# OpenDriveLab/ThinkTwice

Hardware: AMD Instinct MI355X
Metric: frames/sec forward (4-cam+LiDAR, thinktwice.py cfg) (higher is better)
Workload: dtype bf16x3h; 1 GPU; forward_inference thinktwice.py cfg: 8 frames x (2 sweeps x 4 cams x 448x896 + 65536-pt LiDAR), ResNet50+PAFPN+DepthNet+UNet+LSS splat, LidarNet, fusion, 5-stage decoder; parallelism=replicas x1 (no data-path collective), launch=eager launches, 3 batches in flight on alternating streams, batches_in_flight=3

## Files before the change

include/thinktwice_hip.h:

```cpp
#ifndef THINKTWICE_HIP_H
#define THINKTWICE_HIP_H

#include <stddef.h>
#include <stdint.h>

#ifdef __cplusplus
extern "C" {
#endif

#define TT_F32 0
#define TT_BF16 1
#define TT_F16 2

#define TT_ACT_NONE 0
#define TT_ACT_RELU 1
#define TT_ACT_SIGMOID 2
#define TT_ACT_GELU 3
#define TT_ACT_SOFTPLUS 4
#define TT_ACT_SOFTPLUS_CLAMP 5

const char* tt_last_error(void);
const char* tt_conv_last_kernel(void);
int tt_conv_set_trace(void* stamps_or_null);
int tt_version(void);

int tt_voxel_pool_fwd(int batch_size, int num_points, int num_channels,
                      int num_voxel_x, int num_voxel_y, int num_voxel_z,
                      const int32_t* geom_xyz, const float* input_features,
                      float* output_features, int32_t* pos_memo, void* stream);

long long tt_voxel_pool_workspace_bytes(int batch_size, int num_points, int num_channels,
                                        int num_voxel_x, int num_voxel_y);
int tt_voxel_pool_fwd_ws(int batch_size, int num_points, int num_channels,
                         int num_voxel_x, int num_voxel_y, int num_voxel_z,
                         const int32_t* geom_xyz, const float* input_features,
                         float* output_features, int32_t* pos_memo,
                         void* workspace, long long workspace_bytes, void* stream);
int tt_voxel_pool_fwd_plan(int batch_size, int num_points, int num_channels,
                           int num_voxel_x, int num_voxel_y, int num_voxel_z,
                           const int32_t* geom_xyz, const float* input_features,
                           float* output_features, int32_t* pos_memo,
                           void* workspace, long long workspace_bytes, int ws_entry, char* label, int label_bytes);

long long tt_voxel_pool_plan_bytes(int batch_size, int num_points, int num_voxel_x, int num_voxel_y);
long long tt_voxel_pool_plan_workspace_bytes(int batch_size, int num_points);
int tt_voxel_pool_plan_build(int batch_size, int num_points, int num_voxel_x, int num_voxel_y, int num_voxel_z,
                             const int32_t* geom_xyz, void* workspace, long long workspace_bytes, void* plan,
                             long long plan_bytes, void* stream);
long long tt_voxel_pool_planned_workspace_bytes(int batch_size, int num_points, int num_channels, int num_voxel_x,
                                                int num_voxel_y);
int tt_voxel_pool_fwd_planned(int batch_size, int num_points, int num_channels, int num_voxel_x, int num_voxel_y,
                              const void* plan, const float* input_features, float* output_features, void* workspace,
                              long long workspace_bytes, void* stream);

int tt_voxel_pool_bwd(int batch_size, int num_points, int num_channels,
                      int num_voxel_x, int num_voxel_y,
                      const int32_t* pos_memo, const float* grad_out_bhwc,
                      float* grad_in, void* stream);

int tt_frustum_voxel_index(int batch_size, int num_cams, int D, int fH, int fW,
                           const float* frustum, const float* mats,
                           const float* voxel_lo, const float* voxel_size,
                           int32_t* geom_xyz, float* geom_f32_or_null,
                           void* stream);

int tt_lift_splat_fwd(int batch_size, int num_cams, int D, int fH, int fW, int C,
                      int num_voxel_x, int num_voxel_y, int num_voxel_z,
                      const void* depth_logits, const void* context, int dtype,
                      const int32_t* geom_xyz, float* out, int out_cstride,
                      int out_coff, int rot_flip, void* stream);

long long tt_lift_splat_workspace_bytes(int batch_size, int num_cams, int D, int fH, int fW, int C,
                                        int num_voxel_x, int num_voxel_y);
int tt_lift_splat_fwd_ws(int batch_size, int num_cams, int D, int fH, int fW, int C,
                         int num_voxel_x, int num_voxel_y, int num_voxel_z,
                         const void* depth_logits, const void* context, int dtype,
                         const int32_t* geom_xyz, float* out, int out_cstride,
                         int out_coff, int rot_flip, void* ws, long long ws_bytes, void* stream);
int tt_lift_splat_fwd_plan(int batch_size, int num_cams, int D, int fH, int fW, int C,
                           int num_voxel_x, int num_voxel_y, int num_voxel_z,
                           const void* depth_logits, const void* context, int dtype,
                           const int32_t* geom_xyz, float* out, int out_cstride,
                           int out_coff, int rot_flip, void* ws, long long ws_bytes, char* label, int label_bytes);

typedef struct tt_conv_desc {
    const void* in;   int N, H, W, Cin, in_cstride, in_coff;
    long long in_nstride;
    const void* weight; int Cout, KH, KW, stride, pad, dil;
    void* out; int OH, OW, out_cstride, out_coff;
    long long out_nstride;
    int pixel_shuffle2;
    const float* scale; const float* shift;
    const float* shift_n; int shift_n_mod;
    const void* res1; int res1_cstride, res1_coff;
    const void* res2; int res2_cstride, res2_coff;
    int act;
    int dtype;
    int out_dtype;
    const int* gather_idx;
    const int* m_dev;
    float* splitk_ws;
    const void* weight_x3;
    const int* row_perm;
    const unsigned* row_mask;
    int splitk_slices;
    int in_pair, out_pair;
    const void* weight_h2;
    float* out2; int out2_cstride, out2_coff;
    int res1_up_h, res1_up_w;
    int res1_f32;
    int in_up2;
} tt_conv_desc;

int tt_conv2d_fwd(const tt_conv_desc* d, void* stream);
int tt_conv2d_splitk_slices(const tt_conv_desc* d);
int tt_conv2d_plan(const tt_conv_desc* d, char* label, int label_bytes);

int tt_seg_feedback_chain(const float* x, long long R, int x_stride, int K1, const float* w1, const float* scale1,
                          const float* shift1, int act1, const float* w2, const void* w2_x3, int N2, const float* scale2,
                          const float* shift2, int act2, float* out, int out_stride, int out_coff, void* stream);

typedef struct tt_chain_stage {
    const void* w; const float* bias;
    int K, Kp, N, act, in_sel;
    const float* res; int res_stride, res_coff;
    const float* side; const float* side_w; int side_stride, side_k;
    float* out; int out_stride, out_coff;
} tt_chain_stage;
int tt_mlp_chain(const float* x, long long R, int x_stride, int nstages, const tt_chain_stage* stages, int n_split,
                 void* stream);
long long tt_mlp_chain_wide_workspace_bytes(long long R, int nstages, const tt_chain_stage* stages);
int tt_mlp_chain_wide(const float* x, long long R, int x_stride, int nstages, const tt_chain_stage* stages, int n_groups,
                      void* workspace, long long workspace_bytes, void* stream);
int tt_mlp_chain_wide_max_workgroups(void);
int tt_mlp_chain_wide_faults(void);
int tt_device_faults(void);
int tt_clear_device_faults(void);
int tt_mlp_chain_wide_set_max_spin(int polls);
int tt_mlp_chain_wide_set_trace(void* stamps_or_null);

long long tt_dec_gru_scratch_floats(int B);
int tt_dec_gru(int B, const float* inp6, const float* state, float* fut, float* scratch, const void* const* w0,
               const float* const* wx, const float* const* b0, const void* const* w2, const float* const* b2,
               const void* wd0, const float* bd0, const void* wd2, const float* bd2, void* stream);
long long tt_dec_flatten_scratch_floats(int maps);
int tt_dec_flatten(int maps, const float* in, float* out, float* mids_or_null, float* scratch, const void* const* w,
                   const float* const* b, const float* bn_scale, const float* bn_shift, void* stream);
int tt_dec_set_trace(void* stamps_or_null);
long long tt_dec_bev_update_scratch_floats(int B);
int tt_dec_bev_update(int B, const float* bev, const float* G, float* out, long long out_bstride, float* out2,
                      long long out2_bstride, float* scratch, const void* w0, const float* b0, const void* const* w2,
                      const float* b2, void* stream);

int tt_nchw_to_nhwc_pad(const float* in, void* out, int N, int C, int H, int W, int Cp,
                        int out_dtype, void* stream);
int tt_nchw_to_nhwc_border(const float* in, void* out, int N, int C, int H, int W, int Cp, int Hp, int Wp,
                           int top, int left, int out_dtype, void* stream);
int tt_nhwc_to_nchw(const void* in, float* out, int N, int C, int H, int W, int cstride, int coff,
                    int in_dtype, void* stream);
int tt_maxpool3x3s2(const void* in, void* out, int N, int H, int W, int C, int dtype, void* stream);
int tt_upsample_nearest_add(void* dst, const void* src, int N, int H, int W, int C, int h, int w,
                            int dtype, void* stream);
int tt_bilinear_up2(const void* in, void* out, int N, int H, int W, int C, int dtype, void* stream);
int tt_bilinear_up2_pair(const float* in, float* out, int N, int H, int W, int C, void* stream);
int tt_spatial_pool(const void* in, float* out, int N, int HW, int C, int cstride, int coff, int mode,
                    int dtype, void* stream);
int tt_channel_gate(const void* x, const float* gate, const void* res, void* out, int N, int HW, int C,
                    int gate_act, int out_act, int dtype, void* stream);
int tt_affine_rows(const void* x, const float* scale, const float* shift, void* out, long long R, int C,
                   int x_stride, int out_stride, int act, int dtype, void* stream);
int tt_layernorm_rows(const void* x, const float* gamma, const float* beta, void* out, long long R,
                      int D, int x_stride, int out_stride, float eps, int dtype, void* stream);
int tt_copy_nhwc(const void* in, void* out, int N, int H, int W, int C, int in_cstride, int in_coff,
                 int out_cstride, int out_coff, int rot_flip, int in_dtype, int out_dtype, void* stream);
int tt_broadcast_rows(const void* v, void* out, int N, int HW, int C, int v_stride, int out_cstride,
                      int out_coff, int dtype, void* stream);
int tt_ew(const void* a, const void* b, const void* g, void* out, long long R, int C, int a_stride,
          int a_coff, int b_stride, int b_coff, int g_stride, int g_coff, int o_stride, int o_coff,
          int op, int act, int dtype, void* stream);
int tt_concat_rows(float* out, long long R, int out_stride, int nseg, const float* const* srcs, const int* strides,
                   const int* widths, const int* coffs, const int* divs, const int* mods, void* stream);

int tt_deform_im2col3x3(const void* x, const float* offsets, void* cols, int N, int H, int W, int C,
                        int off_cstride, int pad, int dtype, void* stream);

int tt_look_project_pack(int B, const float* wp, const float* lidar2img, const float* ida_mat,
                         float img_h, float img_w, float* ref_packed, int* query_of_slot,
                         int* count, int* max_len, void* stream);
int tt_look_gather_query(int B, const int* query_of_slot, const float* ref_packed, const float* wp,
                         const float* ctrl_softplus, const float* temporal_embedding,
                         const float* static_embedding, const float* measurement_feat,
                         const float* flattened_feat, const void* const* level_maps,
                         const int* level_hw, int maps_dtype, float* out, int row_stride, void* stream);
int tt_msda_sample(int B, const void* value, int value_dtype, const float* offsets, const float* logits,
                   const float* ref_packed, const int* level_hw, float* out, void* stream);
int tt_msda_sample_strided(int B, const void* value, int value_dtype, int value_cstride, int value_coff,
                           const float* offsets, const float* logits, const float* ref_packed, const int* level_hw,
                           float* out, void* stream);
int tt_sca_reduce(int B, const float* x, const int* max_len, float* out, void* stream);

int tt_look_query_ln(int B, const int* query_of_slot, const float* ref_packed, const float* wp, const float* ctrl,
                     int raw_ctrl, const float* temporal_embedding, const float* static_embedding,
                     const float* measurement_feat, const float* flattened_feat, const void* const* level_maps,
                     const int* level_hw, int maps_dtype, const float* gamma, const float* beta, float eps, float* out,
                     int row_stride, void* stream);
int tt_msda_sample_ln(int B, const void* value, int value_dtype, int value_cstride, int value_coff,
                      const float* offsets, const float* logits, const float* ref_packed, const int* level_hw,
                      const float* gamma, const float* beta, float eps, float* out, float* out_ln,
                      const int* max_len_or_null, void* stream);
int tt_msda_sample_proj_ln(int B, const void* const* level_maps, const int* level_hw, const float* offsets,
                           const float* logits, const float* ref_packed, const float* wvT, const float* bias,
                           const float* vshift, const float* gamma, const float* beta, float eps, float* out,
                           float* out_ln, const int* max_len_or_null, void* stream);
int tt_sca_reduce_ln(int B, const float* x, const int* max_len, const float* gamma, const float* beta, float eps,
                     float* out, void* stream);
int tt_dec_merge_in(int B, const float* fflat, const float* look, const float* temporal_embedding,
                    const float* measurement_feat, const float* gamma, const float* beta, float eps, float* out,
                    void* stream);

long long tt_lidar_voxelize_workspace_bytes(long long num_points_total);
int tt_lidar_voxelize(const float* points, int B, int Np, int nfeat, const float* pc_range_lo,
                      const float* voxel_size, const int* grid_xyz, int z_limit, int max_points,
                      void* workspace, long long workspace_bytes, float* voxel_feats, int* coords,
                      int* num_voxels, void* stream);
long long tt_lidar_voxelize_capped_workspace_bytes(long long num_points_total);
int tt_lidar_voxelize_capped(const float* points, int B, int Np, int nfeat, const float* pc_range_lo, const float* voxel_size,
                             const int* grid_xyz, int z_limit, int max_points, int max_voxels, void* workspace,
                             long long workspace_bytes, float* voxel_feats, int* coords, int* num_voxels, void* stream);
int tt_sp_volume_build(const int* coords, const int* num_rows, long long max_rows, int batch,
                       const int* dims_zyx, int* vol, void* stream);
long long tt_sp_strided_outputs_workspace_bytes(long long out_cells);
int tt_sp_strided_outputs(const int* in_coords, const int* in_rows, long long max_in, int batch,
                          const int* kernel_stride_pad, const int* out_dims_zyx, void* workspace,
                          long long workspace_bytes, int* out_vol, int* out_coords, int* out_rows,
                          long long max_out, void* stream);
int tt_sp_rulebook(const int* out_coords, const int* out_rows, long long max_out,
                   const int* kernel_stride_pad, const int* in_dims_zyx, const int* in_vol, int* nbr,
                   void* stream);
long long tt_sp_tile_plan_workspace_bytes(long long max_rows);
int tt_sp_tile_plan(const int* nbr, const int* num_rows, long long max_rows, int KV, void* workspace,
                    long long workspace_bytes, int* row_perm, unsigned* row_mask_sorted,
                    unsigned long long* pairs_or_null, void* stream);
int tt_sp_to_dense(const void* feats, const int* coords, const int* num_rows, long long max_rows, int C,
                   const int* dims_zyx, void* dense, int dtype, void* stream);

int tt_preprocess_images(const uint8_t* raw_hwc, int num_images, int H, int W, const float* mapx,
                         const float* mapy, int resized_h, int resized_w, int crop_y, int crop_x,
                         int out_h, int out_w, const float* mean3, const float* std3, void* out_nhwc,
                         int out_channels_padded, int out_dtype, float* out_nchw_or_null, void* stream);

#define TT_IDA_MAX_SETS 64
typedef struct tt_ida_set {
    int resized_h, resized_w;
    int crop_y, crop_x;
    int flip;
} tt_ida_set;
int tt_preprocess_images_ida(const uint8_t* raw_hwc, int B, int T, int N, int H, int W, const float* mapx,
                             const float* mapy, const tt_ida_set* sets, int out_h, int out_w, const float* mean3,
                             const float* std3, void* out_nhwc, int out_channels_padded, int out_dtype,
                             float* out_nchw_or_null, void* stream);
int tt_preprocess_labels_ida(const float* maps, int B, int N, int H, int W, const float* mapx, const float* mapy,
                             const tt_ida_set* sets, int out_h, int out_w, float* out, void* stream);

#define TT_AUG_MAX_OPS 8
#define TT_AUG_NOISE_K 4
#define TT_AUG_LUT 0
#define TT_AUG_NOISE 1
#define TT_AUG_DROPOUT 2
#define TT_AUG_COARSE 3
// ... 329 lines not shown
```

thinktwice_amd/build.py:

```python
import os
import subprocess
import sys
from concurrent.futures import ThreadPoolExecutor

from . import _lib

HERE = os.path.dirname(os.path.abspath(__file__))
CSRC = os.path.join(HERE, "csrc")
OBJ = os.path.join(CSRC, "_obj")
LIB = os.path.join(HERE, "libthinktwice_hip.so")
HIPCC = os.environ.get("HIPCC", "/opt/rocm/bin/hipcc")
FLAGS = ["--offload-arch=gfx950", "-O3", "-std=c++17", "-fPIC", "-munsafe-fp-atomics", "-ffp-contract=off",
         "-Wno-unused-result"]


EXTRA_FLAGS = {"conv_x3_pipe.hip": ["-fno-slp-vectorize"], "conv_x3_up2.hip": ["-fno-slp-vectorize"],
               "conv_x3_patch.hip": ["-fno-slp-vectorize"]}


def _sources():
    return sorted(f for f in os.listdir(CSRC) if f.endswith((".hip", ".cpp")))


def _deps_mtime():
    hdrs = [os.path.join(CSRC, f) for f in os.listdir(CSRC) if f.endswith((".h", ".inc"))]
    hdrs.append(os.path.join(HERE, "..", "include", "thinktwice_hip.h"))
    hdrs.append(os.path.abspath(__file__))
    return max(os.path.getmtime(h) for h in hdrs)


def _compile(src, hdr_mtime, verbose):
    obj = os.path.join(OBJ, src + ".o")
    spath = os.path.join(CSRC, src)
    if os.path.exists(obj) and os.path.getmtime(obj) > max(os.path.getmtime(spath), hdr_mtime):
        return obj
    cmd = [HIPCC] + FLAGS + EXTRA_FLAGS.get(src, []) + (["-x", "hip"] if src.endswith(".hip") else []) + ["-c", spath, "-o", obj]
    if verbose:
        print(" ".join(cmd), flush=True)
    subprocess.run(cmd, check=True)
    return obj


def write_plan_thunks():
    lines = ["// GENERATED by thinktwice_amd/build.py from include/thinktwice_hip.h -- do not edit.",
             "// One thunk per stream-taking entry: tt_plan argument vector -> the entry's own signature.", ""]
    table = []
    for name, p in _lib.prototypes().items():
        if not _lib.takes_stream(name, p.params):
            continue
        casts = []
        for i, (t, _) in enumerate(p.params[:-1]):
            if "*" in t:
                casts.append(f"({t})a[{i}].p")
            elif t in ("float", "double"):
                casts.append(f"({t})a[{i}].d")
            else:
                casts.append(f"({t})a[{i}].i")
        casts.append("stream")
        lines.append(f"static int thunk_{name}(const PlanVal* a, void* stream) {{ return {name}({', '.join(casts)}); }}")
        table.append((name, len(p.params) - 1))
    lines.append("")
    lines.append("static const PlanThunk kPlanThunks[] = {")
    for name, n in table:
        lines.append(f'    {{"{name}", thunk_{name}, {n}}},')
    lines.append("};")
    text = "\n".join(lines) + "\n"
    out = os.path.join(CSRC, "plan_thunks.inc")
    if not os.path.exists(out) or open(out).read() != text:
        open(out, "w").write(text)


def source_fingerprint():
    import hashlib
    h = hashlib.sha256()
    files = [os.path.join(CSRC, f) for f in sorted(os.listdir(CSRC)) if f.endswith((".hip", ".cpp", ".h"))]
    files.append(os.path.join(HERE, "..", "include", "thinktwice_hip.h"))
    for f in files:
        h.update(os.path.basename(f).encode())
        h.update(open(f, "rb").read())
    return h.hexdigest()[:16]


def build(verbose=True, force=False):
    os.makedirs(OBJ, exist_ok=True)
    write_plan_thunks()
    if force:
        for f in os.listdir(OBJ):
            os.remove(os.path.join(OBJ, f))
    hdr_mtime = _deps_mtime()
    srcs = _sources()
    with ThreadPoolExecutor(max_workers=min(8, len(srcs))) as ex:
        objs = list(ex.map(lambda s: _compile(s, hdr_mtime, verbose), srcs))
    if (not os.path.exists(LIB)) or any(os.path.getmtime(o) > os.path.getmtime(LIB) for o in objs):
        cmd = [HIPCC, "--offload-arch=gfx950", "-shared", "-fPIC", "-o", LIB] + objs
        if verbose:
            print(" ".join(cmd), flush=True)
        subprocess.run(cmd, check=True)
    host_src = os.path.join(HERE, "..", "tools", "plan_host.cpp")
    host_bin = os.path.join(HERE, "..", "tools", "plan_host")
    if os.path.exists(host_src) and (not os.path.exists(host_bin) or
                                     os.path.getmtime(host_bin) < max(os.path.getmtime(host_src), os.path.getmtime(LIB))):
        cmd = [HIPCC, "--offload-arch=gfx950", "-O2", "-std=c++17", "-Wno-unused-result", "-I", os.path.join(HERE, "..", "include"),
               host_src, "-L", HERE, "-lthinktwice_hip", "-Wl,-rpath,$ORIGIN/../thinktwice_amd", "-o", host_bin]
        if verbose:
            print(" ".join(cmd), flush=True)
        subprocess.run(cmd, check=True)
    return LIB


if __name__ == "__main__":
    build(verbose=True, force="--force" in sys.argv)
    print(LIB)
```

thinktwice_amd/csrc/conv_choose.cpp:

```cpp
#include <stdint.h>

#include "conv_choose.h"

namespace tt {
namespace {

bool aligned16(const void* p) { return (reinterpret_cast<uintptr_t>(p) & 15) == 0; }

void set_tile(ConvChoice* c, int family, int bn, int waves_m, int waves_n, int bkb, int stages) {
    c->family = family;
    c->bn = bn;
    c->waves_m = waves_m;
    c->waves_n = waves_n;
    c->bkb = bkb;
    c->stages = stages;
}

bool choose_h2(const ConvArgs& a, ConvChoice* c) {
    if (a.gather || a.m_dev || a.ws || a.pixel_shuffle2 || a.Cin % 64 != 0 || a.KH * a.KW > 31 || a.K < 64) return false;
    static const bool pipe = env_flag("TT_H2_PIPE", true);
    if (pipe && a.Cout % 128 == 0 && a.K >= 1152) set_tile(c, CONV_H2_PIPE, 128, 4, 1, 128, 32);
    else if (a.Cout > 64) set_tile(c, CONV_H2, 128, 4, 2, 128, 32);
    else set_tile(c, CONV_H2, 64, 8, 1, 128, 33);
    return true;
}

bool choose_small(const ConvArgs& a, ConvChoice* c) {
    if (a.gather || a.m_dev || a.M > 4096) return false;
    if ((long long)div_up(a.M, 32) * div_up(a.Cout, 32) > 4096) return false;
    set_tile(c, CONV_SMALL, 32, 1, 1, 32, 1);
    return true;
}

int tail_split_rows(const ConvArgs& a) {
    if (a.Cout % 256 != 0) return 0;
    const int tiles_m = div_up(a.M, 256), tiles_n = a.Cout / 256;
    const long long T = (long long)tiles_m * tiles_n;
    const int rounds = (int)((T + kNumCU - 1) / kNumCU);
    const int last = (int)(T - (long long)kNumCU * (rounds - 1));
    if (rounds < 2 || rounds > 8 || last > kNumCU / 4) return 0;
    const int peel = div_up(last, tiles_n);
    return peel < tiles_m ? tiles_m - peel : 0;
}

bool choose_x3_splitk(const ConvArgs& a, bool assume_ws, ConvChoice* c) {
    if (a.gather || a.m_dev || a.M < 512 || a.M > 8192 || a.Cout < 64 || a.KH * a.KW > 32) return false;
    if (a.Cin % 32 != 0 || a.K < 1024 || a.pixel_shuffle2) return false;
    const int tiles = div_up(a.M, 256) * div_up(a.Cout, 64);
    const int nk = a.K / 32;
    if (tiles >= 256) return false;
    int sp = 512 / tiles;
    if (sp > nk / 8) sp = nk / 8;
    if (sp > 16) sp = 16;
    if (sp < 2) return false;
    const int slices = div_up(nk, div_up(nk, sp));
    if (slices < 2 || (!assume_ws && a.ws_slices < slices)) return false;
    set_tile(c, CONV_GLDS, 64, 8, 1, 128, 2);
    c->x3 = true;
    c->splits = sp;
    c->slices = slices;
    return true;
}

bool choose_sp_runs_l2(const ConvArgs& a, ConvChoice* c) {
    if (!a.gather || a.row_perm || a.KH != 1 || a.KW != 27 || a.pixel_shuffle2 || a.M < kSpL2MinRows) return false;
    if ((a.Cin != 16 && a.Cin != 32) || (a.Cout != 16 && a.Cout != 32 && a.Cout != 64)) return false;
    if ((a.in_cstride & 3) || (a.in_coff & 3) || !aligned16(a.in) || !a.vec_epi || a.out_dtype != TT_F32) return false;
    set_tile(c, CONV_SP_RUNS_L2, 32, 8, 1, a.Cin * 4, 1);
    c->gather = c->x3 = true;
    return true;
}

bool choose_sp_runs(const ConvArgs& a, ConvChoice* c) {
    if (!a.gather || a.row_perm || a.KH != 1 || a.KW != 27) return false;
    if (a.stride != 1) return false;
    if (a.Cin % 32 != 0 || a.Cin > 128 || a.M < 2048 || a.pixel_shuffle2) return false;
    if ((a.in_cstride & 3) || (a.in_coff & 3)) return false;
    if (a.Cout == 32) set_tile(c, CONV_SP_RUNS, 32, 8, 1, 128, 2);
    else if (a.Cout == 64) set_tile(c, CONV_SP_RUNS, 64, 8, 1, 128, 2);
    else if (a.Cout == 128) set_tile(c, CONV_SP_RUNS, 128, 4, 2, 128, 2);
    else return false;
    c->gather = c->x3 = true;
    return true;
}

bool x3_pipe_ok(const ConvArgs& a, int bn) {
    return !(a.gather || a.m_dev || (bn != 256 && bn != 128) || a.Cout % bn != 0 || a.Cin % 32 != 0 || a.KH * a.KW > 31 || a.K < 64);
}

bool choose_x3_patch(const ConvArgs& a, ConvChoice* c) {
    static const bool on = env_flag("TT_X3_PATCH", true);
    if (!on || !(a.flags & 32) || a.M < kPatchMinRows) return false;
    if (a.KH != 3 || a.KW != 3 || a.stride != 1 || a.pad != 1 || a.dil != 1 || a.OH != a.H || a.OW != a.W) return false;
    if (a.Cin % 32 != 0 || !(a.Cout == 64 || (a.Cout >= 8 && a.Cout <= 32)) || !a.vec_epi || a.out_dtype != TT_F32) return false;
    if (a.res1 || a.res2 || a.shift_n || a.out2 || a.ws || a.pixel_shuffle2 || a.gather || a.m_dev) return false;
    if ((long long)a.H * a.W * a.in_cstride >= (1ll << 30)) return false;
    if (a.Cout == 64 && a.K >= 1152) return false;
    set_tile(c, CONV_X3_PATCH, a.Cout == 64 ? 64 : 32, 8, 1, 128, 3);
    return true;
}

bool choose_x3(const ConvArgs& a, ConvChoice* c) {
    c->x3 = true;
    if (a.gather) {
        if (choose_sp_runs_l2(a, c)) return true;
        if (choose_sp_runs(a, c)) return true;
        const bool cin_ok = a.Cin >= 16 && (a.Cin & (a.Cin - 1)) == 0;
        if (!cin_ok || a.M < 2048 || a.Cout < 16 || a.Cout > 128) return false;
        set_tile(c, CONV_GLDS, a.Cout <= 32 ? 32 : (a.Cout <= 64 ? 64 : 128), 8, 1, 128, 2);
        c->gather = true;
        return true;
    }
    if (a.m_dev || a.M < 2048 || a.KH * a.KW > 32) return false;
    if (a.Cin % 32 != 0 || a.K < 64) return false;
    const bool apair = (a.flags & 32) != 0;
    if (apair && (a.in_coff % 16 != 0 || a.in_cstride % 16 != 0)) return false;
    c->apair = apair;
    if (choose_x3_patch(a, c)) return true;
    if (a.Cout < 64) {
        if (a.Cout > 32 || a.Cout < 8) return false;
        if (!apair && a.M < (1 << 16)) return false;
        set_tile(c, CONV_GLDS, 32, 8, 1, 128, 2);
        return true;
    }
    const int tiles_m = div_up(a.M, 256);
    auto cost = [&](int bn, double rate) {
        const long long tiles = (long long)tiles_m * div_up(a.Cout, bn);
        return (double)((tiles + kNumCU - 1) / kNumCU) * bn / rate;
    };
    const bool wide = a.Cout % 256 == 0 || a.Cout > 512;
    const int main_rows = tail_split_rows(a);
    auto cost256 = [&]() {
        if (!main_rows) return cost(256, 1.0);
        const long long tn = a.Cout / 256;
        const long long main_tiles = (long long)main_rows * tn, tail_tiles = (long long)(tiles_m - main_rows) * tn * 4;
        return (double)((main_tiles + kNumCU - 1) / kNumCU) * 256 / 1.0 + (double)((tail_tiles + kNumCU - 1) / kNumCU) * 64 / 0.63;
    };
    const double c256 = wide ? cost256() : 1e30;
    const double c128 = a.Cout > 64 ? cost(128, (a.K >= 1152 && a.Cout % 128 == 0) ? 0.95 : 0.85) : 1e30;
    const double c64 = cost(64, 0.63);
    const int bn = (c256 <= c128 && c256 <= c64) ? 256 : (c128 <= c64 ? 128 : 64);
    static const bool pipe = env_flag("TT_X3_PIPE", true);
    if (pipe && a.K >= 1152 && bn != 64 && x3_pipe_ok(a, bn)) {
        static const bool run3 = env_flag("TT_X3_RUN3", true);
        const bool runs = run3 && a.KW == 3 && a.KH <= 5 && a.stride == 1 && a.dil == 1 && a.pad == 1 && a.OH == a.H && a.OW == a.W &&
                          (a.N == 1 || a.in_nstride == (long long)a.H * a.W * a.in_cstride);
        set_tile(c, runs ? CONV_X3_RUN3 : CONV_X3_PIPE, bn, 4, 1, 128, 23);
    } else if (bn == 256) {
        set_tile(c, CONV_GLDS, 256, 4, 2, 128, 23);
    } else {
        set_tile(c, CONV_GLDS, bn, 8, 1, 128, 2);
    }
    if (bn == 256) c->main_rows = main_rows;
    return true;
}

int choose_up2(const ConvArgs& a, const ConvFacts& f, ConvChoice* c) {
    TT_REQUIRE(f.dtype == TT_F32 && a.out_dtype == TT_F32 && f.weight_x3 && aligned16(f.weight_x3) && !f.weight_h2,
               "tt_conv2d_fwd: in_up2 goes with a bf16x3 layer (f32 storage, a 16-byte aligned weight_x3)");
    TT_REQUIRE(!a.gather && !a.m_dev && !a.ws && !a.pixel_shuffle2 && !(a.flags & 32) && !a.res1 && !a.res2 && !a.shift_n && !f.out2,
               "tt_conv2d_fwd: in_up2 takes no in_pair, residual, per-image shift, out2, split-K workspace, gather or pixel shuffle");
    TT_REQUIRE(a.KH == 3 && a.KW == 3 && a.stride == 1 && a.pad == 1 && a.dil == 1 && a.H % 2 == 0 && a.W % 2 == 0 && a.OH == a.H &&
                   a.OW == a.W,
               "tt_conv2d_fwd: in_up2 is a 3 x 3 / stride 1 / pad 1 layer over an even H x W (got %d x %d, k %d x %d s %d p %d d %d)", a.H,
               a.W, a.KH, a.KW, a.stride, a.pad, a.dil);
    TT_REQUIRE(a.Cin % 32 == 0 && a.Cout == 64 && a.M > 4096 && a.vec_epi,
               "tt_conv2d_fwd: in_up2 layer outside the kernel's contract (Cin %% 32 == 0, Cout == 64, more than 4096 rows, aligned "
               "output: M=%d Cin=%d Cout=%d)", a.M, a.Cin, a.Cout);
    const long long img = (long long)(a.H / 2) * (a.W / 2) * a.Cin;
    TT_REQUIRE(a.in_cstride == a.Cin && a.in_coff == 0 && a.in_nstride == img && img < (1ll << 30),
               "tt_conv2d_fwd: in_up2 reads a contiguous [N][H/2][W/2][Cin] source of less than 2^30 elements per image");
    set_tile(c, CONV_X3_UP2, 64, 8, 1, 128, 3);
    c->x3 = true;
    return 0;
}

bool choose_glds(const ConvArgs& a, int dtype, ConvChoice* c) {
    constexpr int min_tiles = 2;
    if (a.gather) {
        const bool cin_ok = a.Cin >= 16 && (a.Cin & (a.Cin - 1)) == 0;
        if (dtype == TT_F32 || !cin_ok || a.M < 2048 || a.Cout < 16 || a.Cout > 128) return false;
        if (a.Cout <= 32) set_tile(c, CONV_GLDS, 32, 8, 1, 128, 2);
        else if (a.Cout <= 64) set_tile(c, CONV_GLDS, 64, 8, 1, 128, 2);
        else set_tile(c, CONV_GLDS, 128, 4, 2, 128, 2);
        c->gather = true;
        return true;
    }
    if (a.m_dev || a.M < 2048 || a.Cout < 64 || a.KH * a.KW > 32) return false;
    if (dtype == TT_F32) {
        if (a.Cin % 16 != 0 || div_up(a.K, 16) < min_tiles) return false;
        if (a.Cout > 64) set_tile(c, CONV_GLDS, 128, 4, 2, 64, 3);
        else set_tile(c, CONV_GLDS, 64, 8, 1, 64, 3);
        return true;
    }
    if (a.Cin % 32 != 0 || div_up(a.K, 32) < min_tiles) return false;
    if (a.Cout > 64) {
        const long long tiles256 = (long long)div_up(a.M, 256) * (a.Cout / 256);
        if (a.Cout % 256 == 0 && tiles256 >= 200) {
            if (a.Cin % 64 == 0) {
                set_tile(c, CONV_GLDS, 256, 2, 4, 128, 2);
                c->main_rows = tail_split_rows(a);
            } else {
                set_tile(c, CONV_GLDS, 256, 2, 4, 64, 3);
            }
        } else if (a.K <= 512) {
            set_tile(c, CONV_GLDS, 128, 2, 2, 64, 3);
        } else {
            set_tile(c, CONV_GLDS, 128, 4, 2, 64, 3);
        }
        return true;
    }
    if (a.Cin % 64 == 0) set_tile(c, CONV_GLDS, 64, 8, 1, 128, 2);
    else set_tile(c, CONV_GLDS, 64, 8, 1, 64, 3);
    return true;
}

int choose_igemm(const ConvArgs& a, int dtype, bool ws, bool assume_ws, ConvChoice* c) {
    if (a.Cout > 64) set_tile(c, CONV_IGEMM, 128, 2, 2, 64, 2);
    else if (a.Cout > 32) set_tile(c, CONV_IGEMM, 64, 2, 2, 64, 2);
    else set_tile(c, CONV_IGEMM, 32, 4, 1, 64, 2);
    if (dtype != TT_F32) c->bkb = 128;
    c->gather = a.gather != nullptr;
    const int tiles = div_up(a.M, 128) * div_up(a.Cout, c->bn);
    const int nk = div_up(a.K, c->bkb / (dtype == TT_F32 ? 4 : 2));
    if (ws && !a.m_dev && tiles < 128 && nk >= 8) {
        int sp = div_up(512, tiles);
        if (sp > nk / 2) sp = nk / 2;
        if (sp > 64) sp = 64;
        c->splits = sp < 1 ? 1 : sp;
    }
    if (c->splits <= 1) return 0;
    c->slices = c->splits;
    if (!assume_ws) {
        c->slices = 0;
        if (a.ws_slices > 0) {
            const int eff = div_up(nk, div_up(nk, c->splits));
            TT_REQUIRE(a.ws_slices >= eff, "tt_conv2d_fwd: split-K workspace holds %d slices, %d needed", a.ws_slices, eff);
            c->slices = eff;
        }
    }
    return 0;
}

}

int conv_choose(const ConvArgs& a, const ConvFacts& f, ConvChoice* c) {
    *c = ConvChoice{};
    c->splits = 1;
    const bool ws = a.ws || f.assume_ws;
    if (a.flags & 256) return choose_up2(a, f, c);
    if (f.weight_h2) {
        TT_REQUIRE(aligned16(f.weight_h2), "tt_conv2d_fwd: weight_h2 must be 16-byte aligned");
        TT_REQUIRE(choose_h2(a, c), "tt_conv2d_fwd: weight_h2 layer outside the h2 kernel's contract (Cin=%d KH*KW=%d)", a.Cin,
                   a.KH * a.KW);
        return 0;
    }
    TT_REQUIRE(!f.out2 || a.vec_epi, "tt_conv2d_fwd: out2 needs the vector epilogue (aligned channel counts)");
    TT_REQUIRE(!f.res1_up || a.vec_epi, "tt_conv2d_fwd: an upsampled res1 needs the vector epilogue (aligned channel counts)");
    TT_REQUIRE(!f.res1_f32 || (a.vec_epi && a.res_vec), "tt_conv2d_fwd: an f32 res1 needs the vector epilogue and aligned residual rows");
    TT_REQUIRE(!(f.dtype == TT_F32 && a.out_dtype != TT_F32 && a.res1) || (a.vec_epi && a.res_vec),
               "tt_conv2d_fwd: a 16-bit output of an f32 layer with a residual needs the vector epilogue");
    if (a.flags & (32 | 64)) {
        TT_REQUIRE(a.vec_epi && aligned16(f.weight_x3) && a.K % 16 == 0,
                   "tt_conv2d_fwd: in_pair / out_pair need the vector epilogue and a 16-byte aligned weight_x3");
        TT_REQUIRE(choose_x3(a, c), "tt_conv2d_fwd: pair-format layer outside the LDS-DMA bf16x3 kernel's contract (M=%d Cin=%d Cout=%d)",
                   a.M, a.Cin, a.Cout);
        return 0;
    }
    if (!ws && !f.out2 && !f.res1_up && !f.res1_f32 && choose_small(a, c)) return 0;
    const bool x3 = f.weight_x3 && f.dtype == TT_F32;
    if (ws && x3 && a.K % 16 == 0 && aligned16(f.weight_x3) && choose_x3_splitk(a, f.assume_ws, c)) return 0;
    if (!ws && x3) {
        TT_REQUIRE(aligned16(f.weight_x3) && a.K % 16 == 0, "tt_conv2d_fwd: weight_x3 needs 16-byte alignment and K %% 16 == 0 (K = %d)",
                   a.K);
        if (choose_x3(a, c)) return 0;
        *c = ConvChoice{};
        c->splits = 1;
    }
    if (!ws && choose_glds(a, f.dtype, c)) return 0;
    return choose_igemm(a, f.dtype, ws, f.assume_ws, c);
}

ConvChoice conv_tail_choice(const ConvChoice& c) {
    ConvChoice t{};
    set_tile(&t, CONV_GLDS, 64, 8, 1, 128, 2);
    t.x3 = c.x3;
    t.apair = c.apair;
    t.splits = 1;
    return t;
}

void conv_label(const ConvChoice& c, int dtype, char* out, size_t bytes) {
    const char* tn = dtype == TT_F32 ? "float" : "16-bit";
    const char* pre = c.apair ? " pre-split A" : "";
    const char* tail = c.main_rows > 0 ? " + tail" : "";
    switch (c.family) {
        case CONV_H2: snprintf(out, bytes, "conv_h2_kernel<%d, %d, %d, %d, %d>", c.bn, c.waves_m, c.waves_n, c.stages / 10, c.stages % 10); break;
        case CONV_H2_PIPE: snprintf(out, bytes, "conv_h2_pipe_kernel"); break;
        case CONV_SMALL: snprintf(out, bytes, "conv_small_kernel"); break;
        case CONV_SP_RUNS_L2: snprintf(out, bytes, "sp_conv_runs_l2_kernel<%d>", c.bkb / 4); break;
        case CONV_SP_RUNS: snprintf(out, bytes, "sp_conv_runs_kernel<%d, %d, %d>", c.bn / (32 * c.waves_n), c.waves_m, c.waves_n); break;
        case CONV_X3_PIPE: snprintf(out, bytes, "conv_x3_pipe_kernel<%s>%s%s", c.bn == 128 ? "4, 1, 128" : "4, 1", pre, tail); break;
        case CONV_X3_RUN3: snprintf(out, bytes, "conv_x3_run3_kernel<%d>%s%s", c.bn, pre, tail); break;
        case CONV_X3_UP2: snprintf(out, bytes, "conv_x3_run3_kernel<%d, up2>", c.bn); break;
        case CONV_X3_PATCH: snprintf(out, bytes, "conv_x3_run3_kernel<%d, patch>%s", c.bn, pre); break;
        case CONV_GLDS:
            snprintf(out, bytes, "conv_igemm_glds_kernel<%s, %d, %d, %d, %d, %d, %s, %s>%s%s", tn, c.bn, c.waves_m, c.waves_n, c.bkb,
                     c.stages, c.gather ? "true" : "false", c.x3 ? "true" : "false", pre, c.splits > 1 ? " split-K" : tail);
            break;
        default: snprintf(out, bytes, "conv_igemm_kernel<%s, 128, %d>%s", tn, c.bn, c.splits > 1 ? " split-K" : ""); break;
    }
}

}
```

thinktwice_amd/csrc/conv_choose.h:

```cpp
#pragma once
#include <stddef.h>

#include "tt_common.h"

namespace tt {

struct ConvArgs {
    const void* in;
    const void* weight;
    void* out;
    const float* scale;
    const float* shift;
    const float* shift_n;
    const void* res1;
    const void* res2;
    const int* gather;
    const int* m_dev;
    const int* row_perm;
    const unsigned* row_mask;
    float* ws;
    long long in_nstride, out_nstride;
    int N, H, W, Cin, in_cstride, in_coff;
    int Cout, KH, KW, stride, pad, dil;
    int OH, OW, out_cstride, out_coff;
    int pixel_shuffle2, shift_n_mod;
    int res1_cstride, res1_coff, res2_cstride, res2_coff;
    int act, out_dtype;
    int M, K;
    int cin_fast;
    int out_fast;
    int vec_epi;
    int res_vec;
    int splits;
    int tiles_n;
    int m_begin;
    int ws_slices;
    int flags;
    int res1_up_h, res1_up_w;
    float* out2;
    int out2_cstride, out2_coff;
    long long* trace;
};

enum ConvFamily {
    CONV_H2,
    CONV_H2_PIPE,
    CONV_SMALL,
    CONV_SP_RUNS_L2,
    CONV_SP_RUNS,
    CONV_X3_PIPE,
    CONV_X3_RUN3,
    CONV_X3_UP2,
    CONV_X3_PATCH,
    CONV_GLDS,
    CONV_IGEMM,
};

constexpr int kSpL2MinRows = 16384;

constexpr int kPatchMinRows = 16384;

struct ConvFacts {
    int dtype;
    const void* weight_x3;
    const void* weight_h2;
    bool out2, res1_up, res1_f32;
    bool assume_ws;
};

struct ConvChoice {
    int family;
    int bn;
    int waves_m, waves_n, bkb, stages;
    bool gather, x3, apair;
    int main_rows;
    int splits;
    int slices;
};

int conv_choose(const ConvArgs& a, const ConvFacts& f, ConvChoice* c);
ConvChoice conv_tail_choice(const ConvChoice& c);
void conv_label(const ConvChoice& c, int dtype, char* out, size_t bytes);

}
```

thinktwice_amd/csrc/conv_common.h:

```cpp
#pragma once
#include <type_traits>
#include "bf16x3.h"
#include "conv_choose.h"

namespace tt {
extern thread_local char g_conv_kernel[96];
extern long long* g_conv_trace;

template <int TN>
__device__ __forceinline__ void zero_acc(f32x16 (&acc)[TN]) {
#pragma unroll
    for (int j = 0; j < TN; ++j)
#pragma unroll
        for (int r = 0; r < 16; ++r) acc[j][r] = 0.f;
}
template <int TM, int TN>
__device__ __forceinline__ void zero_acc(f32x16 (&acc)[TM][TN]) {
#pragma unroll
    for (int i = 0; i < TM; ++i) zero_acc(acc[i]);
}

template <int TN, int WTN>
__device__ __forceinline__ void stage_scaled(float* sC, const f32x16 (&acc)[TN], const float (&sc)[TN],
                                             const float (&sh)[TN], int lane) {
// ... 211 lines not shown
                        if constexpr (RM == 2) add_rvf(v, r1[q]);
                        else if constexpr (RM == 1) add_rv(v, r1[q]);
                        if (act == TT_ACT_RELU) {
#pragma unroll
                            for (int e = 0; e < CO; ++e) v[e] = v[e] > 0.f ? v[e] : 0.f;
                        }
                        store_row((long long)mr * p.out_cstride + obase, v);
                        if (out2) store_row2(mr, v);
                    }
                }
            };
            if (!has_r1) hot(std::integral_constant<int, 0>{});
            else if (EXT && sizeof(T) == 2 && r1_f32) {
                if constexpr (EXT && sizeof(T) == 2) hot(std::integral_constant<int, 2>{});
            } else hot(std::integral_constant<int, 1>{});
        } else {
#pragma unroll 1
            for (int pass = 0; pass < NPASS; ++pass) {
                const int rl = pass * rpp + row_in_pass;
                const int m = mb + rl;
                if (m >= Mlim || !col_ok) continue;
                float v[CO];
#pragma unroll
                for (int e = 0; e < CO; e += 4) {
                    const float4 t0 = *reinterpret_cast<const float4*>(sC + rl * LDC + col_l + e);
                    v[e] = t0.x; v[e + 1] = t0.y; v[e + 2] = t0.z; v[e + 3] = t0.w;
                }
                int n = 0;
                const int mo = p.row_perm ? p.row_perm[m] : m;
                const long long o = out_offset(mo, co, n);
                if (sn_loop) {
                    const float* sn = p.shift_n + (long long)(n % p.shift_n_mod) * cout_real + co;
#pragma unroll
                    for (int e = 0; e < CO; ++e) v[e] += sn[e];
                }
#pragma unroll
                for (int which = 0; which < 2; ++which) {
                    const void* rb = which ? p.res2 : p.res1;
                    if (!rb) continue;
                    const T* rp = reinterpret_cast<const T*>(rb) +
                                  (which ? (long long)mo : res1_row(mo)) * (which ? p.res2_cstride : p.res1_cstride) +
                                  (which ? p.res2_coff : p.res1_coff) + co;
                    if (which == 0 && r1_f32) {
                        const float* rf = reinterpret_cast<const float*>(rb) + res1_row(mo) * p.res1_cstride + p.res1_coff + co;
#pragma unroll
                        for (int e = 0; e < CO; ++e) v[e] += rf[e];
                    } else if (rvec) {
                        add_rv(v, *reinterpret_cast<const RV*>(rp));
                    } else {
#pragma unroll
                        for (int e = 0; e < CO; ++e) v[e] += Elem<T>::ld(rp + e);
                    }
                }
#pragma unroll
                for (int e = 0; e < CO; ++e) v[e] = apply_act(v[e], act);
                store_row(o, v);
                if (out2) store_row2(mo, v);
            }
        }
    }
}

template <typename T, int TM, int TN, int WTM, int WTN, bool EXT = (sizeof(T) == 4)>
__device__ __forceinline__ void conv_epilogue(const ConvArgs& p, f32x16 (&acc)[TM][TN], unsigned char* smem,
                                              int wave, int lane, int wm, int wn, int m0, int n0, int Mlim) {
    const int cout_real = p.pixel_shuffle2 ? (p.Cout >> 2) : p.Cout;
    const int ohw = p.OH * p.OW;
    if (p.act == 99) return;
    if (p.ws) {
#pragma unroll
        for (int j = 0; j < TN; ++j) {
            const int col = n0 + wn * WTN + j * 32 + (lane & 31);
            if (col >= p.Cout) continue;
#pragma unroll
            for (int i = 0; i < TM; ++i)
#pragma unroll
                for (int r = 0; r < 16; ++r) {
                    const int m = m0 + wm * WTM + i * 32 + (r & 3) + 8 * (r >> 2) + 4 * (lane >> 5);
                    if (m < Mlim) {
                        if (p.ws_slices > 0) p.ws[((long long)blockIdx.y * p.M + m) * p.Cout + col] = acc[i][j][r];
                        else unsafeAtomicAdd(p.ws + (long long)m * p.Cout + col, acc[i][j][r]);
                    }
                }
        }
        return;
    }
    float* sC = reinterpret_cast<float*>(smem) + wave * (32 * (WTN + 4));
    __syncthreads();
    if (p.vec_epi) {
        if (p.out_dtype == TT_F32 && !(p.flags & 64))
            conv_epilogue_vec<T, 4, TM, TN, WTM, WTN, EXT>(p, acc, sC, lane, wm, wn, m0, n0, Mlim);
        else
            conv_epilogue_vec<T, 8, TM, TN, WTM, WTN, EXT>(p, acc, sC, lane, wm, wn, m0, n0, Mlim);
        return;
    }
    constexpr int LDC = WTN + 4;
    const int act = p.act;
    float sc[TN], sh[TN];
    load_scale_shift<TN, WTN>(p, sc, sh, lane, wn, n0);
#pragma unroll
    for (int i = 0; i < TM; ++i) {
        stage_scaled<TN, WTN>(sC, acc[i], sc, sh, lane);
#pragma unroll 1
        for (int idx = lane; idx < 32 * WTN; idx += 64) {
            const int rl = idx / WTN, cl = idx - rl * WTN;
            const int m = m0 + wm * WTM + i * 32 + rl;
            const int col = n0 + wn * WTN + cl;
            if (m >= Mlim || col >= p.Cout) continue;
            int co = col, q = 0;
            if (p.pixel_shuffle2) {
                q = col / cout_real;
                co = col - q * cout_real;
            }
            float v = sC[rl * LDC + cl];
            const int n = m / ohw;
            const int mo = p.row_perm ? p.row_perm[m] : m;
            long long o;
            if (p.out_fast) {
                o = (long long)mo * p.out_cstride + p.out_coff + co;
            } else {
                const int rem = m - n * ohw;
                int oh = rem / p.OW, ow = rem - oh * p.OW;
                int OWo = p.OW;
                if (p.pixel_shuffle2) {
                    oh = 2 * oh + (q >> 1);
                    ow = 2 * ow + (q & 1);
                    OWo = 2 * p.OW;
                }
                o = (long long)n * p.out_nstride + ((long long)oh * OWo + ow) * p.out_cstride + p.out_coff + co;
            }
            if (p.shift_n) v += p.shift_n[(n % p.shift_n_mod) * cout_real + co];
            if (p.res1)
                v += Elem<T>::ld(reinterpret_cast<const T*>(p.res1) + (long long)mo * p.res1_cstride + p.res1_coff + co);
            if (p.res2)
                v += Elem<T>::ld(reinterpret_cast<const T*>(p.res2) + (long long)mo * p.res2_cstride + p.res2_coff + co);
            v = apply_act(v, act);
            if (p.out_dtype == TT_F32)
                reinterpret_cast<float*>(p.out)[o] = v;
            else
                store16(p.out, o, v, p.out_dtype);
            if (p.out2) p.out2[(long long)mo * p.out2_cstride + p.out2_coff + co] = v;
        }
    }
}

int launch_conv_h2(const ConvChoice& c, ConvArgs& a, hipStream_t st);
int launch_conv_small(ConvArgs& a, int dtype, hipStream_t st);
int launch_sp_conv_l2(const ConvChoice& c, ConvArgs& a, hipStream_t st);
int launch_sp_conv_runs(const ConvChoice& c, ConvArgs& a, hipStream_t st);
int launch_conv_x3_pipe(const ConvChoice& c, ConvArgs& a, hipStream_t st);
int launch_conv_glds(const ConvChoice& c, ConvArgs& a, int dtype, hipStream_t st);
int launch_conv_x3_up2(const ConvChoice& c, ConvArgs& a, hipStream_t st);
int launch_conv_x3_patch(const ConvChoice& c, ConvArgs& a, hipStream_t st);

}
```

thinktwice_amd/csrc/conv_igemm.hip:

```cpp
#include <stdlib.h>

#include "conv_common.h"

namespace tt {

template <typename T, int BM, int BN, int WAVES_M, int WAVES_N, bool GATHER, int KX = 1>
__global__ __launch_bounds__(256) void conv_igemm_kernel(const ConvArgs p) {
    constexpr int VEC = Elem<T>::kVec;
    constexpr int BKB = ((sizeof(T) == 4) ? 64 : 128) * KX;
    constexpr int BK = BKB / (int)sizeof(T);
    constexpr int VPR = BKB / 16;
    constexpr int ROWB = BKB + 16;
    constexpr int NVA = (BM * VPR + 255) / 256;
    constexpr int NVB = (BN * VPR + 255) / 256;
    constexpr int WTM = BM / WAVES_M, WTN = BN / WAVES_N;
    constexpr int TM = WTM / 32, TN = WTN / 32;
    static_assert(WAVES_M * WAVES_N == 4, "4 waves");

    extern __shared__ __attribute__((aligned(16))) unsigned char smem[];
    const int nbuf = (p.K > BK) ? 2 : 1;
    unsigned char* sA = smem;
    unsigned char* sB = smem + nbuf * BM * ROWB;

    const int tid = threadIdx.x;
// ... 93 lines not shown
                }
                if (j >= 0) {
                    const T* src = in + (long long)j * p.in_cstride + p.in_coff + ci;
                    ra[i] = *reinterpret_cast<const uint4*>(src);
                } else {
                    ra[i] = make_uint4(0, 0, 0, 0);
                }
            } else {
                const int ih = a_h0[i] + kh * p.dil;
                const int iw = a_w0[i] + kw * p.dil;
                const bool ok = a_ok[i] && (k < p.K) && ih >= 0 && ih < p.H && iw >= 0 && iw < p.W;
                if (ok) {
                    const T* src = in + a_base[i] + ((long long)ih * p.W + iw) * p.in_cstride + ci;
                    ra[i] = *reinterpret_cast<const uint4*>(src);
                } else {
                    ra[i] = make_uint4(0, 0, 0, 0);
                }
            }
        }
#pragma unroll
        for (int i = 0; i < NVB; ++i) {
            const int k = k0 + b_vc[i] * VEC;
            if (b_ok[i] && k < p.K) {
                rb[i] = *reinterpret_cast<const uint4*>(wgt + (long long)(n0 + b_row[i]) * p.K + k);
            } else {
                rb[i] = make_uint4(0, 0, 0, 0);
            }
        }
    };
    auto store_tile = [&](int buf) {
#pragma unroll
        for (int i = 0; i < NVA; ++i)
            if (tid + 256 * i < BM * VPR)
                *reinterpret_cast<uint4*>(sA + (buf * BM + a_row[i]) * ROWB + a_vc[i] * 16) = ra[i];
#pragma unroll
        for (int i = 0; i < NVB; ++i)
            if (tid + 256 * i < BN * VPR)
                *reinterpret_cast<uint4*>(sB + (buf * BN + b_row[i]) * ROWB + b_vc[i] * 16) = rb[i];
    };

    f32x16 acc[TM][TN];
    zero_acc(acc);

    if (GATHER && p.cin_fast) {
#pragma unroll
        for (int i = 0; i < NVA; ++i)
            jn[i] = (a_ok[i] && kt0 * BK < p.K) ? p.gather[a_base[i] + (kt0 * BK) / p.Cin] : -1;
    }
    load_tile(kt0);
    store_tile(0);
    __syncthreads();

    const int frag_off = (lane & 31) * ROWB + (lane >> 5) * 16;
    for (int kt = kt0; kt < nk; ++kt) {
        const int buf = (kt - kt0) & 1;
        if (kt + 1 < nk) load_tile(kt + 1);
        const unsigned char* tA = sA + (buf * BM + wm * WTM) * ROWB + frag_off;
        const unsigned char* tB = sB + (buf * BN + wn * WTN) * ROWB + frag_off;
#pragma unroll
        for (int kc = 0; kc < BKB / 32; ++kc) {
            uint4 fa[TM], fb[TN];
#pragma unroll
            for (int i = 0; i < TM; ++i)
                fa[i] = *reinterpret_cast<const uint4*>(tA + i * 32 * ROWB + kc * 32);
#pragma unroll
            for (int j = 0; j < TN; ++j)
                fb[j] = *reinterpret_cast<const uint4*>(tB + j * 32 * ROWB + kc * 32);
#pragma unroll
            for (int i = 0; i < TM; ++i)
#pragma unroll
                for (int j = 0; j < TN; ++j) Mfma<T>::run(fa[i], fb[j], acc[i][j]);
        }
        if (kt + 1 < nk) store_tile(buf ^ 1);
        __syncthreads();
    }

    conv_epilogue<T, TM, TN, WTM, WTN>(p, acc, smem, wave, lane, wm, wn, m0, n0, Mlim);
}

template <typename T>
__global__ __launch_bounds__(256) void splitk_finalize_kernel(const ConvArgs p) {
    const long long t = (long long)blockIdx.x * blockDim.x + threadIdx.x;
    if (t >= (long long)p.M * p.Cout) return;
    const int m = (int)(t / p.Cout), col = (int)(t % p.Cout);
    const int cout_real = p.pixel_shuffle2 ? (p.Cout >> 2) : p.Cout;
    int co = col, q = 0;
    if (p.pixel_shuffle2) { q = col / cout_real; co = col - q * cout_real; }
    const int ohw = p.OH * p.OW;
    const int n = m / ohw;
    const int rem = m - n * ohw;
    int oh = rem / p.OW, ow = rem - oh * p.OW, OWo = p.OW;
    if (p.pixel_shuffle2) { oh = 2 * oh + (q >> 1); ow = 2 * ow + (q & 1); OWo = 2 * p.OW; }
    const long long o = (long long)n * p.out_nstride + ((long long)oh * OWo + ow) * p.out_cstride + p.out_coff + co;
    float acc = p.ws[t];
    for (int sl = 1; sl < p.ws_slices; ++sl) acc += p.ws[(long long)sl * p.M * p.Cout + t];
    float v = acc * (p.scale ? p.scale[co] : 1.f) + (p.shift ? p.shift[co] : 0.f);
    if (p.shift_n) v += p.shift_n[(n % p.shift_n_mod) * cout_real + co];
    if (p.res1) v += Elem<T>::ld(reinterpret_cast<const T*>(p.res1) + (long long)m * p.res1_cstride + p.res1_coff + co);
    if (p.res2) v += Elem<T>::ld(reinterpret_cast<const T*>(p.res2) + (long long)m * p.res2_cstride + p.res2_coff + co);
    v = apply_act(v, p.act);
    if (p.out_dtype == TT_F32) reinterpret_cast<float*>(p.out)[o] = v;
    else store16(p.out, o, v, p.out_dtype);
}

template <typename T, int BM, int BN, int WAVES_M, int WAVES_N, bool GATHER, int KX = 1>
static int launch_conv(const ConvChoice& c, ConvArgs& a, hipStream_t st) {
    constexpr int BKB = ((sizeof(T) == 4) ? 64 : 128) * KX;
    constexpr int BK = BKB / (int)sizeof(T);
    constexpr int ROWB = BKB + 16;
    const int tiles_m = div_up(a.M, BM);
    a.tiles_n = div_up(a.Cout, BN);
    a.cin_fast = (a.Cin % BK == 0) ? 1 : 0;
    constexpr int WTN_ = BN / WAVES_N;
    size_t smem = (size_t)((a.K > BK) ? 2 : 1) * (BM + BN) * ROWB;
    const size_t epi = (size_t)4 * 32 * (WTN_ + 4) * 4;
    if (smem < epi) smem = epi;
    auto kern = conv_igemm_kernel<T, BM, BN, WAVES_M, WAVES_N, GATHER, KX>;
    const int tiles = tiles_m * a.tiles_n;
    a.splits = c.splits;
    if (a.splits <= 1) a.ws = nullptr;
    if (a.ws) a.ws_slices = c.slices;
    size_t mx = (size_t)2 * (BM + BN) * ROWB;
    if (mx < epi) mx = epi;
    if (mx > 48 * 1024 && lds_opt_in(reinterpret_cast<const void*>(kern), mx, "conv_igemm_kernel")) return -1;
    hipLaunchKernelGGL(kern, dim3((unsigned)tiles, (unsigned)a.splits), dim3(256), smem, st, a);
    return 1;
}

template <typename T, bool GATHER>
static int launch_igemm2(const ConvChoice& c, ConvArgs& a, hipStream_t st) {
    if (c.bn == 128 && c.waves_m == 2 && c.waves_n == 2) return launch_conv<T, 128, 128, 2, 2, GATHER>(c, a, st);
    if (c.bn == 64 && c.waves_m == 2 && c.waves_n == 2) return launch_conv<T, 128, 64, 2, 2, GATHER>(c, a, st);
    if (c.bn == 32 && c.waves_m == 4 && c.waves_n == 1) return launch_conv<T, 128, 32, 4, 1, GATHER>(c, a, st);
    TT_REQUIRE(false, "tt_conv2d_fwd: no conv_igemm_kernel for a %d-wide tile of %d x %d waves", c.bn, c.waves_m, c.waves_n);
}

static int launch_conv_igemm(const ConvChoice& c, ConvArgs& a, int dtype, hipStream_t st) {
    if (dtype == TT_F32) return a.gather ? launch_igemm2<float, true>(c, a, st) : launch_igemm2<float, false>(c, a, st);
    if (dtype == TT_F16) return a.gather ? launch_igemm2<f16_t, true>(c, a, st) : launch_igemm2<f16_t, false>(c, a, st);
    return a.gather ? launch_igemm2<uint16_t, true>(c, a, st) : launch_igemm2<uint16_t, false>(c, a, st);
}

static void launch_splitk_finalize(const ConvArgs& a, int dtype, hipStream_t st) {
    const dim3 grid((unsigned)div_up((long long)a.M * a.Cout, 256));
    if (dtype == TT_F32) hipLaunchKernelGGL(splitk_finalize_kernel<float>, grid, dim3(256), 0, st, a);
    else if (dtype == TT_F16) hipLaunchKernelGGL(splitk_finalize_kernel<f16_t>, grid, dim3(256), 0, st, a);
    else hipLaunchKernelGGL(splitk_finalize_kernel<uint16_t>, grid, dim3(256), 0, st, a);
}

}

using namespace tt;

static int conv2d_prepare(const tt_conv_desc* d, ConvArgs& a, ConvFacts& f) {
    TT_REQUIRE(d && d->in && d->weight && d->out, "tt_conv2d_fwd: null pointer");
    TT_REQUIRE(d->dtype == TT_F32 || d->dtype == TT_BF16 || d->dtype == TT_F16, "tt_conv2d_fwd: bad dtype %d", d->dtype);
    TT_REQUIRE(d->out_dtype == TT_F32 || d->out_dtype == d->dtype ||
                   (d->dtype == TT_F32 && (d->out_dtype == TT_F16 || d->out_dtype == TT_BF16) && !d->res2),
               "tt_conv2d_fwd: out_dtype must be TT_F32, the operand dtype, or (f32 operands, at most res1) a 16-bit type "
               "(got %d for dtype %d)", d->out_dtype, d->dtype);
    TT_REQUIRE(!d->res1_f32 || (d->weight_h2 && d->res1),
               "tt_conv2d_fwd: res1_f32 goes with an h2 layer's res1 (the other 16-bit kernels read residuals of their operand type)");
    TT_REQUIRE(d->dtype == TT_F32 || d->weight_h2 || (!d->out2 && d->res1_up_w <= 0),
               "tt_conv2d_fwd: out2 / res1_up_* exist in the f32-operand kernels and the h2 kernel only");
    TT_REQUIRE(!d->weight_h2 || (d->dtype == TT_F16 && !d->gather_idx && !d->splitk_ws && !d->pixel_shuffle2),
               "tt_conv2d_fwd: weight_h2 goes with dense TT_F16 operands (no split-K workspace, no pixel shuffle)");
    TT_REQUIRE(!d->out2 || (!d->splitk_ws && !d->pixel_shuffle2 && !d->gather_idx && d->out2_cstride % 4 == 0 &&
                            d->out2_coff % 4 == 0 && (reinterpret_cast<uintptr_t>(d->out2) & 15) == 0),
               "tt_conv2d_fwd: out2 needs a dense row-linear layer and 16-byte aligned rows");
    const int vec = d->dtype == TT_F32 ? 4 : 8;
    TT_REQUIRE(d->Cin > 0 && d->Cin % vec == 0 && d->in_cstride % vec == 0 && d->in_coff % vec == 0,
               "tt_conv2d_fwd: Cin=%d in_cstride=%d in_coff=%d must be multiples of %d (pad channels)",
               d->Cin, d->in_cstride, d->in_coff, vec);
    TT_REQUIRE((reinterpret_cast<uintptr_t>(d->in) & 15) == 0 &&
                   (reinterpret_cast<uintptr_t>(d->weight) & 15) == 0,
               "tt_conv2d_fwd: in/weight must be 16-byte aligned");
    TT_REQUIRE(d->N > 0 && d->H > 0 && d->W > 0 && d->Cout > 0 && d->KH > 0 && d->KW > 0 &&
                   d->stride > 0 && d->dil > 0 && d->OH > 0 && d->OW > 0,
               "tt_conv2d_fwd: bad geometry");
    TT_REQUIRE(!d->pixel_shuffle2 || d->Cout % 4 == 0, "tt_conv2d_fwd: pixel_shuffle2 needs Cout%%4==0");
    a.in = d->in; a.weight = d->weight; a.out = d->out;
    a.scale = d->scale; a.shift = d->shift; a.shift_n = d->shift_n;
    a.res1 = d->res1; a.res2 = d->res2;
    a.gather = d->gather_idx; a.m_dev = d->m_dev;
    a.row_perm = d->gather_idx ? d->row_perm : nullptr;
    a.row_mask = d->gather_idx ? d->row_mask : nullptr;
    TT_REQUIRE(!a.row_perm == !a.row_mask, "tt_conv2d_fwd: row_perm and row_mask come together");
    a.ws = d->splitk_ws;
    a.ws_slices = d->splitk_ws ? d->splitk_slices : 0;
    TT_REQUIRE(!d->gather_idx || (d->H == 1 && d->W == 1 && d->OH == 1 && d->OW == 1 && d->KH == 1 &&
                                  !d->pixel_shuffle2),
               "tt_conv2d_fwd: gather mode wants H=W=OH=OW=KH=1, KW=taps");
    a.N = d->N; a.H = d->H; a.W = d->W; a.Cin = d->Cin; a.in_cstride = d->in_cstride; a.in_coff = d->in_coff;
    a.in_nstride = d->in_nstride ? d->in_nstride : (long long)d->H * d->W * d->in_cstride;
    a.Cout = d->Cout; a.KH = d->KH; a.KW = d->KW; a.stride = d->stride; a.pad = d->pad; a.dil = d->dil;
    a.OH = d->OH; a.OW = d->OW; a.out_cstride = d->out_cstride; a.out_coff = d->out_coff;
    const long long def_on = (long long)d->OH * d->OW * d->out_cstride * (d->pixel_shuffle2 ? 4 : 1);
    a.out_nstride = d->out_nstride ? d->out_nstride : def_on;
    a.pixel_shuffle2 = d->pixel_shuffle2;
    a.shift_n_mod = d->shift_n_mod > 0 ? d->shift_n_mod : 1;
    a.res1_cstride = d->res1_cstride; a.res1_coff = d->res1_coff;
    a.res2_cstride = d->res2_cstride; a.res2_coff = d->res2_coff;
    a.act = d->act; a.out_dtype = d->out_dtype;
    a.out2 = d->out2; a.out2_cstride = d->out2_cstride; a.out2_coff = d->out2_coff;
    a.res1_up_h = d->res1_up_h; a.res1_up_w = d->res1_up_w;
    TT_REQUIRE((d->res1_up_h > 0) == (d->res1_up_w > 0) && (d->res1_up_w <= 0 || (d->res1 && !d->gather_idx && !d->splitk_ws &&
                                                                                 !d->pixel_shuffle2)),
               "tt_conv2d_fwd: res1_up_h / res1_up_w come together, with a dense layer's res1");
    a.M = d->N * d->OH * d->OW;
    a.K = d->KH * d->KW * d->Cin;
    a.out_fast = (!d->pixel_shuffle2 && a.out_nstride == (long long)d->OH * d->OW * d->out_cstride) ? 1 : 0;
    TT_REQUIRE(!(d->pixel_shuffle2 && (d->res1 || d->res2)),
               "tt_conv2d_fwd: residuals are not supported with pixel_shuffle2");
    a.tiles_n = 1; a.cin_fast = 0; a.m_begin = 0;
    a.trace = g_conv_trace;
    a.flags = 16;
    if (d->in_pair || d->out_pair) {
        TT_REQUIRE(d->dtype == TT_F32 && d->out_dtype == TT_F32 && d->weight_x3 && !d->gather_idx && !d->splitk_ws && !d->pixel_shuffle2,
                   "tt_conv2d_fwd: in_pair / out_pair go with dense bf16x3 layers (f32 containers, weight_x3, no split-K workspace)");
        TT_REQUIRE(!d->out_pair || (!d->res1 && !d->res2 && !d->shift_n && d->Cout % 16 == 0 && d->out_cstride % 16 == 0 &&
                                    d->out_coff % 16 == 0 && (reinterpret_cast<uintptr_t>(d->out) & 63) == 0),
                   "tt_conv2d_fwd: out_pair needs Cout / out_cstride / out_coff multiples of 16, a 64-byte aligned output and no "
                   "residual / per-image shift");
        if (d->in_pair) a.flags |= 32;
        if (d->out_pair) a.flags |= 64;
    }
    if (d->res1_f32) a.flags |= 128;
    if (d->in_up2) {
        TT_REQUIRE(!d->in_pair, "tt_conv2d_fwd: in_up2 reads an f32 source: it does not go with in_pair");
        a.in_nstride = d->in_nstride ? d->in_nstride : (long long)(d->H / 2) * (d->W / 2) * d->in_cstride;
        a.flags |= 256;
    }
    {
        const int co_vec = (d->out_dtype == TT_F32 && !d->out_pair) ? 4 : 8;
        const int osz = d->out_dtype == TT_F32 ? 4 : 2;
        const int cr = d->pixel_shuffle2 ? d->Cout / 4 : d->Cout;
        bool ok = (cr % co_vec == 0) && (d->out_cstride % co_vec == 0) && (d->out_coff % co_vec == 0) &&
                  (a.out_nstride % co_vec == 0) && ((reinterpret_cast<uintptr_t>(d->out) & 15) == 0);
        (void)osz;
        a.vec_epi = ok ? 1 : 0;
        auto res_ok = [&](const void* r, int cs, int co_) {
            return !r || ((cs % co_vec == 0) && (co_ % co_vec == 0) && ((reinterpret_cast<uintptr_t>(r) & 15) == 0));
        };
        a.res_vec = (res_ok(d->res1, d->res1_cstride, d->res1_coff) && res_ok(d->res2, d->res2_cstride, d->res2_coff)) ? 1 : 0;
    }
    f.dtype = d->dtype;
    f.weight_x3 = d->weight_x3;
    f.weight_h2 = d->weight_h2;
    f.out2 = d->out2 != nullptr;
    f.res1_up = d->res1_up_w > 0;
    f.res1_f32 = d->res1_f32 != 0;
    f.assume_ws = false;
    return 0;
}

extern "C" int tt_conv2d_fwd(const tt_conv_desc* d, void* stream) {
    ConvArgs a;
    ConvFacts f;
    ConvChoice c;
    if (const int r = conv2d_prepare(d, a, f)) return r;
    if (const int r = conv_choose(a, f, &c)) return r;
    hipStream_t st = (hipStream_t)stream;
    const bool pair = d->in_pair || d->out_pair;
    const char* what = "tt_conv2d_fwd";
    int r;
    if (c.x3) a.weight = d->weight_x3;
    switch (c.family) {
        case CONV_H2:
        case CONV_H2_PIPE:
            a.weight = d->weight_h2;
            what = "tt_conv2d_fwd(h2)";
            r = launch_conv_h2(c, a, st);
            break;
        case CONV_SMALL:
            what = "tt_conv2d_fwd(small)";
            r = launch_conv_small(a, d->dtype, st);
            break;
        case CONV_SP_RUNS_L2:
            what = "tt_conv2d_fwd(sp l2)";
            r = launch_sp_conv_l2(c, a, st);
            break;
        case CONV_SP_RUNS:
            what = "tt_conv2d_fwd(glds x3)";
            r = launch_sp_conv_runs(c, a, st);
            break;
        case CONV_X3_PIPE:
        case CONV_X3_RUN3:
            what = pair ? "tt_conv2d_fwd(glds x3, pair)" : "tt_conv2d_fwd(glds x3)";
            r = launch_conv_x3_pipe(c, a, st);
            break;
        case CONV_X3_UP2:
            what = "tt_conv2d_fwd(x3 up2)";
            r = launch_conv_x3_up2(c, a, st);
            break;
        case CONV_X3_PATCH:
            what = "tt_conv2d_fwd(x3 patch, pair)";
            r = launch_conv_x3_patch(c, a, st);
            break;
        case CONV_GLDS:
            what = !c.x3 ? "tt_conv2d_fwd(glds)" : c.splits > 1 ? "tt_conv2d_fwd(glds x3 split-K)" : pair ? "tt_conv2d_fwd(glds x3, pair)" : "tt_conv2d_fwd(glds x3)";
            if (c.splits > 1) a.ws_slices = c.slices;
            r = launch_conv_glds(c, a, d->dtype, st);
            break;
        default:
            a.row_perm = nullptr;
            a.row_mask = nullptr;
            r = launch_conv_igemm(c, a, d->dtype, st);
            break;
    }
    if (r < 0) return r;
    conv_label(c, d->dtype, g_conv_kernel, sizeof(g_conv_kernel));
    if (c.main_rows > 0) {
        ConvArgs t = a;
        t.m_begin = c.main_rows * 256;
        if (launch_conv_glds(conv_tail_choice(c), t, d->dtype, st) < 0) return -1;
    }
    if (c.splits > 1) launch_splitk_finalize(a, d->dtype, st);
    return check_launch(what);
}

extern "C" int tt_conv2d_splitk_slices(const tt_conv_desc* d) {
    ConvArgs a;
    ConvFacts f;
    ConvChoice c;
    if (conv2d_prepare(d, a, f)) return 0;
    if (d->in_pair || d->out_pair || d->in_up2 || d->weight_h2 || d->res1_up_w > 0) return 0;
    f.assume_ws = true;
    if (conv_choose(a, f, &c)) return 0;
    return c.splits > 1 ? c.slices : 0;
}

extern "C" int tt_conv2d_plan(const tt_conv_desc* d, char* label, int label_bytes) {
    ConvArgs a;
    ConvFacts f;
    ConvChoice c;
    if (const int r = conv2d_prepare(d, a, f)) return r;
    if (const int r = conv_choose(a, f, &c)) return r;
    TT_REQUIRE(label && label_bytes > 0, "tt_conv2d_plan: no room for the label");
    conv_label(c, d->dtype, label, (size_t)label_bytes);
    return 0;
}
```

thinktwice_amd/csrc/plan_thunks.inc:

```

static int thunk_tt_voxel_pool_fwd(const PlanVal* a, void* stream) { return tt_voxel_pool_fwd((int)a[0].i, (int)a[1].i, (int)a[2].i, (int)a[3].i, (int)a[4].i, (int)a[5].i, (const int32_t*)a[6].p, (const float*)a[7].p, (float*)a[8].p, (int32_t*)a[9].p, stream); }
static int thunk_tt_voxel_pool_fwd_ws(const PlanVal* a, void* stream) { return tt_voxel_pool_fwd_ws((int)a[0].i, (int)a[1].i, (int)a[2].i, (int)a[3].i, (int)a[4].i, (int)a[5].i, (const int32_t*)a[6].p, (const float*)a[7].p, (float*)a[8].p, (int32_t*)a[9].p, (void*)a[10].p, (long long)a[11].i, stream); }
static int thunk_tt_voxel_pool_plan_build(const PlanVal* a, void* stream) { return tt_voxel_pool_plan_build((int)a[0].i, (int)a[1].i, (int)a[2].i, (int)a[3].i, (int)a[4].i, (const int32_t*)a[5].p, (void*)a[6].p, (long long)a[7].i, (void*)a[8].p, (long long)a[9].i, stream); }
static int thunk_tt_voxel_pool_fwd_planned(const PlanVal* a, void* stream) { return tt_voxel_pool_fwd_planned((int)a[0].i, (int)a[1].i, (int)a[2].i, (int)a[3].i, (int)a[4].i, (const void*)a[5].p, (const float*)a[6].p, (float*)a[7].p, (void*)a[8].p, (long long)a[9].i, stream); }
static int thunk_tt_voxel_pool_bwd(const PlanVal* a, void* stream) { return tt_voxel_pool_bwd((int)a[0].i, (int)a[1].i, (int)a[2].i, (int)a[3].i, (int)a[4].i, (const int32_t*)a[5].p, (const float*)a[6].p, (float*)a[7].p, stream); }
static int thunk_tt_frustum_voxel_index(const PlanVal* a, void* stream) { return tt_frustum_voxel_index((int)a[0].i, (int)a[1].i, (int)a[2].i, (int)a[3].i, (int)a[4].i, (const float*)a[5].p, (const float*)a[6].p, (const float*)a[7].p, (const float*)a[8].p, (int32_t*)a[9].p, (float*)a[10].p, stream); }
static int thunk_tt_lift_splat_fwd(const PlanVal* a, void* stream) { return tt_lift_splat_fwd((int)a[0].i, (int)a[1].i, (int)a[2].i, (int)a[3].i, (int)a[4].i, (int)a[5].i, (int)a[6].i, (int)a[7].i, (int)a[8].i, (const void*)a[9].p, (const void*)a[10].p, (int)a[11].i, (const int32_t*)a[12].p, (float*)a[13].p, (int)a[14].i, (int)a[15].i, (int)a[16].i, stream); }
static int thunk_tt_lift_splat_fwd_ws(const PlanVal* a, void* stream) { return tt_lift_splat_fwd_ws((int)a[0].i, (int)a[1].i, (int)a[2].i, (int)a[3].i, (int)a[4].i, (int)a[5].i, (int)a[6].i, (int)a[7].i, (int)a[8].i, (const void*)a[9].p, (const void*)a[10].p, (int)a[11].i, (const int32_t*)a[12].p, (float*)a[13].p, (int)a[14].i, (int)a[15].i, (int)a[16].i, (void*)a[17].p, (long long)a[18].i, stream); }
static int thunk_tt_conv2d_fwd(const PlanVal* a, void* stream) { return tt_conv2d_fwd((const tt_conv_desc*)a[0].p, stream); }
static int thunk_tt_seg_feedback_chain(const PlanVal* a, void* stream) { return tt_seg_feedback_chain((const float*)a[0].p, (long long)a[1].i, (int)a[2].i, (int)a[3].i, (const float*)a[4].p, (const float*)a[5].p, (const float*)a[6].p, (int)a[7].i, (const float*)a[8].p, (const void*)a[9].p, (int)a[10].i, (const float*)a[11].p, (const float*)a[12].p, (int)a[13].i, (float*)a[14].p, (int)a[15].i, (int)a[16].i, stream); }
static int thunk_tt_mlp_chain(const PlanVal* a, void* stream) { return tt_mlp_chain((const float*)a[0].p, (long long)a[1].i, (int)a[2].i, (int)a[3].i, (const tt_chain_stage*)a[4].p, (int)a[5].i, stream); }
static int thunk_tt_mlp_chain_wide(const PlanVal* a, void* stream) { return tt_mlp_chain_wide((const float*)a[0].p, (long long)a[1].i, (int)a[2].i, (int)a[3].i, (const tt_chain_stage*)a[4].p, (int)a[5].i, (void*)a[6].p, (long long)a[7].i, stream); }
static int thunk_tt_dec_gru(const PlanVal* a, void* stream) { return tt_dec_gru((int)a[0].i, (const float*)a[1].p, (const float*)a[2].p, (float*)a[3].p, (float*)a[4].p, (const void* const*)a[5].p, (const float* const*)a[6].p, (const float* const*)a[7].p, (const void* const*)a[8].p, (const float* const*)a[9].p, (const void*)a[10].p, (const float*)a[11].p, (const void*)a[12].p, (const float*)a[13].p, stream); }
static int thunk_tt_dec_flatten(const PlanVal* a, void* stream) { return tt_dec_flatten((int)a[0].i, (const float*)a[1].p, (float*)a[2].p, (float*)a[3].p, (float*)a[4].p, (const void* const*)a[5].p, (const float* const*)a[6].p, (const float*)a[7].p, (const float*)a[8].p, stream); }
static int thunk_tt_dec_bev_update(const PlanVal* a, void* stream) { return tt_dec_bev_update((int)a[0].i, (const float*)a[1].p, (const float*)a[2].p, (float*)a[3].p, (long long)a[4].i, (float*)a[5].p, (long long)a[6].i, (float*)a[7].p, (const void*)a[8].p, (const float*)a[9].p, (const void* const*)a[10].p, (const float*)a[11].p, stream); }
static int thunk_tt_nchw_to_nhwc_pad(const PlanVal* a, void* stream) { return tt_nchw_to_nhwc_pad((const float*)a[0].p, (void*)a[1].p, (int)a[2].i, (int)a[3].i, (int)a[4].i, (int)a[5].i, (int)a[6].i, (int)a[7].i, stream); }
static int thunk_tt_nchw_to_nhwc_border(const PlanVal* a, void* stream) { return tt_nchw_to_nhwc_border((const float*)a[0].p, (void*)a[1].p, (int)a[2].i, (int)a[3].i, (int)a[4].i, (int)a[5].i, (int)a[6].i, (int)a[7].i, (int)a[8].i, (int)a[9].i, (int)a[10].i, (int)a[11].i, stream); }
static int thunk_tt_nhwc_to_nchw(const PlanVal* a, void* stream) { return tt_nhwc_to_nchw((const void*)a[0].p, (float*)a[1].p, (int)a[2].i, (int)a[3].i, (int)a[4].i, (int)a[5].i, (int)a[6].i, (int)a[7].i, (int)a[8].i, stream); }
static int thunk_tt_maxpool3x3s2(const PlanVal* a, void* stream) { return tt_maxpool3x3s2((const void*)a[0].p, (void*)a[1].p, (int)a[2].i, (int)a[3].i, (int)a[4].i, (int)a[5].i, (int)a[6].i, stream); }
static int thunk_tt_upsample_nearest_add(const PlanVal* a, void* stream) { return tt_upsample_nearest_add((void*)a[0].p, (const void*)a[1].p, (int)a[2].i, (int)a[3].i, (int)a[4].i, (int)a[5].i, (int)a[6].i, (int)a[7].i, (int)a[8].i, stream); }
static int thunk_tt_bilinear_up2(const PlanVal* a, void* stream) { return tt_bilinear_up2((const void*)a[0].p, (void*)a[1].p, (int)a[2].i, (int)a[3].i, (int)a[4].i, (int)a[5].i, (int)a[6].i, stream); }
static int thunk_tt_bilinear_up2_pair(const PlanVal* a, void* stream) { return tt_bilinear_up2_pair((const float*)a[0].p, (float*)a[1].p, (int)a[2].i, (int)a[3].i, (int)a[4].i, (int)a[5].i, stream); }
static int thunk_tt_spatial_pool(const PlanVal* a, void* stream) { return tt_spatial_pool((const void*)a[0].p, (float*)a[1].p, (int)a[2].i, (int)a[3].i, (int)a[4].i, (int)a[5].i, (int)a[6].i, (int)a[7].i, (int)a[8].i, stream); }
static int thunk_tt_channel_gate(const PlanVal* a, void* stream) { return tt_channel_gate((const void*)a[0].p, (const float*)a[1].p, (const void*)a[2].p, (void*)a[3].p, (int)a[4].i, (int)a[5].i, (int)a[6].i, (int)a[7].i, (int)a[8].i, (int)a[9].i, stream); }
static int thunk_tt_affine_rows(const PlanVal* a, void* stream) { return tt_affine_rows((const void*)a[0].p, (const float*)a[1].p, (const float*)a[2].p, (void*)a[3].p, (long long)a[4].i, (int)a[5].i, (int)a[6].i, (int)a[7].i, (int)a[8].i, (int)a[9].i, stream); }
static int thunk_tt_layernorm_rows(const PlanVal* a, void* stream) { return tt_layernorm_rows((const void*)a[0].p, (const float*)a[1].p, (const float*)a[2].p, (void*)a[3].p, (long long)a[4].i, (int)a[5].i, (int)a[6].i, (int)a[7].i, (float)a[8].d, (int)a[9].i, stream); }
static int thunk_tt_copy_nhwc(const PlanVal* a, void* stream) { return tt_copy_nhwc((const void*)a[0].p, (void*)a[1].p, (int)a[2].i, (int)a[3].i, (int)a[4].i, (int)a[5].i, (int)a[6].i, (int)a[7].i, (int)a[8].i, (int)a[9].i, (int)a[10].i, (int)a[11].i, (int)a[12].i, stream); }
static int thunk_tt_broadcast_rows(const PlanVal* a, void* stream) { return tt_broadcast_rows((const void*)a[0].p, (void*)a[1].p, (int)a[2].i, (int)a[3].i, (int)a[4].i, (int)a[5].i, (int)a[6].i, (int)a[7].i, (int)a[8].i, stream); }
static int thunk_tt_ew(const PlanVal* a, void* stream) { return tt_ew((const void*)a[0].p, (const void*)a[1].p, (const void*)a[2].p, (void*)a[3].p, (long long)a[4].i, (int)a[5].i, (int)a[6].i, (int)a[7].i, (int)a[8].i, (int)a[9].i, (int)a[10].i, (int)a[11].i, (int)a[12].i, (int)a[13].i, (int)a[14].i, (int)a[15].i, (int)a[16].i, stream); }
static int thunk_tt_concat_rows(const PlanVal* a, void* stream) { return tt_concat_rows((float*)a[0].p, (long long)a[1].i, (int)a[2].i, (int)a[3].i, (const float* const*)a[4].p, (const int*)a[5].p, (const int*)a[6].p, (const int*)a[7].p, (const int*)a[8].p, (const int*)a[9].p, stream); }
static int thunk_tt_deform_im2col3x3(const PlanVal* a, void* stream) { return tt_deform_im2col3x3((const void*)a[0].p, (const float*)a[1].p, (void*)a[2].p, (int)a[3].i, (int)a[4].i, (int)a[5].i, (int)a[6].i, (int)a[7].i, (int)a[8].i, (int)a[9].i, stream); }
static int thunk_tt_look_project_pack(const PlanVal* a, void* stream) { return tt_look_project_pack((int)a[0].i, (const float*)a[1].p, (const float*)a[2].p, (const float*)a[3].p, (float)a[4].d, (float)a[5].d, (float*)a[6].p, (int*)a[7].p, (int*)a[8].p, (int*)a[9].p, stream); }
static int thunk_tt_look_gather_query(const PlanVal* a, void* stream) { return tt_look_gather_query((int)a[0].i, (const int*)a[1].p, (const float*)a[2].p, (const float*)a[3].p, (const float*)a[4].p, (const float*)a[5].p, (const float*)a[6].p, (const float*)a[7].p, (const float*)a[8].p, (const void* const*)a[9].p, (const int*)a[10].p, (int)a[11].i, (float*)a[12].p, (int)a[13].i, stream); }
static int thunk_tt_msda_sample(const PlanVal* a, void* stream) { return tt_msda_sample((int)a[0].i, (const void*)a[1].p, (int)a[2].i, (const float*)a[3].p, (const float*)a[4].p, (const float*)a[5].p, (const int*)a[6].p, (float*)a[7].p, stream); }
static int thunk_tt_msda_sample_strided(const PlanVal* a, void* stream) { return tt_msda_sample_strided((int)a[0].i, (const void*)a[1].p, (int)a[2].i, (int)a[3].i, (int)a[4].i, (const float*)a[5].p, (const float*)a[6].p, (const float*)a[7].p, (const int*)a[8].p, (float*)a[9].p, stream); }
static int thunk_tt_sca_reduce(const PlanVal* a, void* stream) { return tt_sca_reduce((int)a[0].i, (const float*)a[1].p, (const int*)a[2].p, (float*)a[3].p, stream); }
static int thunk_tt_look_query_ln(const PlanVal* a, void* stream) { return tt_look_query_ln((int)a[0].i, (const int*)a[1].p, (const float*)a[2].p, (const float*)a[3].p, (const float*)a[4].p, (int)a[5].i, (const float*)a[6].p, (const float*)a[7].p, (const float*)a[8].p, (const float*)a[9].p, (const void* const*)a[10].p, (const int*)a[11].p, (int)a[12].i, (const float*)a[13].p, (const float*)a[14].p, (float)a[15].d, (float*)a[16].p, (int)a[17].i, stream); }
static int thunk_tt_msda_sample_ln(const PlanVal* a, void* stream) { return tt_msda_sample_ln((int)a[0].i, (const void*)a[1].p, (int)a[2].i, (int)a[3].i, (int)a[4].i, (const float*)a[5].p, (const float*)a[6].p, (const float*)a[7].p, (const int*)a[8].p, (const float*)a[9].p, (const float*)a[10].p, (float)a[11].d, (float*)a[12].p, (float*)a[13].p, (const int*)a[14].p, stream); }
static int thunk_tt_msda_sample_proj_ln(const PlanVal* a, void* stream) { return tt_msda_sample_proj_ln((int)a[0].i, (const void* const*)a[1].p, (const int*)a[2].p, (const float*)a[3].p, (const float*)a[4].p, (const float*)a[5].p, (const float*)a[6].p, (const float*)a[7].p, (const float*)a[8].p, (const float*)a[9].p, (const float*)a[10].p, (float)a[11].d, (float*)a[12].p, (float*)a[13].p, (const int*)a[14].p, stream); }
static int thunk_tt_sca_reduce_ln(const PlanVal* a, void* stream) { return tt_sca_reduce_ln((int)a[0].i, (const float*)a[1].p, (const int*)a[2].p, (const float*)a[3].p, (const float*)a[4].p, (float)a[5].d, (float*)a[6].p, stream); }
static int thunk_tt_dec_merge_in(const PlanVal* a, void* stream) { return tt_dec_merge_in((int)a[0].i, (const float*)a[1].p, (const float*)a[2].p, (const float*)a[3].p, (const float*)a[4].p, (const float*)a[5].p, (const float*)a[6].p, (float)a[7].d, (float*)a[8].p, stream); }
static int thunk_tt_lidar_voxelize(const PlanVal* a, void* stream) { return tt_lidar_voxelize((const float*)a[0].p, (int)a[1].i, (int)a[2].i, (int)a[3].i, (const float*)a[4].p, (const float*)a[5].p, (const int*)a[6].p, (int)a[7].i, (int)a[8].i, (void*)a[9].p, (long long)a[10].i, (float*)a[11].p, (int*)a[12].p, (int*)a[13].p, stream); }
static int thunk_tt_lidar_voxelize_capped(const PlanVal* a, void* stream) { return tt_lidar_voxelize_capped((const float*)a[0].p, (int)a[1].i, (int)a[2].i, (int)a[3].i, (const float*)a[4].p, (const float*)a[5].p, (const int*)a[6].p, (int)a[7].i, (int)a[8].i, (int)a[9].i, (void*)a[10].p, (long long)a[11].i, (float*)a[12].p, (int*)a[13].p, (int*)a[14].p, stream); }
static int thunk_tt_sp_volume_build(const PlanVal* a, void* stream) { return tt_sp_volume_build((const int*)a[0].p, (const int*)a[1].p, (long long)a[2].i, (int)a[3].i, (const int*)a[4].p, (int*)a[5].p, stream); }
static int thunk_tt_sp_strided_outputs(const PlanVal* a, void* stream) { return tt_sp_strided_outputs((const int*)a[0].p, (const int*)a[1].p, (long long)a[2].i, (int)a[3].i, (const int*)a[4].p, (const int*)a[5].p, (void*)a[6].p, (long long)a[7].i, (int*)a[8].p, (int*)a[9].p, (int*)a[10].p, (long long)a[11].i, stream); }
static int thunk_tt_sp_rulebook(const PlanVal* a, void* stream) { return tt_sp_rulebook((const int*)a[0].p, (const int*)a[1].p, (long long)a[2].i, (const int*)a[3].p, (const int*)a[4].p, (const int*)a[5].p, (int*)a[6].p, stream); }
static int thunk_tt_sp_tile_plan(const PlanVal* a, void* stream) { return tt_sp_tile_plan((const int*)a[0].p, (const int*)a[1].p, (long long)a[2].i, (int)a[3].i, (void*)a[4].p, (long long)a[5].i, (int*)a[6].p, (unsigned*)a[7].p, (unsigned long long*)a[8].p, stream); }
static int thunk_tt_sp_to_dense(const PlanVal* a, void* stream) { return tt_sp_to_dense((const void*)a[0].p, (const int*)a[1].p, (const int*)a[2].p, (long long)a[3].i, (int)a[4].i, (const int*)a[5].p, (void*)a[6].p, (int)a[7].i, stream); }
static int thunk_tt_preprocess_images(const PlanVal* a, void* stream) { return tt_preprocess_images((const uint8_t*)a[0].p, (int)a[1].i, (int)a[2].i, (int)a[3].i, (const float*)a[4].p, (const float*)a[5].p, (int)a[6].i, (int)a[7].i, (int)a[8].i, (int)a[9].i, (int)a[10].i, (int)a[11].i, (const float*)a[12].p, (const float*)a[13].p, (void*)a[14].p, (int)a[15].i, (int)a[16].i, (float*)a[17].p, stream); }
static int thunk_tt_preprocess_images_ida(const PlanVal* a, void* stream) { return tt_preprocess_images_ida((const uint8_t*)a[0].p, (int)a[1].i, (int)a[2].i, (int)a[3].i, (int)a[4].i, (int)a[5].i, (const float*)a[6].p, (const float*)a[7].p, (const tt_ida_set*)a[8].p, (int)a[9].i, (int)a[10].i, (const float*)a[11].p, (const float*)a[12].p, (void*)a[13].p, (int)a[14].i, (int)a[15].i, (float*)a[16].p, stream); }
static int thunk_tt_preprocess_labels_ida(const PlanVal* a, void* stream) { return tt_preprocess_labels_ida((const float*)a[0].p, (int)a[1].i, (int)a[2].i, (int)a[3].i, (int)a[4].i, (const float*)a[5].p, (const float*)a[6].p, (const tt_ida_set*)a[7].p, (int)a[8].i, (int)a[9].i, (float*)a[10].p, stream); }
static int thunk_tt_photometric_u8(const PlanVal* a, void* stream) { return tt_photometric_u8((const uint8_t*)a[0].p, (int)a[1].i, (int)a[2].i, (int)a[3].i, (int)a[4].i, (const tt_aug_program*)a[5].p, (const tt_aug_program*)a[6].p, (void*)a[7].p, (long long)a[8].i, (uint8_t*)a[9].p, stream); }
static int thunk_tt_preprocess_images_ida_aug(const PlanVal* a, void* stream) { return tt_preprocess_images_ida_aug((const uint8_t*)a[0].p, (int)a[1].i, (int)a[2].i, (int)a[3].i, (int)a[4].i, (int)a[5].i, (const float*)a[6].p, (const float*)a[7].p, (const tt_ida_set*)a[8].p, (int)a[9].i, (int)a[10].i, (const float*)a[11].p, (const float*)a[12].p, (void*)a[13].p, (int)a[14].i, (int)a[15].i, (float*)a[16].p, (const tt_aug_program*)a[17].p, (const tt_aug_program*)a[18].p, (void*)a[19].p, (long long)a[20].i, stream); }
static int thunk_tt_decode_depth_u8(const PlanVal* a, void* stream) { return tt_decode_depth_u8((const uint8_t*)a[0].p, (long long)a[1].i, (float*)a[2].p, stream); }
static int thunk_tt_rgb2hsv_u8(const PlanVal* a, void* stream) { return tt_rgb2hsv_u8((const uint8_t*)a[0].p, (long long)a[1].i, (const tt_hsv_tables*)a[2].p, (uint8_t*)a[3].p, stream); }
static int thunk_tt_decode_seg_u8(const PlanVal* a, void* stream) { return tt_decode_seg_u8((const uint8_t*)a[0].p, (int)a[1].i, (int)a[2].i, (int)a[3].i, (int)a[4].i, (const uint8_t*)a[5].p, (long long)a[6].i, (const tt_seg_decode_conf*)a[7].p, (void*)a[8].p, (long long)a[9].i, (float*)a[10].p, stream); }
static int thunk_tt_decode_seg_u8_phases(const PlanVal* a, void* stream) { return tt_decode_seg_u8_phases((const uint8_t*)a[0].p, (int)a[1].i, (int)a[2].i, (int)a[3].i, (int)a[4].i, (const uint8_t*)a[5].p, (long long)a[6].i, (const tt_seg_decode_conf*)a[7].p, (void*)a[8].p, (long long)a[9].i, (float*)a[10].p, (int)a[11].i, stream); }
static int thunk_tt_png_decode_u8(const PlanVal* a, void* stream) { return tt_png_decode_u8((const uint8_t*)a[0].p, (long long)a[1].i, (const tt_png_image*)a[2].p, (const tt_png_image*)a[3].p, (int)a[4].i, (void*)a[5].p, (long long)a[6].i, (uint8_t*)a[7].p, (long long)a[8].i, (int32_t*)a[9].p, stream); }
static int thunk_tt_png_decode_u8_phases(const PlanVal* a, void* stream) { return tt_png_decode_u8_phases((const uint8_t*)a[0].p, (long long)a[1].i, (const tt_png_image*)a[2].p, (const tt_png_image*)a[3].p, (int)a[4].i, (void*)a[5].p, (long long)a[6].i, (uint8_t*)a[7].p, (long long)a[8].i, (int32_t*)a[9].p, (int)a[10].i, stream); }
static int thunk_tt_checksum_ranges_u8(const PlanVal* a, void* stream) { return tt_checksum_ranges_u8((const uint8_t*)a[0].p, (long long)a[1].i, (const tt_checksum_range*)a[2].p, (const tt_checksum_range*)a[3].p, (int)a[4].i, (int)a[5].i, (const uint32_t*)a[6].p, (uint32_t*)a[7].p, (void*)a[8].p, (long long)a[9].i, stream); }
static int thunk_tt_png_decode_u8_verified(const PlanVal* a, void* stream) { return tt_png_decode_u8_verified((const uint8_t*)a[0].p, (long long)a[1].i, (const tt_png_image*)a[2].p, (const tt_png_image*)a[3].p, (int)a[4].i, (const tt_png_chunk*)a[5].p, (const tt_png_chunk*)a[6].p, (int)a[7].i, (int)a[8].i, (void*)a[9].p, (long long)a[10].i, (uint8_t*)a[11].p, (long long)a[12].i, (int32_t*)a[13].p, stream); }
static int thunk_tt_grad_norm_clip(const PlanVal* a, void* stream) { return tt_grad_norm_clip((const float*)a[0].p, (long long)a[1].i, (float)a[2].d, (float*)a[3].p, (float*)a[4].p, stream); }
static int thunk_tt_adamw_step(const PlanVal* a, void* stream) { return tt_adamw_step((float*)a[0].p, (const float*)a[1].p, (float*)a[2].p, (float*)a[3].p, (long long)a[4].i, (float)a[5].d, (float)a[6].d, (float)a[7].d, (float)a[8].d, (float)a[9].d, (int)a[10].i, (const float*)a[11].p, stream); }
static int thunk_tt_adamw_step_dev(const PlanVal* a, void* stream) { return tt_adamw_step_dev((float*)a[0].p, (const float*)a[1].p, (float*)a[2].p, (float*)a[3].p, (long long)a[4].i, (float)a[5].d, (float)a[6].d, (float)a[7].d, (float)a[8].d, (float)a[9].d, (const int*)a[10].p, (const float*)a[11].p, stream); }
static int thunk_tt_adamw_advance(const PlanVal* a, void* stream) { return tt_adamw_advance((int*)a[0].p, (const float*)a[1].p, stream); }
static int thunk_tt_grad_gather(const PlanVal* a, void* stream) { return tt_grad_gather((const tt_grad_seg*)a[0].p, (int)a[1].i, (float*)a[2].p, (const float*)a[3].p, (int)a[4].i, stream); }
static int thunk_tt_loss_smooth_l1(const PlanVal* a, void* stream) { return tt_loss_smooth_l1((const float*)a[0].p, (const float*)a[1].p, (long long)a[2].i, (int)a[3].i, (long long)a[4].i, (float)a[5].d, (float)a[6].d, (int)a[7].i, (float*)a[8].p, (void*)a[9].p, stream); }
static int thunk_tt_loss_smooth_l1_bwd(const PlanVal* a, void* stream) { return tt_loss_smooth_l1_bwd((const float*)a[0].p, (const float*)a[1].p, (long long)a[2].i, (int)a[3].i, (long long)a[4].i, (float)a[5].d, (float)a[6].d, (float*)a[7].p, stream); }
static int thunk_tt_loss_beta_kl_bwd(const PlanVal* a, void* stream) { return tt_loss_beta_kl_bwd((const float*)a[0].p, (const float*)a[1].p, (const float*)a[2].p, (const float*)a[3].p, (long long)a[4].i, (int)a[5].i, (long long)a[6].i, (float)a[7].d, (float*)a[8].p, (float*)a[9].p, stream); }
static int thunk_tt_loss_beta_kl(const PlanVal* a, void* stream) { return tt_loss_beta_kl((const float*)a[0].p, (const float*)a[1].p, (const float*)a[2].p, (const float*)a[3].p, (long long)a[4].i, (int)a[5].i, (long long)a[6].i, (float)a[7].d, (float*)a[8].p, (void*)a[9].p, stream); }
static int thunk_tt_loss_l1_cols(const PlanVal* a, void* stream) { return tt_loss_l1_cols((const float*)a[0].p, (const float*)a[1].p, (long long)a[2].i, (const float*)a[3].p, (const float*)a[4].p, (long long)a[5].i, (int)a[6].i, (float*)a[7].p, (void*)a[8].p, stream); }
static int thunk_tt_loss_seg_focal(const PlanVal* a, void* stream) { return tt_loss_seg_focal((const float*)a[0].p, (int)a[1].i, (int)a[2].i, (const float*)a[3].p, (int)a[4].i, (int)a[5].i, (int)a[6].i, (int)a[7].i, (float*)a[8].p, (void*)a[9].p, stream); }
static int thunk_tt_loss_seg_focal_bwd(const PlanVal* a, void* stream) { return tt_loss_seg_focal_bwd((const float*)a[0].p, (int)a[1].i, (int)a[2].i, (const float*)a[3].p, (int)a[4].i, (int)a[5].i, (int)a[6].i, (int)a[7].i, (const float*)a[8].p, (const float*)a[9].p, (float*)a[10].p, stream); }
static int thunk_tt_loss_depth_bce(const PlanVal* a, void* stream) { return tt_loss_depth_bce((const float*)a[0].p, (int)a[1].i, (int)a[2].i, (const float*)a[3].p, (int)a[4].i, (int)a[5].i, (int)a[6].i, (int)a[7].i, (float)a[8].d, (float)a[9].d, (float*)a[10].p, (void*)a[11].p, stream); }
static int thunk_tt_loss_depth_bce_bwd(const PlanVal* a, void* stream) { return tt_loss_depth_bce_bwd((const float*)a[0].p, (int)a[1].i, (int)a[2].i, (const float*)a[3].p, (int)a[4].i, (int)a[5].i, (int)a[6].i, (int)a[7].i, (float)a[8].d, (float)a[9].d, (const float*)a[10].p, (const float*)a[11].p, (float*)a[12].p, stream); }
static int thunk_tt_conv2d_wgrad(const PlanVal* a, void* stream) { return tt_conv2d_wgrad((const float*)a[0].p, (int)a[1].i, (int)a[2].i, (int)a[3].i, (int)a[4].i, (int)a[5].i, (int)a[6].i, (const float*)a[7].p, (int)a[8].i, (int)a[9].i, (int)a[10].i, (int)a[11].i, (int)a[12].i, (int)a[13].i, (int)a[14].i, (int)a[15].i, (int)a[16].i, (int)a[17].i, (int)a[18].i, (int)a[19].i, (float*)a[20].p, (void*)a[21].p, (long long)a[22].i, stream); }
static int thunk_tt_conv2d_wgrad_x3(const PlanVal* a, void* stream) { return tt_conv2d_wgrad_x3((const float*)a[0].p, (int)a[1].i, (int)a[2].i, (int)a[3].i, (int)a[4].i, (int)a[5].i, (int)a[6].i, (const float*)a[7].p, (int)a[8].i, (int)a[9].i, (int)a[10].i, (int)a[11].i, (int)a[12].i, (int)a[13].i, (int)a[14].i, (int)a[15].i, (int)a[16].i, (int)a[17].i, (int)a[18].i, (int)a[19].i, (float*)a[20].p, (void*)a[21].p, (long long)a[22].i, stream); }
static int thunk_tt_conv_epilogue_bwd(const PlanVal* a, void* stream) { return tt_conv_epilogue_bwd((const float*)a[0].p, (int)a[1].i, (int)a[2].i, (const float*)a[3].p, (int)a[4].i, (int)a[5].i, (const float*)a[6].p, (int)a[7].i, (int)a[8].i, (const float*)a[9].p, (int)a[10].i, (int)a[11].i, (const float*)a[12].p, (const float*)a[13].p, (long long)a[14].i, (int)a[15].i, (int)a[16].i, (float*)a[17].p, (int)a[18].i, (int)a[19].i, (float*)a[20].p, (int)a[21].i, (int)a[22].i, (float*)a[23].p, (int)a[24].i, (int)a[25].i, (int)a[26].i, (float*)a[27].p, (float*)a[28].p, (int)a[29].i, (const int*)a[30].p, (const float*)a[31].p, (const float*)a[32].p, (void*)a[33].p, (long long)a[34].i, stream); }
static int thunk_tt_gather_conv_wgrad(const PlanVal* a, void* stream) { return tt_gather_conv_wgrad((const float*)a[0].p, (int)a[1].i, (int)a[2].i, (const int*)a[3].p, (const int*)a[4].p, (long long)a[5].i, (int)a[6].i, (const float*)a[7].p, (int)a[8].i, (int)a[9].i, (int)a[10].i, (int)a[11].i, (float*)a[12].p, (void*)a[13].p, (long long)a[14].i, stream); }
static int thunk_tt_sp_inverse_rulebook(const PlanVal* a, void* stream) { return tt_sp_inverse_rulebook((const int*)a[0].p, (const int*)a[1].p, (long long)a[2].i, (int)a[3].i, (int*)a[4].p, stream); }
static int thunk_tt_sp_from_dense(const PlanVal* a, void* stream) { return tt_sp_from_dense((const float*)a[0].p, (const int*)a[1].p, (const int*)a[2].p, (long long)a[3].i, (int)a[4].i, (int)a[5].i, (int)a[6].i, (int)a[7].i, (float*)a[8].p, stream); }
static int thunk_tt_maxpool3x3s2_bwd(const PlanVal* a, void* stream) { return tt_maxpool3x3s2_bwd((const float*)a[0].p, (const float*)a[1].p, (float*)a[2].p, (int)a[3].i, (int)a[4].i, (int)a[5].i, (int)a[6].i, stream); }
static int thunk_tt_upsample_nearest_add_bwd(const PlanVal* a, void* stream) { return tt_upsample_nearest_add_bwd((const float*)a[0].p, (float*)a[1].p, (int)a[2].i, (int)a[3].i, (int)a[4].i, (int)a[5].i, (int)a[6].i, (int)a[7].i, stream); }
static int thunk_tt_bilinear_up2_bwd(const PlanVal* a, void* stream) { return tt_bilinear_up2_bwd((const float*)a[0].p, (float*)a[1].p, (int)a[2].i, (int)a[3].i, (int)a[4].i, (int)a[5].i, stream); }
static int thunk_tt_channel_gate_bwd(const PlanVal* a, void* stream) { return tt_channel_gate_bwd((const float*)a[0].p, (const float*)a[1].p, (const float*)a[2].p, (float*)a[3].p, (float*)a[4].p, (int)a[5].i, (int)a[6].i, (int)a[7].i, (const float*)a[8].p, (float*)a[9].p, stream); }
static int thunk_tt_spatial_meanmax_bwd(const PlanVal* a, void* stream) { return tt_spatial_meanmax_bwd((const float*)a[0].p, (const float*)a[1].p, (float*)a[2].p, (int)a[3].i, (int)a[4].i, (int)a[5].i, stream); }
static int thunk_tt_spatial_mean_bwd(const PlanVal* a, void* stream) { return tt_spatial_mean_bwd((const float*)a[0].p, (float*)a[1].p, (int)a[2].i, (int)a[3].i, (int)a[4].i, (int)a[5].i, (int)a[6].i, stream); }
static int thunk_tt_ew_bwd(const PlanVal* a, void* stream) { return tt_ew_bwd((int)a[0].i, (int)a[1].i, (long long)a[2].i, (int)a[3].i, (const float*)a[4].p, (int)a[5].i, (int)a[6].i, (const float*)a[7].p, (int)a[8].i, (int)a[9].i, (const float*)a[10].p, (int)a[11].i, (int)a[12].i, (const float*)a[13].p, (int)a[14].i, (int)a[15].i, (const float*)a[16].p, (int)a[17].i, (int)a[18].i, (float*)a[19].p, (int)a[20].i, (int)a[21].i, (float*)a[22].p, (int)a[23].i, (int)a[24].i, (float*)a[25].p, (int)a[26].i, (int)a[27].i, stream); }
static int thunk_tt_look_gather_query_bwd(const PlanVal* a, void* stream) { return tt_look_gather_query_bwd((int)a[0].i, (const int*)a[1].p, (const float*)a[2].p, (const float*)a[3].p, (int)a[4].i, (float*)a[5].p, (float*)a[6].p, (float*)a[7].p, (float*)a[8].p, (float* const*)a[9].p, (const int*)a[10].p, stream); }
static int thunk_tt_msda_sample_bwd(const PlanVal* a, void* stream) { return tt_msda_sample_bwd((int)a[0].i, (const float*)a[1].p, (int)a[2].i, (int)a[3].i, (const float*)a[4].p, (const float*)a[5].p, (const float*)a[6].p, (const int*)a[7].p, (const float*)a[8].p, (float*)a[9].p, (float*)a[10].p, (float*)a[11].p, stream); }
static int thunk_tt_sca_reduce_bwd(const PlanVal* a, void* stream) { return tt_sca_reduce_bwd((int)a[0].i, (const float*)a[1].p, (const int*)a[2].p, (float*)a[3].p, stream); }
static int thunk_tt_layernorm_rows_bwd(const PlanVal* a, void* stream) { return tt_layernorm_rows_bwd((const float*)a[0].p, (const float*)a[1].p, (const float*)a[2].p, (float*)a[3].p, (float*)a[4].p, (float*)a[5].p, (long long)a[6].i, (int)a[7].i, (int)a[8].i, (int)a[9].i, (int)a[10].i, (float)a[11].d, (void*)a[12].p, (long long)a[13].i, stream); }
static int thunk_tt_concat_piece_bwd(const PlanVal* a, void* stream) { return tt_concat_piece_bwd((const float*)a[0].p, (int)a[1].i, (int)a[2].i, (long long)a[3].i, (int)a[4].i, (int)a[5].i, (int)a[6].i, (float*)a[7].p, (int)a[8].i, (int)a[9].i, stream); }
static int thunk_tt_broadcast_rows_bwd(const PlanVal* a, void* stream) { return tt_broadcast_rows_bwd((const float*)a[0].p, (float*)a[1].p, (int)a[2].i, (int)a[3].i, (int)a[4].i, (int)a[5].i, (int)a[6].i, (int)a[7].i, stream); }
static int thunk_tt_lift_splat_bwd(const PlanVal* a, void* stream) { return tt_lift_splat_bwd((int)a[0].i, (int)a[1].i, (int)a[2].i, (int)a[3].i, (int)a[4].i, (int)a[5].i, (int)a[6].i, (int)a[7].i, (int)a[8].i, (const float*)a[9].p, (const float*)a[10].p, (const int32_t*)a[11].p, (const float*)a[12].p, (int)a[13].i, (int)a[14].i, (float*)a[15].p, (float*)a[16].p, stream); }
static int thunk_tt_deform_im2col3x3_bwd(const PlanVal* a, void* stream) { return tt_deform_im2col3x3_bwd((const float*)a[0].p, (const float*)a[1].p, (const float*)a[2].p, (float*)a[3].p, (float*)a[4].p, (int)a[5].i, (int)a[6].i, (int)a[7].i, (int)a[8].i, (int)a[9].i, (int)a[10].i, stream); }
static int thunk_tt_lidar_merge_half_sweeps(const PlanVal* a, void* stream) { return tt_lidar_merge_half_sweeps((const float*)a[0].p, (int)a[1].i, (const float*)a[2].p, (int)a[3].i, (const float*)a[4].p, (float)a[5].d, (float*)a[6].p, stream); }
static int thunk_tt_lidar_union_sweeps(const PlanVal* a, void* stream) { return tt_lidar_union_sweeps((const float*)a[0].p, (long long)a[1].i, (const tt_union_sweep*)a[2].p, (int)a[3].i, (int)a[4].i, (int)a[5].i, (float*)a[6].p, stream); }
static int thunk_tt_bn_stats(const PlanVal* a, void* stream) { return tt_bn_stats((const float*)a[0].p, (long long)a[1].i, (int)a[2].i, (int)a[3].i, (int)a[4].i, (const int*)a[5].p, (int)a[6].i, (double*)a[7].p, (void*)a[8].p, (long long)a[9].i, stream); }
static int thunk_tt_bn_finalize(const PlanVal* a, void* stream) { return tt_bn_finalize((const double*)a[0].p, (int)a[1].i, (int)a[2].i, (const float*)a[3].p, (const float*)a[4].p, (float)a[5].d, (float)a[6].d, (float*)a[7].p, (float*)a[8].p, (float*)a[9].p, (float*)a[10].p, (float*)a[11].p, (float*)a[12].p, stream); }
static int thunk_tt_bn_apply(const PlanVal* a, void* stream) { return tt_bn_apply((const float*)a[0].p, (long long)a[1].i, (int)a[2].i, (int)a[3].i, (int)a[4].i, (const int*)a[5].p, (int)a[6].i, (const float*)a[7].p, (const float*)a[8].p, (const float*)a[9].p, (const float*)a[10].p, (int)a[11].i, (int)a[12].i, (const float*)a[13].p, (int)a[14].i, (int)a[15].i, (int)a[16].i, (float*)a[17].p, (int)a[18].i, (int)a[19].i, stream); }
static int thunk_tt_bn_bwd_reduce(const PlanVal* a, void* stream) { return tt_bn_bwd_reduce((float*)a[0].p, (int)a[1].i, (int)a[2].i, (const float*)a[3].p, (int)a[4].i, (int)a[5].i, (const float*)a[6].p, (int)a[7].i, (int)a[8].i, (long long)a[9].i, (int)a[10].i, (const int*)a[11].p, (int)a[12].i, (const float*)a[13].p, (const float*)a[14].p, (int)a[15].i, (float*)a[16].p, (int)a[17].i, (int)a[18].i, (float*)a[19].p, (int)a[20].i, (int)a[21].i, (double*)a[22].p, (void*)a[23].p, (long long)a[24].i, stream); }
static int thunk_tt_bn_bwd_apply(const PlanVal* a, void* stream) { return tt_bn_bwd_apply((const float*)a[0].p, (int)a[1].i, (int)a[2].i, (const float*)a[3].p, (int)a[4].i, (int)a[5].i, (long long)a[6].i, (int)a[7].i, (const int*)a[8].p, (int)a[9].i, (const double*)a[10].p, (const double*)a[11].p, (const float*)a[12].p, (const float*)a[13].p, (const float*)a[14].p, (float*)a[15].p, (int)a[16].i, (int)a[17].i, stream); }
static int thunk_tt_dropout_fwd(const PlanVal* a, void* stream) { return tt_dropout_fwd((const float*)a[0].p, (float*)a[1].p, (long long)a[2].i, (float)a[3].d, (unsigned long long)a[4].i, (const uint8_t*)a[5].p, (uint8_t*)a[6].p, stream); }
static int thunk_tt_dropout_bwd(const PlanVal* a, void* stream) { return tt_dropout_bwd((const float*)a[0].p, (const uint8_t*)a[1].p, (float*)a[2].p, (long long)a[3].i, (float)a[4].d, stream); }
static int thunk_tt_action_post(const PlanVal* a, void* stream) { return tt_action_post((const float*)a[0].p, (const float*)a[1].p, (const float*)a[2].p, (float)a[3].d, (float)a[4].d, (float)a[5].d, (float)a[6].d, (const tt_action_cfg*)a[7].p, (tt_action_state*)a[8].p, (double*)a[9].p, stream); }
static int thunk_tt_fill_u32(const PlanVal* a, void* stream) { return tt_fill_u32((void*)a[0].p, (long long)a[1].i, (unsigned)a[2].i, stream); }
static int thunk_tt_copy_bytes(const PlanVal* a, void* stream) { return tt_copy_bytes((void*)a[0].p, (const void*)a[1].p, (long long)a[2].i, stream); }

static const PlanThunk kPlanThunks[] = {
    {"tt_voxel_pool_fwd", thunk_tt_voxel_pool_fwd, 10},
    {"tt_voxel_pool_fwd_ws", thunk_tt_voxel_pool_fwd_ws, 12},
    {"tt_voxel_pool_plan_build", thunk_tt_voxel_pool_plan_build, 10},
    {"tt_voxel_pool_fwd_planned", thunk_tt_voxel_pool_fwd_planned, 10},
    {"tt_voxel_pool_bwd", thunk_tt_voxel_pool_bwd, 8},
    {"tt_frustum_voxel_index", thunk_tt_frustum_voxel_index, 11},
    {"tt_lift_splat_fwd", thunk_tt_lift_splat_fwd, 17},
    {"tt_lift_splat_fwd_ws", thunk_tt_lift_splat_fwd_ws, 19},
    {"tt_conv2d_fwd", thunk_tt_conv2d_fwd, 1},
    {"tt_seg_feedback_chain", thunk_tt_seg_feedback_chain, 17},
    {"tt_mlp_chain", thunk_tt_mlp_chain, 6},
    {"tt_mlp_chain_wide", thunk_tt_mlp_chain_wide, 8},
    {"tt_dec_gru", thunk_tt_dec_gru, 14},
    {"tt_dec_flatten", thunk_tt_dec_flatten, 9},
    {"tt_dec_bev_update", thunk_tt_dec_bev_update, 12},
    {"tt_nchw_to_nhwc_pad", thunk_tt_nchw_to_nhwc_pad, 8},
    {"tt_nchw_to_nhwc_border", thunk_tt_nchw_to_nhwc_border, 12},
    {"tt_nhwc_to_nchw", thunk_tt_nhwc_to_nchw, 9},
    {"tt_maxpool3x3s2", thunk_tt_maxpool3x3s2, 7},
    {"tt_upsample_nearest_add", thunk_tt_upsample_nearest_add, 9},
    {"tt_bilinear_up2", thunk_tt_bilinear_up2, 7},
    {"tt_bilinear_up2_pair", thunk_tt_bilinear_up2_pair, 6},
    {"tt_spatial_pool", thunk_tt_spatial_pool, 9},
    {"tt_channel_gate", thunk_tt_channel_gate, 10},
    {"tt_affine_rows", thunk_tt_affine_rows, 10},
    {"tt_layernorm_rows", thunk_tt_layernorm_rows, 10},
    {"tt_copy_nhwc", thunk_tt_copy_nhwc, 13},
    {"tt_broadcast_rows", thunk_tt_broadcast_rows, 9},
    {"tt_ew", thunk_tt_ew, 17},
    {"tt_concat_rows", thunk_tt_concat_rows, 10},
    {"tt_deform_im2col3x3", thunk_tt_deform_im2col3x3, 10},
    {"tt_look_project_pack", thunk_tt_look_project_pack, 10},
    {"tt_look_gather_query", thunk_tt_look_gather_query, 14},
    {"tt_msda_sample", thunk_tt_msda_sample, 8},
    {"tt_msda_sample_strided", thunk_tt_msda_sample_strided, 10},
    {"tt_sca_reduce", thunk_tt_sca_reduce, 4},
    {"tt_look_query_ln", thunk_tt_look_query_ln, 18},
    {"tt_msda_sample_ln", thunk_tt_msda_sample_ln, 15},
    {"tt_msda_sample_proj_ln", thunk_tt_msda_sample_proj_ln, 15},
    {"tt_sca_reduce_ln", thunk_tt_sca_reduce_ln, 7},
    {"tt_dec_merge_in", thunk_tt_dec_merge_in, 9},
    {"tt_lidar_voxelize", thunk_tt_lidar_voxelize, 14},
    {"tt_lidar_voxelize_capped", thunk_tt_lidar_voxelize_capped, 15},
    {"tt_sp_volume_build", thunk_tt_sp_volume_build, 6},
    {"tt_sp_strided_outputs", thunk_tt_sp_strided_outputs, 12},
    {"tt_sp_rulebook", thunk_tt_sp_rulebook, 7},
    {"tt_sp_tile_plan", thunk_tt_sp_tile_plan, 9},
    {"tt_sp_to_dense", thunk_tt_sp_to_dense, 8},
    {"tt_preprocess_images", thunk_tt_preprocess_images, 18},
    {"tt_preprocess_images_ida", thunk_tt_preprocess_images_ida, 17},
    {"tt_preprocess_labels_ida", thunk_tt_preprocess_labels_ida, 11},
    {"tt_photometric_u8", thunk_tt_photometric_u8, 10},
    {"tt_preprocess_images_ida_aug", thunk_tt_preprocess_images_ida_aug, 21},
    {"tt_decode_depth_u8", thunk_tt_decode_depth_u8, 3},
    {"tt_rgb2hsv_u8", thunk_tt_rgb2hsv_u8, 4},
    {"tt_decode_seg_u8", thunk_tt_decode_seg_u8, 11},
    {"tt_decode_seg_u8_phases", thunk_tt_decode_seg_u8_phases, 12},
    {"tt_png_decode_u8", thunk_tt_png_decode_u8, 10},
    {"tt_png_decode_u8_phases", thunk_tt_png_decode_u8_phases, 11},
    {"tt_checksum_ranges_u8", thunk_tt_checksum_ranges_u8, 10},
    {"tt_png_decode_u8_verified", thunk_tt_png_decode_u8_verified, 14},
    {"tt_grad_norm_clip", thunk_tt_grad_norm_clip, 5},
    {"tt_adamw_step", thunk_tt_adamw_step, 12},
    {"tt_adamw_step_dev", thunk_tt_adamw_step_dev, 12},
    {"tt_adamw_advance", thunk_tt_adamw_advance, 2},
    {"tt_grad_gather", thunk_tt_grad_gather, 5},
    {"tt_loss_smooth_l1", thunk_tt_loss_smooth_l1, 10},
    {"tt_loss_smooth_l1_bwd", thunk_tt_loss_smooth_l1_bwd, 8},
    {"tt_loss_beta_kl_bwd", thunk_tt_loss_beta_kl_bwd, 10},
    {"tt_loss_beta_kl", thunk_tt_loss_beta_kl, 10},
    {"tt_loss_l1_cols", thunk_tt_loss_l1_cols, 9},
    {"tt_loss_seg_focal", thunk_tt_loss_seg_focal, 10},
    {"tt_loss_seg_focal_bwd", thunk_tt_loss_seg_focal_bwd, 11},
    {"tt_loss_depth_bce", thunk_tt_loss_depth_bce, 12},
    {"tt_loss_depth_bce_bwd", thunk_tt_loss_depth_bce_bwd, 13},
    {"tt_conv2d_wgrad", thunk_tt_conv2d_wgrad, 23},
    {"tt_conv2d_wgrad_x3", thunk_tt_conv2d_wgrad_x3, 23},
    {"tt_conv_epilogue_bwd", thunk_tt_conv_epilogue_bwd, 35},
    {"tt_gather_conv_wgrad", thunk_tt_gather_conv_wgrad, 15},
    {"tt_sp_inverse_rulebook", thunk_tt_sp_inverse_rulebook, 5},
    {"tt_sp_from_dense", thunk_tt_sp_from_dense, 9},
    {"tt_maxpool3x3s2_bwd", thunk_tt_maxpool3x3s2_bwd, 7},
    {"tt_upsample_nearest_add_bwd", thunk_tt_upsample_nearest_add_bwd, 8},
    {"tt_bilinear_up2_bwd", thunk_tt_bilinear_up2_bwd, 6},
    {"tt_channel_gate_bwd", thunk_tt_channel_gate_bwd, 10},
    {"tt_spatial_meanmax_bwd", thunk_tt_spatial_meanmax_bwd, 6},
    {"tt_spatial_mean_bwd", thunk_tt_spatial_mean_bwd, 7},
    {"tt_ew_bwd", thunk_tt_ew_bwd, 28},
    {"tt_look_gather_query_bwd", thunk_tt_look_gather_query_bwd, 11},
    {"tt_msda_sample_bwd", thunk_tt_msda_sample_bwd, 12},
    {"tt_sca_reduce_bwd", thunk_tt_sca_reduce_bwd, 4},
    {"tt_layernorm_rows_bwd", thunk_tt_layernorm_rows_bwd, 14},
    {"tt_concat_piece_bwd", thunk_tt_concat_piece_bwd, 10},
    {"tt_broadcast_rows_bwd", thunk_tt_broadcast_rows_bwd, 8},
    {"tt_lift_splat_bwd", thunk_tt_lift_splat_bwd, 17},
    {"tt_deform_im2col3x3_bwd", thunk_tt_deform_im2col3x3_bwd, 11},
    {"tt_lidar_merge_half_sweeps", thunk_tt_lidar_merge_half_sweeps, 7},
    {"tt_lidar_union_sweeps", thunk_tt_lidar_union_sweeps, 7},
    {"tt_bn_stats", thunk_tt_bn_stats, 10},
    {"tt_bn_finalize", thunk_tt_bn_finalize, 13},
    {"tt_bn_apply", thunk_tt_bn_apply, 20},
    {"tt_bn_bwd_reduce", thunk_tt_bn_bwd_reduce, 25},
    {"tt_bn_bwd_apply", thunk_tt_bn_bwd_apply, 18},
    {"tt_dropout_fwd", thunk_tt_dropout_fwd, 7},
    {"tt_dropout_bwd", thunk_tt_dropout_bwd, 5},
    {"tt_action_post", thunk_tt_action_post, 10},
    {"tt_fill_u32", thunk_tt_fill_u32, 3},
    {"tt_copy_bytes", thunk_tt_copy_bytes, 3},
};
```

thinktwice_amd/layers.py:

```python
import torch

from . import _lib, ops, weights

ACT = {"none": _lib.ACT_NONE, "relu": _lib.ACT_RELU, "sigmoid": _lib.ACT_SIGMOID, "gelu": _lib.ACT_GELU,
       "softplus": _lib.ACT_SOFTPLUS}


BN_TRAIN = False
BN_GROUPS = 1


class bn_groups:

    def __init__(self, n):
        self.n = n

    def __enter__(self):
        global BN_GROUPS
        self.saved, BN_GROUPS = BN_GROUPS, self.n

    def __exit__(self, *exc):
        global BN_GROUPS
        BN_GROUPS = self.saved
        return False


def _bn_spec(sd, bn, device, eps, momentum):
    return ops.BNSpec(bn, _dev(sd[bn + ".weight"], device), _dev(sd[bn + ".bias"], device),
                      _dev(sd[bn + ".running_mean"], device), _dev(sd[bn + ".running_var"], device), eps, momentum)


class Conv:
    def __init__(self, w, scale, shift, stride=1, pad=0, dil=1, act="none", pixel_shuffle2=False, x3=False, bn=None,
                 bias=None, h2=False):
        self.w, self.scale, self.shift = w, scale, shift
        self.bn, self.bias = bn, bias
        self.w_x3 = weights.split_pairs_x3(w) if x3 else None
        self.w_h2 = None
        if h2:
            self.w_h2 = weights.split_pairs_h2(w)
            self.w = w.to(torch.float16)
        self.stride, self.pad, self.dil = stride, pad, dil
        self.act = ACT[act]
        self.ps2 = pixel_shuffle2
        self.cin = w.shape[-1]

    def __call__(self, x, **kw):
        if BN_TRAIN and self.bn is not None:
            return self._bn_train(x, **kw)
        return ops.conv2d(x, self.w, stride=self.stride, pad=self.pad, dil=self.dil, scale=self.scale,
                          shift=self.shift, act=self.act, pixel_shuffle2=self.ps2, w_x3=self.w_x3, w_h2=self.w_h2, **kw)

    def _bn_train(self, x, res1=None, res1_coff=0, res2=None, res2_coff=0, out=None, out_coff=0, out_dtype=None, **kw):
        z = ops.conv2d(x, self.w, stride=self.stride, pad=self.pad, dil=self.dil, scale=None, shift=self.bias, act=0,
                       pixel_shuffle2=self.ps2, w_x3=self.w_x3, out_dtype=torch.float32, bn_raw=True, **kw)
        return ops.batchnorm_train(z, self.bn, self.act, res1=res1, res1_coff=res1_coff, res2=res2, res2_coff=res2_coff,
                                   out=out, out_coff=out_coff, groups=BN_GROUPS)


def _dev(t, device):
    return None if t is None else t.to(device=device, dtype=torch.float32).contiguous()


def conv_from_sd(sd, name, dtype, device, bn=None, eps=1e-5, stride=1, pad=0, dil=1, act="none",
                 cin_pad=None, weight=None, cin_lo=0, bn_momentum=0.1):
    w = sd[name + ".weight"] if weight is None else weight
    bias = sd.get(name + ".bias")
    h2 = isinstance(dtype, str) and dtype == weights.H2
    wq = weights.prep_conv_weight(w.to(device), torch.float32 if h2 else dtype, cin_pad)
    if bn is not None:
        scale, shift = weights.fold_bn(sd[bn + ".weight"], sd[bn + ".bias"], sd[bn + ".running_mean"],
                                       sd[bn + ".running_var"], eps, bias)
    else:
        scale, shift = None, bias
    from . import autodiff
    full = sd[name + ".weight"]
    autodiff.CONV_META[wq] = autodiff.ConvMeta(
        name, w.shape[1], bn,
        None if bn is None else _dev(sd[bn + ".running_mean"], device),
        None if bn is None else torch.sqrt(_dev(sd[bn + ".running_var"], device) + eps), _dev(bias, device),
        kind="conv" if weight is None else "cin_slice", full_shape=tuple(full.shape), lo=cin_lo)
    if bn is not None:
        autodiff.CONV_META[wq].scale_ref = _dev(scale, device)
    return Conv(wq, _dev(scale, device), _dev(shift, device), stride, pad, dil, act, x3=weights.is_x3(dtype),
                bn=None if bn is None else _bn_spec(sd, bn, device, eps, bn_momentum), bias=_dev(bias, device), h2=h2)


def conv_from_weight(w, dtype, scale=None, shift=None, **kw):
    return Conv(w, scale, shift, x3=weights.is_x3(dtype), **kw)


def linear_from_sd(sd, name, device, act="none", in_pad=None, dtype=torch.float32, bn=None, eps=1e-5, bn_momentum=0.1):
    w = sd[name + ".weight"]
    wq = weights.prep_linear_weight(w.to(device), dtype, in_pad)
    bias = sd.get(name + ".bias")
    if bn is not None:
        scale, shift = weights.fold_bn(sd[bn + ".weight"], sd[bn + ".bias"], sd[bn + ".running_mean"],
                                       sd[bn + ".running_var"], eps, bias)
    else:
        scale, shift = None, bias
    from . import autodiff
    autodiff.CONV_META[wq] = autodiff.ConvMeta(
        name, w.shape[1], bn,
        None if bn is None else _dev(sd[bn + ".running_mean"], device),
        None if bn is None else torch.sqrt(_dev(sd[bn + ".running_var"], device) + eps), _dev(bias, device),
        kind="linear")
    return Conv(wq, _dev(scale, device), _dev(shift, device), act=act, x3=weights.is_x3(dtype),
                bn=None if bn is None else _bn_spec(sd, bn, device, eps, bn_momentum), bias=_dev(bias, device))


def deconv2x2_from_sd(sd, name, dtype, device, bn=None, eps=1e-5, act="none", bn_momentum=0.1):
    wq = weights.prep_deconv2x2_weight(sd[name + ".weight"].to(device), dtype)
    bias = sd.get(name + ".bias")
    from . import autodiff
    autodiff.CONV_META[wq] = autodiff.ConvMeta(
        name, sd[name + ".weight"].shape[0], bn,
        None if bn is None else _dev(sd[bn + ".running_mean"], device),
        None if bn is None else torch.sqrt(_dev(sd[bn + ".running_var"], device) + eps), _dev(bias, device))
    if bn is not None:
        scale, shift = weights.fold_bn(sd[bn + ".weight"], sd[bn + ".bias"], sd[bn + ".running_mean"],
                                       sd[bn + ".running_var"], eps, bias)
    else:
        scale, shift = None, bias
    return Conv(wq, _dev(scale, device), _dev(shift, device), act=act, pixel_shuffle2=True, x3=weights.is_x3(dtype),
                bn=None if bn is None else _bn_spec(sd, bn, device, eps, bn_momentum), bias=_dev(bias, device))


def rows(x):
    return x.view(x.shape[0], 1, 1, x.shape[1])


def unrows(x):
    return x.view(x.shape[0], x.shape[-1])


class BNAffine:

    def __init__(self, scale, shift, spec):
        self.scale, self.shift, self.spec = scale, shift, spec

    def __getitem__(self, i):
        return (self.scale, self.shift)[i]

    def __call__(self, x, act=0, out=None, running_updates=1):
        if BN_TRAIN:
            if running_updates == 1:
                return ops.batchnorm_train(x.contiguous(), self.spec, act, out=out)
            import copy
            spec = copy.copy(self.spec)
            spec.momentum = 1.0 - (1.0 - float(self.spec.momentum)) ** int(running_updates)
            return ops.batchnorm_train(x.contiguous(), spec, act, out=out)
        return ops.affine_rows(x, self.scale, self.shift, act=act, out=out)


def bn_affine(sd, bn, device, eps=1e-5, momentum=0.1):
    s, t = weights.fold_bn(sd[bn + ".weight"], sd[bn + ".bias"], sd[bn + ".running_mean"],
                           sd[bn + ".running_var"], eps)
    s, t = _dev(s, device), _dev(t, device)
    from . import autodiff
    autodiff.AFFINE_META[s] = (bn, _dev(sd[bn + ".running_mean"], device),
                                   torch.sqrt(_dev(sd[bn + ".running_var"], device) + eps))
    return BNAffine(s, t, _bn_spec(sd, bn, device, eps, momentum))
```

thinktwice_amd/lss.py:

```python
import os

import torch

from . import _lib, camera, layers, ops, weights
from .layers import conv_from_sd, conv_from_weight, deconv2x2_from_sd, linear_from_sd, rows, unrows
from .registry import BACKBONES, NECKS, build_neck


class _ResNet50:

    def __init__(self, sd, p, dtype, device):
        vec = weights.vec_of(dtype)
        self.cin_pad = vec
        self.stem = conv_from_sd(sd, p + ".conv1", dtype, device, bn=p + ".bn1", stride=2, pad=3, act="relu",
                                 cin_pad=vec)
        self.stem_rr, self.stem_rr_x3 = None, None
        if weights.storage_dtype(dtype) != torch.float32:
            w = sd[p + ".conv1.weight"].to(device)
            wr = torch.zeros(w.shape[0], 7, 1, 64, dtype=dtype, device=device)
            wr[:, :, 0, :56] = torch.nn.functional.pad(w.permute(0, 2, 3, 1), (0, 5)).reshape(w.shape[0], 7, 56).to(dtype)
            self.stem_rr = wr.contiguous()
        elif dtype == weights.X3 and os.environ.get("TT_X3_STEM_ROWRUN", "1") == "1":
            w = sd[p + ".conv1.weight"].to(device).float()
            wr = torch.zeros(w.shape[0], 7, 1, 32, dtype=torch.float32, device=device)
            wr[:, :, 0, :28] = torch.nn.functional.pad(w.permute(0, 2, 3, 1), (0, 1)).reshape(w.shape[0], 7, 28)
            self.stem_rr = wr.contiguous()
            self.stem_rr_x3 = weights.split_pairs_x3(self.stem_rr)
        self.blocks = []
        for li, nb in enumerate((3, 4, 6, 3), start=1):
            stage = []
            for b in range(nb):
                q = f"{p}.layer{li}.{b}"
                s = 2 if (b == 0 and li > 1) else 1
                blk = {
                    "c1": conv_from_sd(sd, q + ".conv1", dtype, device, bn=q + ".bn1", act="relu"),
                    "c2": conv_from_sd(sd, q + ".conv2", dtype, device, bn=q + ".bn2", stride=s, pad=1, act="relu"),
                    "c3": conv_from_sd(sd, q + ".conv3", dtype, device, bn=q + ".bn3", act="relu"),
                    "ds": conv_from_sd(sd, q + ".downsample.0", dtype, device, bn=q + ".downsample.1", stride=s)
                    if b == 0 else None,
                }
                stage.append(blk)
            self.blocks.append(stage)

    def stem_border(self):
        return (3, 3, 3, 5) if self.stem_rr is not None else None

    def __call__(self, x, bordered=False):
        if bordered:
            NI, Hp, Wp, _ = x.shape
            if layers.BN_TRAIN:
                z = ops.conv2d(x, self.stem_rr, stride=2, pad=0, act=0, in_cstride=self.cin_pad,
                               out_hw=((Hp - 6) // 2, (Wp - 8) // 2), w_x3=self.stem_rr_x3, out_dtype=torch.float32)
                y = ops.batchnorm_train(z, self.stem.bn, self.stem.act, groups=layers.BN_GROUPS)
            else:
                y = ops.conv2d(x, self.stem_rr, stride=2, pad=0, scale=self.stem.scale, shift=self.stem.shift,
                               act=self.stem.act, in_cstride=self.cin_pad, out_hw=((Hp - 6) // 2, (Wp - 8) // 2),
                               w_x3=self.stem_rr_x3)
        else:
            y = self.stem(x, stop_grad=True)
        x = ops.maxpool3x3s2(y)
        outs = []
        for stage in self.blocks:
            for blk in stage:
                idt = blk["ds"](x) if blk["ds"] is not None else x
                c2 = blk["c2"]
                rows2 = x.shape[0] * (x.shape[1] // c2.stride) * (x.shape[2] // c2.stride)
                pr = (c2.w_x3 is not None and not layers.BN_TRAIN and
                      ops.pair_ok(min(rows2, x.shape[0] * x.shape[1] * x.shape[2]), c2.w.shape[-1], c2.w.shape[0]))
                y = c2(blk["c1"](x, out_pair=pr), in_pair=pr)
                x = blk["c3"](y, res1=idt)
            outs.append(x)
        return outs


@NECKS.register_module(name="PAFPN")
@NECKS.register_module()
class PAFPN_fp32:

    def __init__(self, in_channels, out_channels, num_outs, start_level=0, end_level=-1, add_extra_convs=False,
                 dtype=torch.float32, device="cuda", **unused):
        assert start_level == 0 and end_level in (-1, len(in_channels)) and not add_extra_convs and \
            num_outs == len(in_channels), "PAFPN: only the thinktwice.py form (all levels, no extra convs) is built"
        self.in_channels, self.out_channels, self.num_outs = list(in_channels), out_channels, num_outs
        self.half = isinstance(dtype, str) and dtype == weights.X3H
        self.wdtype, self.device = (weights.X3 if self.half else dtype), torch.device(device)
        self.loaded = False

    def load_state_dict(self, sd, prefix):
        n, dt, dev, L = prefix, self.wdtype, self.device, self.num_outs
        self.lat = [conv_from_sd(sd, f"{n}.lateral_convs.{i}.conv", dt, dev) for i in range(L)]
        self.fpn = [conv_from_sd(sd, f"{n}.fpn_convs.{i}.conv", dt, dev, pad=1) for i in range(L)]
        self.down = [conv_from_sd(sd, f"{n}.downsample_convs.{i}.conv", dt, dev, stride=2, pad=1) for i in range(L - 1)]
        self.paf = [conv_from_sd(sd, f"{n}.pafpn_convs.{i}.conv", dt, dev, pad=1) for i in range(L - 1)]
        if self.half:
            assert self.out_channels % 64 == 0, "half-storage PAFPN: out_channels must be a multiple of 64"
            h2 = weights.H2
            self.fpn_h = [conv_from_sd(sd, f"{n}.fpn_convs.{i}.conv", h2, dev, pad=1) for i in range(L)]
            self.down_h = [conv_from_sd(sd, f"{n}.downsample_convs.{i}.conv", h2, dev, stride=2, pad=1) for i in range(L - 1)]
            self.paf_h = [conv_from_sd(sd, f"{n}.pafpn_convs.{i}.conv", h2, dev, pad=1) for i in range(L - 1)]
        self.loaded = True
        return self

    def _call_half(self, inputs, targets):
        L, C, f16, f32 = self.num_outs, self.out_channels, torch.float16, torch.float32
        dev = inputs[0].device
        rows = [t.shape[0] * t.shape[1] * t.shape[2] for t in inputs]
        half = [r > 4096 for r in rows]
        lat32, lat16 = [None] * L, [None] * L
        for i in range(L - 1, -1, -1):
            n, h, w, _ = inputs[i].shape
            up = dict(res1=lat32[i + 1], res1_up=True) if i < L - 1 else {}
            if half[i]:
                lat32[i] = torch.empty(n, h, w, C, dtype=f32, device=dev)
                lat16[i] = self.lat[i](inputs[i], out_dtype=f16, out2=lat32[i], **up)
            else:
                lat32[i] = self.lat[i](inputs[i])
                if i < L - 1:
                    ops.upsample_nearest_add_(lat32[i], lat32[i + 1])
        if targets[0] is not None:
            buf0, off0 = targets[0]
        else:
            buf0, off0 = torch.empty(inputs[0].shape[0], inputs[0].shape[1], inputs[0].shape[2], C, dtype=f32, device=dev), 0
        inter32, inter16 = [None] * L, [None] * L
        if half[0]:
            inter16[0] = self.fpn_h[0](lat16[0], out2=buf0, out2_coff=off0)
        else:
            self.fpn[0](lat32[0], out=buf0, out_coff=off0)
        for i in range(1, L):
            inter32[i] = self.fpn_h[i](lat16[i], out_dtype=f32) if half[i] else self.fpn[i](lat32[i])
        for i in range(L - 1):
            if half[i]:
                src = inter16[i]
                if half[i + 1]:
                    inter16[i + 1] = self.down_h[i](src, res1=inter32[i + 1], out_dtype=f16)
                    inter32[i + 1] = None
                else:
                    self.down_h[i](src, res1=inter32[i + 1], out=inter32[i + 1])
            elif i == 0:
                self.down[0](buf0, in_coff=off0, cin=C, res1=inter32[1], out=inter32[1])
            else:
                self.down[i](inter32[i], res1=inter32[i + 1], out=inter32[i + 1])
        outs = [(buf0, off0, C)]
        for i in range(1, L):
            conv, src = (self.paf_h[i - 1], inter16[i]) if half[i] else (self.paf[i - 1], inter32[i])
            if targets[i] is not None:
                buf, off = targets[i]
                conv(src, out=buf, out_coff=off)
            else:
                buf, off = conv(src, out_dtype=f32), 0
            outs.append((buf, off, C))
        return outs

    def __call__(self, inputs, targets=None):
        L = self.num_outs
        assert len(inputs) == len(self.in_channels)
        targets = list(targets) if targets is not None else [None] * L
        C = self.out_channels
        if self.half:
            from . import autodiff
            if autodiff.TAPE is not None or layers.BN_TRAIN:
                raise _lib.TTError("PAFPN: the half-storage mode ('f32x3h') is an inference mode; train in 'f32x3' or float32")
            return self._call_half(inputs, targets)
        from . import autodiff
        lat = [None] * L
        lat[L - 1] = self.lat[L - 1](inputs[L - 1])
        for i in range(L - 2, -1, -1):
            n, h, w, _ = inputs[i].shape
            if autodiff.TAPE is None and not layers.BN_TRAIN and n * h * w > 4096 and inputs[i].dtype == torch.float32:
                lat[i] = self.lat[i](inputs[i], res1=lat[i + 1], res1_up=True)
            else:
                lat[i] = self.lat[i](inputs[i])
                ops.upsample_nearest_add_(lat[i], lat[i + 1])
        if targets[0] is not None:
            buf0, off0 = targets[0]
            self.fpn[0](lat[0], out=buf0, out_coff=off0)
        else:
            buf0, off0 = self.fpn[0](lat[0]), 0
        inter = [None] + [self.fpn[i](lat[i]) for i in range(1, L)]
        if L > 1:
            self.down[0](buf0, in_coff=off0, cin=C, res1=inter[1], out=inter[1])
        for i in range(1, L - 1):
            self.down[i](inter[i], res1=inter[i + 1], out=inter[i + 1])
        outs = [(buf0, off0, C)]
        for i in range(1, L):
            if targets[i] is not None:
                buf, off = targets[i]
                self.paf[i - 1](inter[i], out=buf, out_coff=off)
            else:
                buf, off = self.paf[i - 1](inter[i]), 0
            outs.append((buf, off, C))
        return outs


@BACKBONES.register_module()
class LSS:
    def __init__(self, x_bound, y_bound, z_bound, d_bound, final_dim, downsample_factor, output_channels,
                 img_backbone_conf=None, img_neck_conf=None, depth_net_conf=None, seg_net_conf=None,
                 queue_len=1, fpn_in_channels=(64, 128, 256, 512), dtype=torch.float32, device="cuda"):
        self.grid = camera.VoxelGrid(x_bound, y_bound, z_bound)
        self.d_bound = d_bound
        self.final_dim = tuple(final_dim)
        self.downsample_factor = downsample_factor
        self.output_channels = output_channels
        self.queue_len = queue_len
        self.img_neck_conf = dict(img_neck_conf) if img_neck_conf else dict(type="PAFPN", in_channels=[256, 512, 1024, 2048],
                                                                              num_outs=4, out_channels=256)
        self.half_neck = isinstance(dtype, str) and dtype == weights.X3H
        if self.half_neck:
            dtype = weights.X3
        self.wdtype = dtype
        self.dtype = weights.storage_dtype(dtype)
        self.device = torch.device(device)
        self.frustum = camera.make_frustum(self.final_dim, downsample_factor, d_bound)
        self.depth_channels = self.frustum.shape[0]
        self.voxel_num = self.grid.voxel_num
        self._frustum_dev = None
        self.loaded = False
        self._xpad = {}

    def load_state_dict(self, sd, prefix="img_encoder"):
        dt, dev, p = self.wdtype, self.device, prefix
        f32 = torch.float32
        self.backbone = _ResNet50(sd, p + ".img_backbone", dt, dev)
        self.img_neck = build_neck(self.img_neck_conf, dtype=weights.X3H if self.half_neck else dt,
# ... 255 lines not shown
```

thinktwice_amd/ops.py:

```python
import ctypes
import os

import torch

from . import _lib
from ._lib import (TT_BF16, TT_F16, TT_F32, TTError, check, clear_device_faults, cur_stream, device_faults, lib, ptr,
                   raise_on_device_fault, require_cuda)


def dtype_code(t):
    if t.dtype == torch.float32:
        return TT_F32
    if t.dtype == torch.bfloat16:
        return TT_BF16
    if t.dtype == torch.float16:
        return TT_F16
    raise _lib.TTError(f"unsupported dtype {t.dtype}")


def frustum_voxel_index(frustum, mats, voxel_lo, voxel_size, batch_size, num_cams, want_f32=False):
    require_cuda(frustum, mats)
    assert frustum.is_contiguous() and mats.is_contiguous()
    D, fH, fW, _ = frustum.shape
    geom = torch.empty(batch_size, num_cams * D * fH * fW, 3, dtype=torch.int32, device=frustum.device)
    gf = torch.empty(geom.shape, dtype=torch.float32, device=frustum.device) if want_f32 else None
    lo = (ctypes.c_float * 3)(*[float(v) for v in voxel_lo])
    sz = (ctypes.c_float * 3)(*[float(v) for v in voxel_size])
    rc = lib().tt_frustum_voxel_index(batch_size, num_cams, D, fH, fW, ptr(frustum), ptr(mats), lo, sz, ptr(geom), ptr(gf),
                                      cur_stream(frustum.device))
    check(rc, "tt_frustum_voxel_index")
    return (geom, gf) if want_f32 else geom


_LIFT_SPLAT_ATOMIC = os.environ.get("TT_LIFT_SPLAT_ATOMIC", "0") == "1"


def lift_splat(depth_logits, context, geom_xyz, voxel_num, batch_size, num_cams, out=None,
               out_coff=0, rot_flip=False, record=True):
    require_cuda(depth_logits, context, geom_xyz)
    assert depth_logits.is_contiguous() and context.is_contiguous() and geom_xyz.is_contiguous()
    BN, fH, fW, D = depth_logits.shape
    C = context.shape[-1]
    vx, vy, vz = (int(v) for v in voxel_num)
    if out is None:
        oh, ow = (vx, vy) if rot_flip else (vy, vx)
        out = torch.zeros(batch_size, oh, ow, C, dtype=torch.float32, device=context.device)
    ws, ws_bytes = None, 0
    if not _LIFT_SPLAT_ATOMIC:
        ws_bytes = int(lib().tt_lift_splat_workspace_bytes(batch_size, num_cams, D, fH, fW, C, vx, vy))
        if ws_bytes > 0:
            ws = torch.empty(ws_bytes, dtype=torch.uint8, device=context.device)
    rc = lib().tt_lift_splat_fwd_ws(batch_size, num_cams, D, fH, fW, C, vx, vy, vz, ptr(depth_logits), ptr(context),
                                    dtype_code(context), ptr(geom_xyz), ptr(out), out.shape[-1], out_coff, 1 if rot_flip else 0,
                                    ptr(ws), ws_bytes, cur_stream(context.device))
    check(rc, "tt_lift_splat_fwd_ws")
    if record:
        from . import autodiff
        if autodiff.TAPE is not None:
            autodiff.TAPE.lift_splat(depth_logits, context, geom_xyz, (vx, vy, vz), batch_size, num_cams, out, out_coff,
                                     rot_flip)
    return out


def lift_splat_bwd(depth_logits, context, geom_xyz, voxel_num, batch_size, num_cams, gout, out_coff, gdepth, gctx):
    require_cuda(depth_logits, context, geom_xyz, gout, gdepth, gctx)
    BN, fH, fW, D = depth_logits.shape
    C = context.shape[-1]
    vx, vy, vz = voxel_num
    assert all(t.is_contiguous() and t.dtype == torch.float32 for t in (depth_logits, context, gout, gdepth, gctx))
    check(lib().tt_lift_splat_bwd(batch_size, num_cams, D, fH, fW, C, vx, vy, vz,
                                  ptr(depth_logits), ptr(context), ptr(geom_xyz), ptr(gout), gout.shape[-1],
                                  out_coff, ptr(gdepth), ptr(gctx), cur_stream(context.device)), "tt_lift_splat_bwd")


_AUTO_SPLITK = os.environ.get("TT_CONV_AUTO_SPLITK", "1") == "1"
CONV_PROFILE = None
CONV_KERNELS = None
CONV_BYTES = None

_ConvDesc = _lib.structs()["tt_conv_desc"]


def _last_conv_kernel():
    L = lib()
    return L.tt_conv_last_kernel().decode()


SPARSE_PAIRS = None


def sp_tile_plan(nbr, m_dev):
    require_cuda(nbr, m_dev)
    M, KV = nbr.shape
    ws_bytes = int(lib().tt_sp_tile_plan_workspace_bytes(M))
    ws = torch.empty(ws_bytes, dtype=torch.uint8, device=nbr.device)
    perm = torch.empty(M, dtype=torch.int32, device=nbr.device)
    mask = torch.empty(M, dtype=torch.int32, device=nbr.device)
    check(lib().tt_sp_tile_plan(ptr(nbr), ptr(m_dev), M, KV, ptr(ws), ws_bytes, ptr(perm), ptr(mask),
                                ptr(SPARSE_PAIRS), cur_stream(nbr.device)), "tt_sp_tile_plan")
    return perm, mask


def gather_conv(feats, nbr, m_dev, w, *, scale=None, shift=None, act=0, res=None, out_dtype=None, w_x3=None, plan=None,
                out=None, in_rows=None, stride=1, _no_tape=False, bn_raw=False):
    require_cuda(feats, nbr, w)
    M, taps = nbr.shape
    Cout, _, KW, Cin = w.shape
    assert KW == taps and feats.shape[1] == Cin and feats.is_contiguous() and nbr.is_contiguous()
    if out is None:
        out = torch.empty(M, Cout, dtype=out_dtype or feats.dtype, device=feats.device)
    assert tuple(out.shape) == (M, Cout) and out.is_contiguous()
    d = _ConvDesc()
    d.in_ = feats.data_ptr(); d.N = M; d.H = 1; d.W = 1; d.Cin = Cin; d.in_cstride = Cin; d.in_coff = 0
    d.in_nstride = 0
    d.weight = w.data_ptr(); d.Cout = Cout; d.KH = 1; d.KW = KW; d.stride = stride; d.pad = 0; d.dil = 1
    d.out = out.data_ptr(); d.OH = 1; d.OW = 1; d.out_cstride = Cout; d.out_coff = 0; d.out_nstride = 0
    d.scale = ptr(scale); d.shift = ptr(shift)
    d.res1 = ptr(res); d.res1_cstride = 0 if res is None else res.shape[-1]
    d.act = act; d.dtype = dtype_code(feats); d.out_dtype = dtype_code(out)
    d.gather_idx = nbr.data_ptr(); d.m_dev = ptr(m_dev)
    d.weight_x3 = ptr(w_x3)
    if plan is not None:
        d.row_perm, d.row_mask = plan[0].data_ptr(), plan[1].data_ptr()
    if CONV_PROFILE is not None:
        e0, e1 = torch.cuda.Event(enable_timing=True), torch.cuda.Event(enable_timing=True)
        e0.record()
    check(lib().tt_conv2d_fwd(ctypes.byref(d), cur_stream(feats.device)), "tt_conv2d_fwd(gather)")
    if CONV_PROFILE is not None:
        e1.record()
        CONV_PROFILE.append((2.0 * Cout * KW * Cin, e0, e1, f"sparse M<={M} N={Cout} K={KW * Cin}", m_dev, M,
                             ((nbr >= 0).sum(1), 2.0 * Cout * Cin)))
        if CONV_KERNELS is not None:
            CONV_KERNELS.append(_last_conv_kernel())
        if CONV_BYTES is not None:
            esz, osz = feats.element_size(), out.element_size()
            CONV_BYTES.append((Cin * esz + Cout * osz + (Cout * esz if res is not None else 0) + KW * 4,
                               w.numel() * w.element_size()))
    if not _no_tape:
        from . import autodiff
        if autodiff.TAPE is not None:
            autodiff.TAPE.gather_conv(feats, nbr, m_dev, w, scale, shift, act, res, out, in_rows, bn_raw)
    return out


def gather_conv_wgrad(feats, nbr, m_dev, dy, taps, cin_pad=None):
    require_cuda(feats, nbr, dy)
    M, Cout = dy.shape
    Cin = feats.shape[1]
    cin_pad = cin_pad or Cin
    out = torch.empty(Cout, 1, taps, cin_pad, dtype=torch.float32, device=dy.device)
    L = lib()
    nb = int(L.tt_gather_conv_wgrad_workspace_bytes(M, Cout, Cin, cin_pad, taps))
    ws = torch.empty(nb, dtype=torch.uint8, device=dy.device)
    assert feats.is_contiguous() and dy.is_contiguous() and nbr.is_contiguous() and feats.dtype == torch.float32
    check(L.tt_gather_conv_wgrad(ptr(feats), Cin, Cin, ptr(nbr), ptr(m_dev), M, taps, ptr(dy), Cout,
                                 Cout, cin_pad, 0, ptr(out), ptr(ws), nb, _st(dy)), "tt_gather_conv_wgrad")
    if CONV_KERNELS is not None:
        label = ctypes.create_string_buffer(192)
        check(L.tt_gather_conv_wgrad_plan(ptr(feats), Cin, Cin, ptr(nbr), ptr(m_dev), M, taps, ptr(dy), Cout, Cout, cin_pad, 0,
                                          ptr(out), ptr(ws), nb, 0, label, len(label)), "tt_gather_conv_wgrad_plan")
        CONV_KERNELS.append(label.value.decode())
    return out


def sp_inverse_rulebook(nbr, m_dev, rows_in):
    M, taps = nbr.shape
    inv = torch.full((rows_in, taps), -1, dtype=torch.int32, device=nbr.device)
    check(lib().tt_sp_inverse_rulebook(ptr(nbr), ptr(m_dev), M, taps, ptr(inv), _st(nbr)), "tt_sp_inverse_rulebook")
    return inv


def sp_to_dense(x, coords, rows, max_rows, dims, batch_size):
    D, H, W = dims
    C = x.shape[1]
    dense = torch.zeros(batch_size, H, W, C * D, dtype=x.dtype, device=x.device)
    dc = (ctypes.c_int * 3)(*dims)
    check(lib().tt_sp_to_dense(ptr(x), ptr(coords), ptr(rows), max_rows, C, dc, ptr(dense), dtype_code(x),
                               cur_stream(x.device)), "tt_sp_to_dense")
    from . import autodiff
    if autodiff.TAPE is not None:
        autodiff.TAPE.sp_to_dense(x, coords, rows, max_rows, dims, dense)
    return dense


def sp_from_dense(gdense, coords, rows, max_rows, dims, grows):
    D, H, W = dims
    C = grows.shape[1]
    check(lib().tt_sp_from_dense(ptr(gdense), ptr(coords), ptr(rows), max_rows, C, D, H, W,
                                 ptr(grows), cur_stream(grows.device)), "tt_sp_from_dense")


def conv2d(x, w, *, stride=1, pad=0, dil=1, scale=None, shift=None, act=0, res1=None, res1_coff=0,
           res2=None, res2_coff=0, out=None, out_coff=0, in_coff=0, cin=None, pixel_shuffle2=False,
           shift_n=None, shift_n_mod=1, out_dtype=None, out_nstride=0, out_hw=None, splitk_ws=None,
           in_cstride=None, w_x3=None, _no_tape=False, stop_grad=False, bn_raw=False, in_pair=False, out_pair=False,
           w_h2=None, out2=None, out2_coff=0, res1_up=False, in_up2=False):
    require_cuda(x, w)
    assert w.is_contiguous() and x.dim() == 4 and w.dim() == 4
    N, H, W, Cs = x.shape
    assert x.stride(3) == 1 and (W == 1 or x.stride(2) == Cs) and (H == 1 or x.stride(1) == W * Cs), x.stride()
    src_px = N * H * W
    if in_up2:
        assert x.dtype == torch.float32 and x.is_contiguous() and w_x3 is not None and not in_pair and splitk_ws is None
        H, W = 2 * H, 2 * W
    Cout, KH, KW, Cin = w.shape
    if cin is None:
        cin = Cin
    assert cin == Cin, (cin, Cin)
    OH = (H + 2 * pad - dil * (KH - 1) - 1) // stride + 1
    OW = (W + 2 * pad - dil * (KW - 1) - 1) // stride + 1
    if out_hw is not None:
        OH, OW = out_hw
    cr = Cout // 4 if pixel_shuffle2 else Cout
    if out is None:
        odt = out_dtype or x.dtype
        oh, ow = (2 * OH, 2 * OW) if pixel_shuffle2 else (OH, OW)
        out = torch.empty(N, oh, ow, cr, dtype=odt, device=x.device)
    d = _ConvDesc()
    d.in_ = x.data_ptr(); d.N = N; d.H = H; d.W = W; d.Cin = Cin; d.in_cstride = in_cstride or Cs; d.in_coff = in_coff
    d.in_nstride = x.stride(0) if N > 1 else 0
    d.weight = w.data_ptr(); d.Cout = Cout; d.KH = KH; d.KW = KW; d.stride = stride; d.pad = pad; d.dil = dil
    d.out = out.data_ptr(); d.OH = OH; d.OW = OW
    d.out_cstride = out.shape[-1]; d.out_coff = out_coff
    d.out_nstride = out_nstride or (out.stride(0) if (out.dim() == 4 and N > 1) else 0)
    d.pixel_shuffle2 = 1 if pixel_shuffle2 else 0
    d.scale = ptr(scale); d.shift = ptr(shift); d.shift_n = ptr(shift_n); d.shift_n_mod = shift_n_mod
    d.res1 = ptr(res1); d.res1_cstride = 0 if res1 is None else res1.shape[-1]; d.res1_coff = res1_coff
    if res1 is not None and res1.dtype == torch.float32 and x.dtype != torch.float32:
        d.res1_f32 = 1
    if res1_up:
        assert res1 is not None and res1.dim() == 4 and res1.is_contiguous() and res1.shape[0] == N and splitk_ws is None
        d.res1_up_h, d.res1_up_w = res1.shape[1], res1.shape[2]
    d.res2 = ptr(res2); d.res2_cstride = 0 if res2 is None else res2.shape[-1]; d.res2_coff = res2_coff
    d.act = act; d.dtype = dtype_code(x); d.out_dtype = dtype_code(out)
    from . import autodiff
    if w_h2 is not None:
        assert x.dtype == torch.float16 and w.dtype == torch.float16 and w_h2.dtype == torch.float16 and w_h2.is_contiguous() \
            and w_h2.numel() == 2 * w.numel() and w_x3 is None and splitk_ws is None
        if autodiff.TAPE is not None:
            raise _lib.TTError("conv2d: half-storage (h2) layers have no backward; train in dtype torch.float32 or 'f32x3'")
        d.weight_h2 = w_h2.data_ptr()
    if out2 is not None:
        assert out2.dtype == torch.float32 and out2.numel() // out2.shape[-1] == N * OH * OW and out2.stride(-1) == 1
        d.out2 = out2.data_ptr(); d.out2_cstride = out2.shape[-1]; d.out2_coff = out2_coff
    if in_pair or out_pair:
        assert w_x3 is not None and x.dtype == torch.float32 and out.dtype == torch.float32 and splitk_ws is None
        if autodiff.TAPE is not None:
            raise _lib.TTError("conv2d: pair-format activations are an inference-path layout (the tape reads f32 tensors)")
        d.in_pair, d.out_pair = int(bool(in_pair)), int(bool(out_pair))
    if in_up2:
        if autodiff.TAPE is not None:
            raise _lib.TTError("conv2d: in_up2 is an inference-path fusion (the tape records bilinear_up2 and the convolution apart)")
        d.in_up2 = 1
    if w_x3 is not None and Cout < 64 and (autodiff.TAPE is not None or _no_tape):
        w_x3 = None
    if w_x3 is not None:
        assert x.dtype == torch.float32 and w_x3.shape == w.shape and w_x3.is_contiguous()
        x3_splitk = autodiff.TAPE is None and not _no_tape
        if x3_splitk:
            d.weight_x3 = w_x3.data_ptr()
    if _AUTO_SPLITK and splitk_ws is None and not (in_pair or out_pair or in_up2) and w_h2 is None and not res1_up and N * OH * OW <= 4096 and KH * KW * Cin >= 2048:
        slices = int(lib().tt_conv2d_splitk_slices(ctypes.byref(d)))
        if slices > 0:
            splitk_ws = torch.empty(slices, N * OH * OW, Cout, dtype=torch.float32, device=x.device)
            d.splitk_slices = slices
    if splitk_ws is not None:
        d.splitk_ws = splitk_ws.data_ptr()
    elif w_x3 is not None:
        d.weight_x3 = w_x3.data_ptr()
    if CONV_PROFILE is not None:
        e0, e1 = torch.cuda.Event(enable_timing=True), torch.cuda.Event(enable_timing=True)
        e0.record()
    rc = lib().tt_conv2d_fwd(ctypes.byref(d), cur_stream(x.device))
    check(rc, "tt_conv2d_fwd")
    if CONV_PROFILE is not None:
        e1.record()
        CONV_PROFILE.append((2.0 * N * OH * OW * Cout * KH * KW * Cin, e0, e1,
                             f"M={N * OH * OW} N={Cout} K={KH * KW * Cin} k{KH}x{KW}s{stride}"))
        if CONV_KERNELS is not None:
            CONV_KERNELS.append(_last_conv_kernel())
        if CONV_BYTES is not None:
            esz, osz = x.element_size(), out.element_size()
            m_out = N * OH * OW
            in_px = min(src_px, m_out * KH * KW)
            wsz = w.numel() * w.element_size() * (2 if w_h2 is not None else 1)
            CONV_BYTES.append(in_px * (in_cstride or Cin) * esz + m_out * Cout * osz + wsz +
                              m_out * Cout * esz * ((res1 is not None) + (res2 is not None)) +
                              (m_out * Cout * 4 if out2 is not None else 0))
    if not _no_tape:
        from . import autodiff
        if autodiff.TAPE is not None:
            autodiff.TAPE.conv(x, w, out, stride, pad, dil, scale, shift, act, in_coff, cin, out_coff, res1, res1_coff,
                               res2, res2_coff, pixel_shuffle2, in_cstride, shift_n, shift_n_mod, stop_grad, bn_raw)
    return out


SEG_CHAIN = os.environ.get("TT_SEG_CHAIN", "1") != "0"


def seg_feedback_chain(x, cv1, cv2, out=None, out_coff=0):
    require_cuda(x, cv1.w, cv2.w)
    assert x.dtype == torch.float32 and x.is_contiguous() and x.dim() == 4
    assert cv2.w_x3 is not None and cv1.w.dtype == torch.float32 and cv2.w.dtype == torch.float32
    N, H, W, Cs = x.shape
    n1, kh1, kw1, k1 = cv1.w.shape
    n2, kh2, kw2, k2 = cv2.w.shape
    assert (kh1, kw1, kh2, kw2) == (1, 1, 1, 1) and k1 == Cs and k2 == n1 == 64, (cv1.w.shape, cv2.w.shape, Cs)
    assert (cv1.stride, cv1.pad, cv2.stride, cv2.pad) == (1, 0, 1, 0) and not cv1.ps2 and not cv2.ps2
    if out is None:
        out = torch.empty(N, H, W, n2, dtype=torch.float32, device=x.device)
    assert out.dtype == torch.float32 and out.is_contiguous() and out.numel() // out.shape[-1] == N * H * W
    R = N * H * W
    if CONV_PROFILE is not None:
        e0, e1 = torch.cuda.Event(enable_timing=True), torch.cuda.Event(enable_timing=True)
        e0.record()
    check(lib().tt_seg_feedback_chain(ptr(x), R, Cs, k1, ptr(cv1.w), ptr(cv1.scale), ptr(cv1.shift), cv1.act, ptr(cv2.w),
                                      ptr(cv2.w_x3), n2, ptr(cv2.scale), ptr(cv2.shift), cv2.act, ptr(out), out.shape[-1],
                                      out_coff, cur_stream(x.device)), "tt_seg_feedback_chain")
    if CONV_PROFILE is not None:
        e1.record()
        CONV_PROFILE.append((2.0 * R * (k1 * n1 + k2 * n2), e0, e1, f"M={R} N={n1}->{n2} K={k1} chain k1x1s1"))
        if CONV_KERNELS is not None:
            CONV_KERNELS.append("seg_chain_kernel")
        if CONV_BYTES is not None:
            CONV_BYTES.append(R * (Cs + n2) * 4 + (cv1.w.numel() + cv2.w.numel()) * 4)
    return out


def _st(t):
    return cur_stream(t.device)


BN_SYNC = True
DROPOUT_MASKS = None
DROPOUT_SEED = [0x5EED, 0]


def _all_reduce_sum_(t):
    import torch.distributed as dist
    if not (BN_SYNC and dist.is_available() and dist.is_initialized()) or dist.get_world_size() == 1:
        return t
    if t.is_cuda and dist.get_backend() == "gloo":
        h = t.cpu()
        dist.all_reduce(h, op=dist.ReduceOp.SUM)
        t.copy_(h)
    else:
        dist.all_reduce(t, op=dist.ReduceOp.SUM)
    return t


class BNSpec:

    def __init__(self, name, gamma, beta, running_mean, running_var, eps=1e-5, momentum=0.1):
        self.name, self.gamma, self.beta, self.running_mean, self.running_var = name, gamma, beta, running_mean, running_var
        self.eps, self.momentum = float(eps), float(momentum)


def _bn_ws(C, groups, dev):
    L = lib()
    nb = int(L.tt_bn_workspace_bytes(C, groups))
    return torch.empty(nb, dtype=torch.uint8, device=dev), nb


def batchnorm_train(z, spec, act=0, res1=None, res1_coff=0, res2=None, res2_coff=0, out=None, out_coff=0, m_dev=None,
                    groups=1, update_running=True):
    require_cuda(z)
    assert z.dtype == torch.float32 and z.is_contiguous()
    C = z.shape[-1]
    M = z.numel() // C
    dev = z.device
    if out is None:
        out = torch.empty_like(z)
    assert out.is_contiguous() and out.dtype == torch.float32 and out.numel() // out.shape[-1] == M, (out.shape, z.shape)
    for r in (res1, res2):
        assert r is None or (r.is_contiguous() and r.dtype == torch.float32 and r.numel() // r.shape[-1] == M)
    stats = torch.empty(groups, 2 * C + 2, dtype=torch.float64, device=dev)
    ws, nb = _bn_ws(C, groups, dev)
    st = _st(z)
    L = lib()
    check(L.tt_bn_stats(ptr(z), M, C, C, 0, ptr(m_dev), groups, ptr(stats), ptr(ws), nb, st), "tt_bn_stats")
    _all_reduce_sum_(stats)
    scale, shift, mean, invstd = (torch.empty(groups, C, dtype=torch.float32, device=dev) for _ in range(4))
    check(L.tt_bn_finalize(ptr(stats), C, groups, ptr(spec.gamma), ptr(spec.beta), spec.eps, spec.momentum,
                           ptr(spec.running_mean if update_running else None),
                           ptr(spec.running_var if update_running else None), ptr(scale), ptr(shift), ptr(mean), ptr(invstd),
                           st), "tt_bn_finalize")

    def cs(t):
        return 0 if t is None else t.shape[-1]
    check(L.tt_bn_apply(ptr(z), M, C, C, 0, ptr(m_dev), groups, ptr(scale), ptr(shift), ptr(mean), ptr(res1), cs(res1),
                        res1_coff, ptr(res2), cs(res2), res2_coff, act, ptr(out), out.shape[-1], out_coff, st), "tt_bn_apply")
    from . import autodiff
    if autodiff.TAPE is not None:
        autodiff.TAPE.bn_train(z, out, out_coff, spec, act, res1, res1_coff, res2, res2_coff, m_dev, groups, stats, scale,
                               mean, invstd)
    return out


def batchnorm_train_bwd(dy, dy_coff, y, y_coff, z, mean, invstd, scale, stats, act, dres1, dres1_coff, dres2, dres2_coff, dz,
                        m_dev=None, groups=1):
    C = z.shape[-1]
    M = z.numel() // C
    dev = z.device
    sums = torch.empty(groups, 2 * C, dtype=torch.float64, device=dev)
    ws, nb = _bn_ws(C, groups, dev)
    st = _st(z)
    L = lib()

    def cs(t):
        return 0 if t is None else t.shape[-1]
    check(L.tt_bn_bwd_reduce(ptr(dy), dy.shape[-1], dy_coff, ptr(y), y.shape[-1], y_coff, ptr(z), C, 0,
                             M, C, ptr(m_dev), groups, ptr(mean), ptr(invstd), act, ptr(dres1), cs(dres1),
                             dres1_coff, ptr(dres2), cs(dres2), dres2_coff, ptr(sums), ptr(ws), nb, st), "tt_bn_bwd_reduce")
    local = sums.sum(0).to(torch.float32)
    _all_reduce_sum_(sums)
    check(L.tt_bn_bwd_apply(ptr(dy), dy.shape[-1], dy_coff, ptr(z), C, 0, M, C, ptr(m_dev), groups,
                            ptr(sums), ptr(stats), ptr(scale), ptr(mean), ptr(invstd), ptr(dz), dz.shape[-1], 0, st),
          "tt_bn_bwd_apply")
    return local[C:].contiguous(), local[:C].contiguous()


def dropout(x, p=0.5):
    require_cuda(x)
    assert x.dtype == torch.float32 and x.is_contiguous()
    out = torch.empty_like(x)
    mask = torch.empty(x.numel(), dtype=torch.uint8, device=x.device)
    mask_in = None
    if DROPOUT_MASKS is not None:
        mask_in = next(DROPOUT_MASKS).to(device=x.device, dtype=torch.uint8).contiguous()
        assert mask_in.numel() == x.numel()
    DROPOUT_SEED[1] += 1
    seed = (DROPOUT_SEED[0] * 0x100000001B3 + DROPOUT_SEED[1] * 0x9E3779B97F4A7C15) & 0xFFFFFFFFFFFFFFFF
    check(lib().tt_dropout_fwd(ptr(x), ptr(out), x.numel(), p, seed, ptr(mask_in), ptr(mask), _st(x)), "tt_dropout_fwd")
    from . import autodiff
    if autodiff.TAPE is not None:
        autodiff.TAPE.dropout(x, out, mask, p)
    return out


def dropout_bwd(dout, mask, dx, p):
    assert dout.is_contiguous() and dx.is_contiguous()
    check(lib().tt_dropout_bwd(ptr(dout), ptr(mask), ptr(dx), dout.numel(), p, _st(dout)), "tt_dropout_bwd")


def nchw_to_nhwc_border(x, out, top, left):
    require_cuda(x, out)
    assert x.is_contiguous() and x.dtype == torch.float32 and out.is_contiguous()
    N, C, H, W = x.shape
    _, Hp, Wp, Cp = out.shape
    check(lib().tt_nchw_to_nhwc_border(ptr(x), ptr(out), N, C, H, W, Cp, Hp, Wp,
                                       top, left, dtype_code(out), _st(x)), "tt_nchw_to_nhwc_border")
    return out


def nchw_to_nhwc_pad(x, dtype, c_pad):
    require_cuda(x)
    assert x.is_contiguous() and x.dtype == torch.float32
    N, C, H, W = x.shape
    out = torch.empty(N, H, W, c_pad, dtype=dtype, device=x.device)
    check(lib().tt_nchw_to_nhwc_pad(ptr(x), ptr(out), N, C, H, W, c_pad, dtype_code(out), _st(x)), "tt_nchw_to_nhwc_pad")
    return out


def nhwc_to_nchw(x, C=None, coff=0):
    require_cuda(x)
    N, H, W, Cs = x.shape
    C = C or Cs
    out = torch.empty(N, C, H, W, dtype=torch.float32, device=x.device)
    check(lib().tt_nhwc_to_nchw(ptr(x), ptr(out), N, C, H, W, Cs, coff, dtype_code(x), _st(x)), "tt_nhwc_to_nchw")
    return out


def maxpool3x3s2(x):
    N, H, W, C = x.shape
    out = torch.empty(N, (H + 2 - 3) // 2 + 1, (W + 2 - 3) // 2 + 1, C, dtype=x.dtype, device=x.device)
    check(lib().tt_maxpool3x3s2(ptr(x), ptr(out), N, H, W, C, dtype_code(x), _st(x)), "tt_maxpool3x3s2")
    from . import autodiff
    if autodiff.TAPE is not None:
        autodiff.TAPE.maxpool3x3s2(x, out)
    return out


def upsample_nearest_add_(dst, src):
    N, H, W, C = dst.shape
    check(lib().tt_upsample_nearest_add(ptr(dst), ptr(src), N, H, W, C, src.shape[1],
                                        src.shape[2], dtype_code(dst), _st(dst)), "tt_upsample_nearest_add")
    from . import autodiff
    if autodiff.TAPE is not None:
        autodiff.TAPE.upsample_nearest_add_(dst, src)
    return dst


PAIR = os.environ.get("TT_X3_PAIR", "1") != "0"


def pair_ok(rows, cin=32, cout=64, taps=9):
    from . import autodiff
    return (PAIR and autodiff.TAPE is None and rows > 4096 and cin % 32 == 0 and taps * cin >= 64 and
            (8 <= cout <= 32 or cout >= 64))


SEG_UP2 = os.environ.get("TT_SEG_UP2", "1") != "0"


def up2_ok(rows, cin, cout):
    from . import autodiff
    return autodiff.TAPE is None and rows > 4096 and cin % 32 == 0 and cout == 64


def bilinear_up2(x, out_pair=False):
    N, H, W, C = x.shape
    out = torch.empty(N, 2 * H, 2 * W, C, dtype=x.dtype, device=x.device)
    if out_pair:
        assert x.dtype == torch.float32 and x.is_contiguous() and C % 16 == 0
        check(lib().tt_bilinear_up2_pair(ptr(x), ptr(out), N, H, W, C, _st(x)), "tt_bilinear_up2_pair")
        return out
    check(lib().tt_bilinear_up2(ptr(x), ptr(out), N, H, W, C, dtype_code(x), _st(x)), "tt_bilinear_up2")
    from . import autodiff
    if autodiff.TAPE is not None:
        autodiff.TAPE.bilinear_up2(x, out)
    return out


def spatial_pool(x, mode, C=None, coff=0):
    N, H, W, Cs = x.shape
    C = C or Cs
    out = torch.empty(N, C, dtype=torch.float32, device=x.device)
    check(lib().tt_spatial_pool(ptr(x), ptr(out), N, H * W, C, Cs, coff, mode, dtype_code(x), _st(x)), "tt_spatial_pool")
    from . import autodiff
    if autodiff.TAPE is not None:
        autodiff.TAPE.spatial_pool(x, out, mode, C, coff)
    return out


def channel_gate(x, gate, res=None, gate_act=_lib.ACT_SIGMOID, out_act=_lib.ACT_NONE, out=None):
    N, H, W, C = x.shape
    assert gate.dtype == torch.float32 and gate.shape == (N, C) and gate.is_contiguous()
    out = torch.empty_like(x) if out is None else out
    check(lib().tt_channel_gate(ptr(x), ptr(gate), ptr(res), ptr(out), N, H * W, C, gate_act,
                                out_act, dtype_code(x), _st(x)), "tt_channel_gate")
    from . import autodiff
    if autodiff.TAPE is not None:
        autodiff.TAPE.channel_gate(x, gate, res, out, gate_act, out_act)
    return out


def affine_rows(x, scale, shift, act=0, out=None):
    R, C = x.shape
    out = torch.empty(R, C, dtype=x.dtype, device=x.device) if out is None else out
    check(lib().tt_affine_rows(ptr(x), ptr(scale), ptr(shift), ptr(out), R, C, x.stride(0),
                               out.stride(0), act, dtype_code(x), _st(x)), "tt_affine_rows")
    from . import autodiff
    if autodiff.TAPE is not None:
        autodiff.TAPE.affine_rows(x, scale, shift, act, out)
    return out


def layernorm_rows(x, gamma, beta, eps=1e-5, out=None, D=None):
    R = x.shape[0]
    D = D or x.shape[1]
    out = torch.zeros(R, x.shape[1], dtype=x.dtype, device=x.device) if out is None else out
    check(lib().tt_layernorm_rows(ptr(x), ptr(gamma), ptr(beta), ptr(out), R, D, x.stride(0),
                                  out.stride(0), eps, dtype_code(x), _st(x)), "tt_layernorm_rows")
    from . import autodiff
    if autodiff.TAPE is not None:
        autodiff.TAPE.layernorm_rows(x, gamma, beta, out, D, eps)
    return out


def layernorm_rows_bwd(x, gamma, dout, dx, dgamma, dbeta, D, eps=1e-5):
    R = x.shape[0]
    L = lib()
    nb = int(L.tt_layernorm_rows_bwd_workspace_bytes(R, D))
    ws = torch.empty(nb, dtype=torch.uint8, device=x.device)
    check(L.tt_layernorm_rows_bwd(ptr(x), ptr(gamma), ptr(dout), ptr(dx), ptr(dgamma), ptr(dbeta), R, D,
                                  x.stride(0), dout.stride(0), dx.stride(0), eps, ptr(ws), nb, _st(x)), "tt_layernorm_rows_bwd")


def concat_piece_bwd(dout, coff, C, div, mod, dsrc):
    R = dout.shape[0]
    check(lib().tt_concat_piece_bwd(ptr(dout), dout.stride(0), coff, R, C, div, mod, ptr(dsrc),
                                    dsrc.stride(0), dsrc.shape[0], _st(dout)), "tt_concat_piece_bwd")


def copy_nhwc(x, out, C=None, in_coff=0, out_coff=0, rot_flip=False):
    N, H, W, Cs = x.shape
    C = C or Cs
    check(lib().tt_copy_nhwc(ptr(x), ptr(out), N, H, W, C, Cs, in_coff, out.shape[-1], out_coff, 1 if rot_flip else 0,
                             dtype_code(x), dtype_code(out), _st(x)), "tt_copy_nhwc")
    from . import autodiff
    if autodiff.TAPE is not None:
        autodiff.TAPE.copy_nhwc(x, out, C, in_coff, out_coff, rot_flip)
    return out


def broadcast_rows(v, out, out_coff=0):
    N, C = v.shape
    _, H, W, Ct = out.shape
    check(lib().tt_broadcast_rows(ptr(v), ptr(out), N, H * W, C, v.stride(0), Ct,
                                  out_coff, dtype_code(out), _st(out)), "tt_broadcast_rows")
    from . import autodiff
    if autodiff.TAPE is not None:
        autodiff.TAPE.broadcast_rows(v, out, out_coff)
    return out


def ew(op, a, b=None, g=None, out=None, C=None, a_coff=0, b_coff=0, g_coff=0, out_coff=0, act=0):
    a2 = a.reshape(-1, a.shape[-1])
    R = a2.shape[0]
    C = C or a2.shape[1]
    if out is None:
        out = torch.empty(R, C, dtype=a.dtype, device=a.device)
    o2 = out.reshape(-1, out.shape[-1])
    assert o2.data_ptr() == out.data_ptr() and o2.stride(1) == 1, "ew: `out` must be viewable as rows"
    b2 = None if b is None else b.reshape(-1, b.shape[-1])
    g2 = None if g is None else g.reshape(-1, g.shape[-1])
    check(lib().tt_ew(ptr(a2), ptr(b2), ptr(g2), ptr(o2), R, C, a2.stride(0), a_coff,
                      0 if b2 is None else b2.stride(0), b_coff, 0 if g2 is None else g2.stride(0),
                      g_coff, o2.stride(0), out_coff, op, act, dtype_code(a), _st(a)), "tt_ew")
    from . import autodiff
    if autodiff.TAPE is not None:
        autodiff.TAPE.ew(op, act, R, C, a2, a_coff, b2, b_coff, g2, g_coff, o2, out_coff)
    return out


def ew_bwd(op, act, R, C, a2, a_coff, b2, b_coff, g2, g_coff, o2, out_coff, dout, da, db, dg):
    def st(t):
        return 0 if t is None else t.stride(0)
    check(lib().tt_ew_bwd(op, act, R, C, ptr(a2), st(a2), a_coff, ptr(b2), st(b2), b_coff, ptr(g2), st(g2), g_coff, ptr(o2),
                          st(o2), out_coff, ptr(dout), st(dout), out_coff, ptr(da), st(da), a_coff, ptr(db), st(db), b_coff,
                          ptr(dg), st(dg), g_coff, _st(a2)), "tt_ew_bwd")


def concat_rows(out, pieces, coff=0):
    o2 = out.reshape(-1, out.shape[-1])
    assert o2.data_ptr() == out.data_ptr() and o2.dtype == torch.float32 and 1 <= len(pieces) <= 8
    assert o2.stride(1) == 1, "concat_rows: `out` rows must be element-contiguous"
    n = len(pieces)
    srcs = (ctypes.c_void_p * n)()
    strides, widths, coffs, divs, mods = ((ctypes.c_int * n)() for _ in range(5))
    c = coff
    for i, (src, C, div, mod) in enumerate(pieces):
        if src is not None:
            s2 = src.reshape(-1, src.shape[-1])
            assert s2.dtype == torch.float32 and s2.stride(1) == 1 and s2.shape[1] >= C
            need = mod if mod else -(-o2.shape[0] // div)
            assert s2.shape[0] >= need, f"concat_rows: piece {i} has {s2.shape[0]} rows, mapping reads {need}"
            srcs[i], strides[i] = s2.data_ptr(), s2.stride(0)
        else:
            srcs[i], strides[i] = None, 0
        widths[i], coffs[i], divs[i], mods[i] = C, c, div, mod
        c += C
# ... 505 lines not shown
```

Baseline: 111.9 frames/s.

## Fuse bottleneck c3 conv with next block's c1 conv in joined bf16x3 kernel

After: 113.9 frames/s (median of 6 runs). +1.8%, better.

```diff
diff --git a/include/thinktwice_hip.h b/include/thinktwice_hip.h
--- a/include/thinktwice_hip.h
+++ b/include/thinktwice_hip.h
@@ -112,9 +112,20 @@
     int in_up2;
 } tt_conv_desc;
 
+typedef struct tt_conv_next {
+    const void* next_weight; const void* next_weight_x3;
+    int next_cout;
+    const float* next_scale; const float* next_shift;
+    int next_act;
+    void* next_out; int next_out_cstride, next_out_coff;
+    int next_out_pair;
+} tt_conv_next;
+
 int tt_conv2d_fwd(const tt_conv_desc* d, void* stream);
+int tt_conv2d_fwd_next(const tt_conv_desc* d, const tt_conv_next* next, void* stream);
 int tt_conv2d_splitk_slices(const tt_conv_desc* d);
 int tt_conv2d_plan(const tt_conv_desc* d, char* label, int label_bytes);
+int tt_conv2d_plan_next(const tt_conv_desc* d, const tt_conv_next* next, char* label, int label_bytes);
 
 int tt_seg_feedback_chain(const float* x, long long R, int x_stride, int K1, const float* w1, const float* scale1,
                           const float* shift1, int act1, const float* w2, const void* w2_x3, int N2, const float* scale2,
diff --git a/thinktwice_amd/build.py b/thinktwice_amd/build.py
--- a/thinktwice_amd/build.py
+++ b/thinktwice_amd/build.py
@@ -15,7 +15,7 @@
 
 
 EXTRA_FLAGS = {"conv_x3_pipe.hip": ["-fno-slp-vectorize"], "conv_x3_up2.hip": ["-fno-slp-vectorize"],
-               "conv_x3_patch.hip": ["-fno-slp-vectorize"]}
+               "conv_x3_patch.hip": ["-fno-slp-vectorize"], "conv_x3_join.hip": ["-fno-slp-vectorize"]}
 
 
 def _sources():
diff --git a/thinktwice_amd/csrc/conv_choose.cpp b/thinktwice_amd/csrc/conv_choose.cpp
--- a/thinktwice_amd/csrc/conv_choose.cpp
+++ b/thinktwice_amd/csrc/conv_choose.cpp
@@ -175,6 +175,47 @@
     return 0;
 }
 
+int choose_join(const ConvArgs& a, const ConvFacts& f, ConvChoice* c) {
+    const ConvArgs& n = *f.join;
+    TT_REQUIRE(f.dtype == TT_F32 && a.out_dtype == TT_F32 && f.weight_x3 && aligned16(f.weight_x3) && !f.weight_h2,
+               "tt_conv2d_fwd: next_out goes with a bf16x3 layer (dtype / out_dtype TT_F32, a 16-byte aligned weight_x3)");
+    TT_REQUIRE(f.join_weight_x3 && aligned16(f.join_weight_x3), "tt_conv2d_fwd: next_weight_x3 must be given and 16-byte aligned");
+    TT_REQUIRE(a.KH == 1 && a.KW == 1 && a.stride == 1 && a.pad == 0 && a.OH == a.H && a.OW == a.W,
+               "tt_conv2d_fwd: next_out needs a 1 x 1 / stride 1 / pad 0 layer (got k %d x %d s %d p %d)", a.KH, a.KW, a.stride, a.pad);
+    TT_REQUIRE(!a.gather && !a.m_dev && !a.ws && !a.pixel_shuffle2 && !a.res2 && !a.shift_n && !f.out2 && !f.res1_up && !(a.flags & (64 | 256)),
+               "tt_conv2d_fwd: next_out takes no res2, shift_n, out2, res1_up, out_pair, in_up2, splitk_ws, gather_idx or pixel_shuffle2");
+    TT_REQUIRE((a.Cin == 64 || a.Cin == 128 || a.Cin == 256) && a.Cout == 4 * a.Cin,
+               "tt_conv2d_fwd: next_out needs Cin = 64, 128 or 256 and Cout = 4 Cin (got Cin=%d Cout=%d)", a.Cin, a.Cout);
+    TT_REQUIRE(n.Cout == a.Cin || (n.Cout == 2 * a.Cin && a.Cin <= 128),
+               "tt_conv2d_fwd: next_cout = %d has no joined kernel beside Cin = %d (64 or 128 / 128 or 256 / 256)", n.Cout, a.Cin);
+    TT_REQUIRE(a.act == TT_ACT_NONE || a.act == TT_ACT_RELU, "tt_conv2d_fwd: next_out needs act none or ReLU (got %d)", a.act);
+    TT_REQUIRE(n.act == TT_ACT_NONE || n.act == TT_ACT_RELU, "tt_conv2d_fwd: next_act must be none or ReLU (got %d)", n.act);
+    TT_REQUIRE(a.M >= kJoinFloorRows, "tt_conv2d_fwd: next_out needs N*OH*OW of at least %d rows (got %d)", kJoinFloorRows, a.M);
+    TT_REQUIRE(a.in_nstride == (long long)a.H * a.W * a.in_cstride && (!(a.flags & 32) || (a.in_cstride % 16 == 0 && a.in_coff % 16 == 0)),
+               "tt_conv2d_fwd: next_out needs a row-linear `in` (in_nstride 0 or H*W*in_cstride; in_pair: in_cstride / in_coff multiples of 16)");
+    TT_REQUIRE(a.out_fast && a.vec_epi && a.res_vec, "tt_conv2d_fwd: next_out needs a row-linear `out` and 16-byte aligned out / res1 rows");
+    TT_REQUIRE((n.flags & 64) && n.out_fast && n.vec_epi,
+               "tt_conv2d_fwd: next_out_pair must be 1, with a row-linear next_out and next_cout / next_out_cstride / next_out_coff multiples of 16");
+    ConvFacts f1 = f, f2{};
+    f1.join = nullptr;
+    f1.join_weight_x3 = nullptr;
+    f2.dtype = TT_F32;
+    f2.weight_x3 = f.join_weight_x3;
+    ConvChoice s1, s2;
+    if (conv_choose(a, f1, &s1) || conv_choose(n, f2, &s2)) return -1;
+    auto same_sums = [](const ConvChoice& s) { return s.family == CONV_GLDS && s.x3 && !s.gather && s.splits <= 1; };
+    TT_REQUIRE(same_sums(s1), "tt_conv2d_fwd: next_out: this layer alone (M=%d Cin=%d Cout=%d) would not run on a bf16x3 LDS-DMA tile", a.M,
+               a.Cin, a.Cout);
+    TT_REQUIRE(same_sums(s2), "tt_conv2d_fwd: next_out: the next layer alone (M=%d %d -> next_cout=%d) would not run on a bf16x3 LDS-DMA tile",
+               n.M, n.Cin, n.Cout);
+    const int nw = (n.Cout == 256) ? 4 : 8;
+    set_tile(c, CONV_X3_JOIN, n.Cout, nw, 1, a.Cin * 4, 2);
+    c->x3 = true;
+    c->apair = (a.flags & 32) != 0;
+    c->below_min = a.M < kJoinMinRows;
+    return 0;
+}
+
 bool choose_glds(const ConvArgs& a, int dtype, ConvChoice* c) {
     constexpr int min_tiles = 2;
     if (a.gather) {
@@ -248,6 +289,7 @@
     *c = ConvChoice{};
     c->splits = 1;
     const bool ws = a.ws || f.assume_ws;
+    if (f.join) return choose_join(a, f, c);
     if (a.flags & 256) return choose_up2(a, f, c);
     if (f.weight_h2) {
         TT_REQUIRE(aligned16(f.weight_h2), "tt_conv2d_fwd: weight_h2 must be 16-byte aligned");
@@ -304,6 +346,7 @@
         case CONV_X3_RUN3: snprintf(out, bytes, "conv_x3_run3_kernel<%d>%s%s", c.bn, pre, tail); break;
         case CONV_X3_UP2: snprintf(out, bytes, "conv_x3_run3_kernel<%d, up2>", c.bn); break;
         case CONV_X3_PATCH: snprintf(out, bytes, "conv_x3_run3_kernel<%d, patch>%s", c.bn, pre); break;
+        case CONV_X3_JOIN: snprintf(out, bytes, "conv_x3_join_kernel<%d, %d, %d>%s%s", c.bkb / 4, c.bn, c.waves_m, pre, c.below_min ? " below kJoinMinRows" : ""); break;
         case CONV_GLDS:
             snprintf(out, bytes, "conv_igemm_glds_kernel<%s, %d, %d, %d, %d, %d, %s, %s>%s%s", tn, c.bn, c.waves_m, c.waves_n, c.bkb,
                      c.stages, c.gather ? "true" : "false", c.x3 ? "true" : "false", pre, c.splits > 1 ? " split-K" : tail);
diff --git a/thinktwice_amd/csrc/conv_choose.h b/thinktwice_amd/csrc/conv_choose.h
--- a/thinktwice_amd/csrc/conv_choose.h
+++ b/thinktwice_amd/csrc/conv_choose.h
@@ -52,6 +52,7 @@
     CONV_X3_RUN3,
     CONV_X3_UP2,
     CONV_X3_PATCH,
+    CONV_X3_JOIN,
     CONV_GLDS,
     CONV_IGEMM,
 };
@@ -60,12 +61,17 @@
 
 constexpr int kPatchMinRows = 16384;
 
+constexpr int kJoinFloorRows = 4097;
+constexpr int kJoinMinRows = 32768;
+
 struct ConvFacts {
     int dtype;
     const void* weight_x3;
     const void* weight_h2;
     bool out2, res1_up, res1_f32;
     bool assume_ws;
+    const ConvArgs* join;
+    const void* join_weight_x3;
 };
 
 struct ConvChoice {
@@ -76,6 +82,7 @@
     int main_rows;
     int splits;
     int slices;
+    bool below_min;
 };
 
 int conv_choose(const ConvArgs& a, const ConvFacts& f, ConvChoice* c);
diff --git a/thinktwice_amd/csrc/conv_common.h b/thinktwice_amd/csrc/conv_common.h
--- a/thinktwice_amd/csrc/conv_common.h
+++ b/thinktwice_amd/csrc/conv_common.h
@@ -387,5 +387,6 @@
 int launch_conv_glds(const ConvChoice& c, ConvArgs& a, int dtype, hipStream_t st);
 int launch_conv_x3_up2(const ConvChoice& c, ConvArgs& a, hipStream_t st);
 int launch_conv_x3_patch(const ConvChoice& c, ConvArgs& a, hipStream_t st);
-
-}
+int launch_conv_x3_join(const ConvChoice& c, ConvArgs& a, const ConvArgs& a2, hipStream_t st);
+
+}
diff --git a/thinktwice_amd/csrc/conv_igemm.hip b/thinktwice_amd/csrc/conv_igemm.hip
--- a/thinktwice_amd/csrc/conv_igemm.hip
+++ b/thinktwice_amd/csrc/conv_igemm.hip
@@ -269,7 +269,7 @@
 
 using namespace tt;
 
-static int conv2d_prepare(const tt_conv_desc* d, ConvArgs& a, ConvFacts& f) {
+static int conv2d_prepare(const tt_conv_desc* d, const tt_conv_next* n, ConvArgs& a, ConvFacts& f, ConvArgs& a2) {
     TT_REQUIRE(d && d->in && d->weight && d->out, "tt_conv2d_fwd: null pointer");
     TT_REQUIRE(d->dtype == TT_F32 || d->dtype == TT_BF16 || d->dtype == TT_F16, "tt_conv2d_fwd: bad dtype %d", d->dtype);
     TT_REQUIRE(d->out_dtype == TT_F32 || d->out_dtype == d->dtype ||
@@ -368,14 +368,45 @@
     f.res1_up = d->res1_up_w > 0;
     f.res1_f32 = d->res1_f32 != 0;
     f.assume_ws = false;
+    f.join = nullptr;
+    f.join_weight_x3 = nullptr;
+    if (n) {
+        TT_REQUIRE(n->next_out, "tt_conv2d_fwd_next: next_out is null");
+        TT_REQUIRE(n->next_weight && (reinterpret_cast<uintptr_t>(n->next_weight) & 15) == 0 && n->next_cout > 0,
+                   "tt_conv2d_fwd: next_out needs next_weight (16-byte aligned) and next_cout > 0");
+        TT_REQUIRE(n->next_out_cstride > 0 && n->next_out_coff >= 0 && n->next_out_coff + n->next_cout <= n->next_out_cstride,
+                   "tt_conv2d_fwd: next_out_cstride=%d / next_out_coff=%d do not hold next_cout=%d channels", n->next_out_cstride,
+                   n->next_out_coff, n->next_cout);
+        TT_REQUIRE(!n->next_out_pair || (n->next_cout % 16 == 0 && n->next_out_cstride % 16 == 0 && n->next_out_coff % 16 == 0 &&
+                                         (reinterpret_cast<uintptr_t>(n->next_out) & 63) == 0),
+                   "tt_conv2d_fwd: next_out_pair needs next_cout / next_out_cstride / next_out_coff multiples of 16 and a 64-byte aligned next_out");
+        a2 = ConvArgs{};
+        a2.in = d->out; a2.weight = n->next_weight; a2.out = n->next_out;
+        a2.scale = n->next_scale; a2.shift = n->next_shift;
+        a2.N = d->N; a2.H = d->OH; a2.W = d->OW; a2.Cin = d->Cout; a2.in_cstride = d->out_cstride; a2.in_coff = d->out_coff;
+        a2.in_nstride = a.out_nstride;
+        a2.Cout = n->next_cout; a2.KH = a2.KW = a2.stride = a2.dil = 1;
+        a2.OH = d->OH; a2.OW = d->OW; a2.out_cstride = n->next_out_cstride; a2.out_coff = n->next_out_coff;
+        a2.out_nstride = (long long)d->OH * d->OW * n->next_out_cstride;
+        a2.shift_n_mod = 1;
+        a2.act = n->next_act; a2.out_dtype = TT_F32;
+        a2.M = a.M; a2.K = d->Cout;
+        a2.out_fast = 1; a2.tiles_n = 1;
+        a2.vec_epi = (n->next_cout % 8 == 0 && n->next_out_cstride % 8 == 0 && n->next_out_coff % 8 == 0 &&
+                      (reinterpret_cast<uintptr_t>(n->next_out) & 15) == 0) ? 1 : 0;
+        a2.res_vec = 1;
+        a2.flags = 16 | (n->next_out_pair ? 64 : 0);
+        f.join = &a2;
+        f.join_weight_x3 = n->next_weight_x3;
+    }
     return 0;
 }
 
-extern "C" int tt_conv2d_fwd(const tt_conv_desc* d, void* stream) {
-    ConvArgs a;
+static int conv2d_run(const tt_conv_desc* d, const tt_conv_next* n, void* stream) {
+    ConvArgs a, a2;
     ConvFacts f;
     ConvChoice c;
-    if (const int r = conv2d_prepare(d, a, f)) return r;
+    if (const int r = conv2d_prepare(d, n, a, f, a2)) return r;
     if (const int r = conv_choose(a, f, &c)) return r;
     hipStream_t st = (hipStream_t)stream;
     const bool pair = d->in_pair || d->out_pair;
@@ -414,6 +445,11 @@
             what = "tt_conv2d_fwd(x3 patch, pair)";
             r = launch_conv_x3_patch(c, a, st);
             break;
+        case CONV_X3_JOIN:
+            what = "tt_conv2d_fwd(x3 join)";
+            a2.weight = n->next_weight_x3;
+            r = launch_conv_x3_join(c, a, a2, st);
+            break;
         case CONV_GLDS:
             what = !c.x3 ? "tt_conv2d_fwd(glds)" : c.splits > 1 ? "tt_conv2d_fwd(glds x3 split-K)" : pair ? "tt_conv2d_fwd(glds x3, pair)" : "tt_conv2d_fwd(glds x3)";
             if (c.splits > 1) a.ws_slices = c.slices;
@@ -436,24 +472,38 @@
     return check_launch(what);
 }
 
+extern "C" int tt_conv2d_fwd(const tt_conv_desc* d, void* stream) { return conv2d_run(d, nullptr, stream); }
+
+extern "C" int tt_conv2d_fwd_next(const tt_conv_desc* d, const tt_conv_next* next, void* stream) {
+    TT_REQUIRE(next, "tt_conv2d_fwd_next: null tt_conv_next");
+    return conv2d_run(d, next, stream);
+}
+
 extern "C" int tt_conv2d_splitk_slices(const tt_conv_desc* d) {
-    ConvArgs a;
+    ConvArgs a, a2;
     ConvFacts f;
     ConvChoice c;
-    if (conv2d_prepare(d, a, f)) return 0;
+    if (conv2d_prepare(d, nullptr, a, f, a2)) return 0;
     if (d->in_pair || d->out_pair || d->in_up2 || d->weight_h2 || d->res1_up_w > 0) return 0;
     f.assume_ws = true;
     if (conv_choose(a, f, &c)) return 0;
     return c.splits > 1 ? c.slices : 0;
 }
 
-extern "C" int tt_conv2d_plan(const tt_conv_desc* d, char* label, int label_bytes) {
-    ConvArgs a;
+static int conv2d_plan(const tt_conv_desc* d, const tt_conv_next* n, char* label, int label_bytes) {
+    ConvArgs a, a2;
     ConvFacts f;
     ConvChoice c;
-    if (const int r = conv2d_prepare(d, a, f)) return r;
+    if (const int r = conv2d_prepare(d, n, a, f, a2)) return r;
     if (const int r = conv_choose(a, f, &c)) return r;
     TT_REQUIRE(label && label_bytes > 0, "tt_conv2d_plan: no room for the label");
     conv_label(c, d->dtype, label, (size_t)label_bytes);
     return 0;
 }
+
+extern "C" int tt_conv2d_plan(const tt_conv_desc* d, char* label, int label_bytes) { return conv2d_plan(d, nullptr, label, label_bytes); }
+
+extern "C" int tt_conv2d_plan_next(const tt_conv_desc* d, const tt_conv_next* next, char* label, int label_bytes) {
+    TT_REQUIRE(next, "tt_conv2d_plan_next: null tt_conv_next");
+    return conv2d_plan(d, next, label, label_bytes);
+}
diff --git a/thinktwice_amd/csrc/conv_x3_join.hip b/thinktwice_amd/csrc/conv_x3_join.hip
--- /dev/null
+++ b/thinktwice_amd/csrc/conv_x3_join.hip
@@ -0,0 +1,272 @@
+#include <utility>
+
+#include "conv_lds_dma.h"
+
+namespace tt {
+namespace {
+
+__device__ __forceinline__ void lds_wait() { asm volatile("s_waitcnt lgkmcnt(0)" ::: "memory"); }
+__device__ __forceinline__ void pin(u32x4& v) { asm volatile("" : "+v"(v)); }
+template <int OFF>
+__device__ __forceinline__ u32x4 lds_read_at(unsigned addr) {
+    u32x4 v;
+    asm volatile("ds_read_b128 %0, %1 offset:%2" : "=v"(v) : "v"(addr), "n"(OFF) : "memory");
+    return v;
+}
+template <int OFF>
+__device__ __forceinline__ void lds_write_f32_at(unsigned addr, float v) {
+    asm volatile("ds_write_b32 %0, %1 offset:%2" ::"v"(addr), "v"(v), "n"(OFF) : "memory");
+}
+template <int OFF>
+__device__ __forceinline__ void lds_write4_at(unsigned addr, const u32x4& v) {
+    asm volatile("ds_write_b128 %0, %1 offset:%2\n\ts_nop 1" ::"v"(addr), "v"(v), "n"(OFF) : "memory");
+}
+
+constexpr int kJoinCB = 32;
+constexpr int kJoinLdc = kJoinCB + 4;
+constexpr int kJoinBlockBytes = 32 * kJoinLdc * 4;
+
+template <int... R>
+__device__ __forceinline__ void stage_block(unsigned addr, const f32x16& acc, float sc, float sh, std::integer_sequence<int, R...>) {
+    (lds_write_f32_at<((R & 3) + 8 * (R >> 2)) * kJoinLdc * 4>(addr, acc[R] * sc + sh), ...);
+}
+
+}
+
+template <int K1, int N2, int NW>
+__global__ __launch_bounds__(NW * 64, NW / 4) void conv_x3_join_kernel(const ConvArgs p, const void* , int ,
+                                                                       int , const ConvArgs p2) {
+#if defined(__HIP_DEVICE_COMPILE__)
+    constexpr int CB = kJoinCB, LDC = kJoinLdc;
+    constexpr int K2 = 4 * K1, NCB = K2 / CB, KS1 = K1 / 16, NJ = N2 / 32;
+    constexpr int P1 = K1 / 8, P2 = N2 / 8;
+    constexpr int PPW = (P1 + P2) / NW;
+    constexpr int TILE = (P1 + P2) * 1024;
+    static_assert((P1 + P2) % NW == 0 && K1 % 32 == 0 && (N2 == 64 || N2 == 128 || N2 == 256), "whole pieces per wave, whole 128-byte sub-tiles, column block pairs");
+
+    extern __shared__ __attribute__((aligned(16))) unsigned char smem[];
+    const int tid = threadIdx.x, lane = tid & 63;
+    const int wave = __builtin_amdgcn_readfirstlane(tid >> 6);
+    const int r = lane & 31, half = lane >> 5;
+    const int Mlim = p.M;
+    const int m0 = (int)blockIdx.x * (32 * NW);
+    const int mb = m0 + wave * 32;
+    const bool full = mb + 32 <= Mlim;
+    const unsigned lds_base = (unsigned)(uintptr_t)(__attribute__((address_space(3))) unsigned char*)smem;
+    const unsigned blk = lds_base + 2u * TILE + (unsigned)wave * kJoinBlockBytes;
+
+    uint4 ah[KS1], al[KS1];
+    {
+        const int m = mb + r;
+        const float* row = reinterpret_cast<const float*>(p.in) + (long long)(m < Mlim ? m : Mlim - 1) * p.in_cstride + p.in_coff;
+        if (p.flags & 32) {
+#pragma unroll
+            for (int ks = 0; ks < KS1; ++ks) {
+                ah[ks] = *reinterpret_cast<const uint4*>(row + ks * 16 + half * 4);
+                al[ks] = *reinterpret_cast<const uint4*>(row + ks * 16 + 8 + half * 4);
+            }
+        } else {
+#pragma unroll
+            for (int ks = 0; ks < KS1; ++ks) {
+                const uint4 r0 = *reinterpret_cast<const uint4*>(row + ks * 16 + half * 8);
+                const uint4 r1 = *reinterpret_cast<const uint4*>(row + ks * 16 + half * 8 + 4);
+                split8(r0, r1, ah[ks], al[ks]);
+            }
+        }
+    }
+
+    const float* dsrc[PPW];
+    int dstep[PPW];
+#pragma unroll
+    for (int j = 0; j < PPW; ++j) {
+        const int q = wave + NW * j;
+        if (q < P1) {
+            const int g = q * 64 + lane, t = g >> 8, row = (g & 255) >> 3, pos = g & 7;
+            dsrc[j] = reinterpret_cast<const float*>(p.weight) + (long long)row * K1 + t * 32 + ((pos ^ swz<128>(row)) << 2);
+            dstep[j] = CB * K1;
+        } else {
+            const int g = (q - P1) * 64 + lane, row = g >> 3, pos = g & 7;
+            dsrc[j] = reinterpret_cast<const float*>(p2.weight) + (long long)row * K2 + ((pos ^ swz<128>(row)) << 2);
+            dstep[j] = CB;
+        }
+    }
+    auto issue_tile = [&](int cb) {
+        const unsigned st = lds_base + (unsigned)(cb & 1) * TILE;
+#pragma unroll
+        for (int j = 0; j < PPW; ++j) {
+            dma_piece(dsrc[j], st + (unsigned)(wave + NW * j) * 1024u);
+            dsrc[j] += dstep[j];
+        }
+    };
+
+    const int prow = lane >> 3, pcol = (lane & 7) * 4;
+    const unsigned pass_addr = blk + (unsigned)(prow * LDC + pcol) * 4u;
+    const unsigned stage_addr = blk + (unsigned)(4 * half * LDC + r) * 4u;
+    const unsigned a_addr = blk + (unsigned)(r * LDC + half * 8) * 4u;
+    const bool has_res = p.res1 != nullptr, relu1 = p.act == TT_ACT_RELU;
+    float* const obase = reinterpret_cast<float*>(p.out) + (long long)mb * p.out_cstride + p.out_coff;
+    const float* const rbase = has_res ? reinterpret_cast<const float*>(p.res1) + (long long)mb * p.res1_cstride + p.res1_coff : nullptr;
+    int ooff[4], roff[4];
+    bool row_ok[4];
+#pragma unroll
+    for (int q = 0; q < 4; ++q) {
+        const int m = mb + q * 8 + prow;
+        row_ok[q] = m < Mlim;
+        const int dr = (row_ok[q] ? m : Mlim - 1) - mb;
+        ooff[q] = dr * p.out_cstride + pcol;
+        roff[q] = dr * p.res1_cstride + pcol;
+    }
+    float4 res[4];
+    float sc = 1.f, sh = 0.f;
+    auto load_epi = [&](int cb) {
+        sc = p.scale ? p.scale[cb * CB + r] : 1.f;
+        sh = p.shift ? p.shift[cb * CB + r] : 0.f;
+        if (has_res) {
+#pragma unroll
+            for (int q = 0; q < 4; ++q) res[q] = *reinterpret_cast<const float4*>(rbase + roff[q] + cb * CB);
+        }
+    };
+
+    const unsigned fo[2] = {frag_off<128>(r, (unsigned)half), frag_off<128>(r, 4u + (unsigned)half)};
+
+    f32x16 acc2[N2 / 64][1][2];
+#pragma unroll
+    for (int g = 0; g < N2 / 64; ++g) zero_acc(acc2[g]);
+
+    typedef float f4v __attribute__((ext_vector_type(4)));
+    issue_tile(0);
+    asm volatile("" ::: "memory");
+    load_epi(0);
+#pragma unroll
+    for (int ks = 0; ks < KS1; ++ks) {
+        asm volatile("" ::"v"(ah[ks].x), "v"(al[ks].x));
+    }
+#pragma unroll 1
+    for (int cb = 0; cb < NCB; ++cb) {
+        if (cb > 0 && full) wait_vmcnt<4>();
+        else wait_vmcnt<0>();
+        asm volatile("s_barrier" ::: "memory");
+        if (cb + 1 < NCB) issue_tile(cb + 1);
+        asm volatile("" ::: "memory");
+        const unsigned w1 = lds_base + (unsigned)(cb & 1) * TILE, w2 = w1 + P1 * 1024u;
+
+        f32x16 acc1;
+#pragma unroll
+        for (int e = 0; e < 16; ++e) acc1[e] = 0.f;
+        u32x4 bh[2], bl[2];
+        bh[0] = lds_read(w1 + fo[0]);
+        bl[0] = lds_read(w1 + (fo[0] ^ 32u));
+#pragma unroll
+        for (int ks = 0; ks < KS1; ++ks) {
+            const int b = ks & 1;
+            lds_wait();
+            pin(bh[b]);
+            pin(bl[b]);
+            if (ks + 1 < KS1) {
+                const unsigned o = (unsigned)((ks + 1) >> 1) * 4096u + fo[(ks + 1) & 1];
+                bh[b ^ 1] = lds_read(w1 + o);
+                bl[b ^ 1] = lds_read(w1 + (o ^ 32u));
+            }
+            mfma3(ah[ks], al[ks], __builtin_bit_cast(uint4, bh[b]), __builtin_bit_cast(uint4, bl[b]), acc1);
+        }
+
+        stage_block(stage_addr, acc1, sc, sh, std::make_integer_sequence<int, 16>{});
+        u32x4 t[4];
+        t[0] = lds_read_at<0 * 8 * LDC * 4>(pass_addr);
+        t[1] = lds_read_at<1 * 8 * LDC * 4>(pass_addr);
+        t[2] = lds_read_at<2 * 8 * LDC * 4>(pass_addr);
+        t[3] = lds_read_at<3 * 8 * LDC * 4>(pass_addr);
+        lds_wait();
+#pragma unroll
+        for (int q = 0; q < 4; ++q) pin(t[q]);
+        f4v v[4];
+#pragma unroll
+        for (int q = 0; q < 4; ++q) {
+            float x[4] = {__uint_as_float(t[q].x), __uint_as_float(t[q].y), __uint_as_float(t[q].z), __uint_as_float(t[q].w)};
+            if (has_res) {
+                x[0] += res[q].x; x[1] += res[q].y; x[2] += res[q].z; x[3] += res[q].w;
+            }
+            if (relu1) {
+#pragma unroll
+                for (int e = 0; e < 4; ++e) x[e] = x[e] > 0.f ? x[e] : 0.f;
+            }
+            v[q] = f4v{x[0], x[1], x[2], x[3]};
+        }
+        lds_write4_at<0 * 8 * LDC * 4>(pass_addr, __builtin_bit_cast(u32x4, v[0]));
+        lds_write4_at<1 * 8 * LDC * 4>(pass_addr, __builtin_bit_cast(u32x4, v[1]));
+        lds_write4_at<2 * 8 * LDC * 4>(pass_addr, __builtin_bit_cast(u32x4, v[2]));
+        lds_write4_at<3 * 8 * LDC * 4>(pass_addr, __builtin_bit_cast(u32x4, v[3]));
+        u32x4 xa[2][2];
+        xa[0][0] = lds_read_at<0>(a_addr);
+        xa[0][1] = lds_read_at<16>(a_addr);
+        xa[1][0] = lds_read_at<64>(a_addr);
+        xa[1][1] = lds_read_at<80>(a_addr);
+        bh[0] = lds_read(w2 + fo[0]);
+        bl[0] = lds_read(w2 + (fo[0] ^ 32u));
+        if (cb + 1 < NCB) load_epi(cb + 1);
+        asm volatile("" ::: "memory");
+        if (full) {
+#pragma unroll
+            for (int q = 0; q < 4; ++q) __builtin_nontemporal_store(v[q], reinterpret_cast<f4v*>(obase + ooff[q] + cb * CB));
+        } else {
+#pragma unroll
+            for (int q = 0; q < 4; ++q)
+                if (row_ok[q]) __builtin_nontemporal_store(v[q], reinterpret_cast<f4v*>(obase + ooff[q] + cb * CB));
+        }
+        asm volatile("" ::: "memory");
+
+        uint4 xh[2], xl[2];
+        constexpr int NS = 2 * NJ;
+#pragma unroll
+        for (int s = 0; s < NS; ++s) {
+            const int ks = s / NJ, j = s % NJ, b = s & 1;
+            lds_wait();
+            pin(bh[b]);
+            pin(bl[b]);
+            if (s == 0) {
+                pin(xa[0][0]); pin(xa[0][1]); pin(xa[1][0]); pin(xa[1][1]);
+                split8(xa[0][0], xa[0][1], xh[0], xl[0]);
+                split8(xa[1][0], xa[1][1], xh[1], xl[1]);
+            }
+            if (s + 1 < NS) {
+                const unsigned o = (unsigned)((s + 1) % NJ) * 4096u + fo[(s + 1) / NJ];
+                bh[b ^ 1] = lds_read(w2 + o);
+                bl[b ^ 1] = lds_read(w2 + (o ^ 32u));
+            }
+            mfma3(xh[ks], xl[ks], __builtin_bit_cast(uint4, bh[b]), __builtin_bit_cast(uint4, bl[b]), acc2[j >> 1][0][j & 1]);
+        }
+    }
+
+    __syncthreads();
+    float* sC = reinterpret_cast<float*>(smem) + (tid >> 6) * (32 * (64 + 4));
+    auto epi2 = [&](auto g) { conv_epilogue_vec<float, 8, 1, 2, 32, 64, false>(p2, acc2[decltype(g)::value], sC, lane, tid >> 6, decltype(g)::value, m0, 0, Mlim); };
+    epi2(std::integral_constant<int, 0>{});
+    if constexpr (N2 >= 128) epi2(std::integral_constant<int, 1>{});
+    if constexpr (N2 >= 256) {
+        epi2(std::integral_constant<int, 2>{});
+        epi2(std::integral_constant<int, 3>{});
+    }
+#endif
+}
+
+template <int K1, int N2, int NW>
+static int launch_join(ConvArgs& a, const ConvArgs& a2, hipStream_t st) {
+    constexpr size_t ring = 2 * (size_t)(K1 / 8 + N2 / 8) * 1024 + (size_t)NW * kJoinBlockBytes;
+    constexpr size_t epi = (size_t)NW * 32 * (64 + 4) * 4;
+    constexpr size_t lds = ring > epi ? ring : epi;
+    const int tiles_m = div_up(a.M, 32 * NW);
+    return launch_lds_dma(conv_x3_join_kernel<K1, N2, NW>, dim3((unsigned)tiles_m), dim3(NW * 64), lds, lds, "conv_x3_join_kernel", a, st,
+                          tiles_m, 1, 1, a2);
+}
+
+int launch_conv_x3_join(const ConvChoice& c, ConvArgs& a, const ConvArgs& a2, hipStream_t st) {
+    const int k1 = a.Cin, n2 = a2.Cout, nw = c.waves_m;
+    if (k1 == 64 && n2 == 64 && nw == 8) return launch_join<64, 64, 8>(a, a2, st);
+    if (k1 == 64 && n2 == 128 && nw == 8) return launch_join<64, 128, 8>(a, a2, st);
+    if (k1 == 128 && n2 == 128 && nw == 8) return launch_join<128, 128, 8>(a, a2, st);
+    if (k1 == 128 && n2 == 256 && nw == 4) return launch_join<128, 256, 4>(a, a2, st);
+    if (k1 == 256 && n2 == 256 && nw == 4) return launch_join<256, 256, 4>(a, a2, st);
+    TT_REQUIRE(false, "tt_conv2d_fwd: no conv_x3_join_kernel<%d, %d, %d>", k1, n2, nw);
+}
+
+}
diff --git a/thinktwice_amd/csrc/plan_thunks.inc b/thinktwice_amd/csrc/plan_thunks.inc
--- a/thinktwice_amd/csrc/plan_thunks.inc
+++ b/thinktwice_amd/csrc/plan_thunks.inc
@@ -8,6 +8,7 @@
 static int thunk_tt_lift_splat_fwd(const PlanVal* a, void* stream) { return tt_lift_splat_fwd((int)a[0].i, (int)a[1].i, (int)a[2].i, (int)a[3].i, (int)a[4].i, (int)a[5].i, (int)a[6].i, (int)a[7].i, (int)a[8].i, (const void*)a[9].p, (const void*)a[10].p, (int)a[11].i, (const int32_t*)a[12].p, (float*)a[13].p, (int)a[14].i, (int)a[15].i, (int)a[16].i, stream); }
 static int thunk_tt_lift_splat_fwd_ws(const PlanVal* a, void* stream) { return tt_lift_splat_fwd_ws((int)a[0].i, (int)a[1].i, (int)a[2].i, (int)a[3].i, (int)a[4].i, (int)a[5].i, (int)a[6].i, (int)a[7].i, (int)a[8].i, (const void*)a[9].p, (const void*)a[10].p, (int)a[11].i, (const int32_t*)a[12].p, (float*)a[13].p, (int)a[14].i, (int)a[15].i, (int)a[16].i, (void*)a[17].p, (long long)a[18].i, stream); }
 static int thunk_tt_conv2d_fwd(const PlanVal* a, void* stream) { return tt_conv2d_fwd((const tt_conv_desc*)a[0].p, stream); }
+static int thunk_tt_conv2d_fwd_next(const PlanVal* a, void* stream) { return tt_conv2d_fwd_next((const tt_conv_desc*)a[0].p, (const tt_conv_next*)a[1].p, stream); }
 static int thunk_tt_seg_feedback_chain(const PlanVal* a, void* stream) { return tt_seg_feedback_chain((const float*)a[0].p, (long long)a[1].i, (int)a[2].i, (int)a[3].i, (const float*)a[4].p, (const float*)a[5].p, (const float*)a[6].p, (int)a[7].i, (const float*)a[8].p, (const void*)a[9].p, (int)a[10].i, (const float*)a[11].p, (const float*)a[12].p, (int)a[13].i, (float*)a[14].p, (int)a[15].i, (int)a[16].i, stream); }
 static int thunk_tt_mlp_chain(const PlanVal* a, void* stream) { return tt_mlp_chain((const float*)a[0].p, (long long)a[1].i, (int)a[2].i, (int)a[3].i, (const tt_chain_stage*)a[4].p, (int)a[5].i, stream); }
 static int thunk_tt_mlp_chain_wide(const PlanVal* a, void* stream) { return tt_mlp_chain_wide((const float*)a[0].p, (long long)a[1].i, (int)a[2].i, (int)a[3].i, (const tt_chain_stage*)a[4].p, (int)a[5].i, (void*)a[6].p, (long long)a[7].i, stream); }
@@ -118,6 +119,7 @@
     {"tt_lift_splat_fwd", thunk_tt_lift_splat_fwd, 17},
     {"tt_lift_splat_fwd_ws", thunk_tt_lift_splat_fwd_ws, 19},
     {"tt_conv2d_fwd", thunk_tt_conv2d_fwd, 1},
+    {"tt_conv2d_fwd_next", thunk_tt_conv2d_fwd_next, 2},
     {"tt_seg_feedback_chain", thunk_tt_seg_feedback_chain, 17},
     {"tt_mlp_chain", thunk_tt_mlp_chain, 6},
     {"tt_mlp_chain_wide", thunk_tt_mlp_chain_wide, 8},
diff --git a/thinktwice_amd/layers.py b/thinktwice_amd/layers.py
--- a/thinktwice_amd/layers.py
+++ b/thinktwice_amd/layers.py
@@ -45,7 +45,10 @@
         self.ps2 = pixel_shuffle2
         self.cin = w.shape[-1]
 
-    def __call__(self, x, **kw):
+    def __call__(self, x, join=None, **kw):
+        if join is not None:
+            assert not BN_TRAIN
+            kw["nxt"] = (join.w, join.w_x3, join.scale, join.shift, join.act)
         if BN_TRAIN and self.bn is not None:
             return self._bn_train(x, **kw)
         return ops.conv2d(x, self.w, stride=self.stride, pad=self.pad, dil=self.dil, scale=self.scale,
diff --git a/thinktwice_amd/lss.py b/thinktwice_amd/lss.py
--- a/thinktwice_amd/lss.py
+++ b/thinktwice_amd/lss.py
@@ -60,16 +60,34 @@
             y = self.stem(x, stop_grad=True)
         x = ops.maxpool3x3s2(y)
         outs = []
-        for stage in self.blocks:
-            for blk in stage:
-                idt = blk["ds"](x) if blk["ds"] is not None else x
-                c2 = blk["c2"]
-                rows2 = x.shape[0] * (x.shape[1] // c2.stride) * (x.shape[2] // c2.stride)
-                pr = (c2.w_x3 is not None and not layers.BN_TRAIN and
-                      ops.pair_ok(min(rows2, x.shape[0] * x.shape[1] * x.shape[2]), c2.w.shape[-1], c2.w.shape[0]))
-                y = c2(blk["c1"](x, out_pair=pr), in_pair=pr)
-                x = blk["c3"](y, res1=idt)
-            outs.append(x)
+
+        def pair_c1(blk, shape):
+            c2 = blk["c2"]
+            rows2 = shape[0] * (shape[1] // c2.stride) * (shape[2] // c2.stride)
+            return (c2.w_x3 is not None and not layers.BN_TRAIN and
+                    ops.pair_ok(min(rows2, shape[0] * shape[1] * shape[2]), c2.w.shape[-1], c2.w.shape[0]))
+
+        from . import autodiff
+        flat = [blk for stage in self.blocks for blk in stage]
+        last = [len(stage) for stage in self.blocks]
+        last = [sum(last[:i + 1]) - 1 for i in range(len(last))]
+        y1 = None
+        for i, blk in enumerate(flat):
+            idt = blk["ds"](x) if blk["ds"] is not None else x
+            pr = pair_c1(blk, x.shape)
+            if y1 is None:
+                y1 = blk["c1"](x, out_pair=pr)
+            y = blk["c2"](y1, in_pair=pr)
+            c3, nb = blk["c3"], flat[i + 1] if i + 1 < len(flat) else None
+            rows = y.shape[0] * y.shape[1] * y.shape[2]
+            if (nb is not None and autodiff.TAPE is None and not layers.BN_TRAIN and c3.w_x3 is not None and
+                    nb["c1"].w_x3 is not None and pair_c1(nb, y.shape) and
+                    ops.join_ok(rows, c3.w.shape[-1], c3.w.shape[0], nb["c1"].w.shape[0])):
+                x, y1 = c3(y, res1=idt, join=nb["c1"])
+            else:
+                x, y1 = c3(y, res1=idt), None
+            if i in last:
+                outs.append(x)
         return outs
 
 
diff --git a/thinktwice_amd/ops.py b/thinktwice_amd/ops.py
--- a/thinktwice_amd/ops.py
+++ b/thinktwice_amd/ops.py
@@ -79,6 +79,7 @@
 CONV_BYTES = None
 
 _ConvDesc = _lib.structs()["tt_conv_desc"]
+_ConvNext = _lib.structs()["tt_conv_next"]
 
 
 def _last_conv_kernel():
@@ -194,7 +195,7 @@
            res2=None, res2_coff=0, out=None, out_coff=0, in_coff=0, cin=None, pixel_shuffle2=False,
            shift_n=None, shift_n_mod=1, out_dtype=None, out_nstride=0, out_hw=None, splitk_ws=None,
            in_cstride=None, w_x3=None, _no_tape=False, stop_grad=False, bn_raw=False, in_pair=False, out_pair=False,
-           w_h2=None, out2=None, out2_coff=0, res1_up=False, in_up2=False):
+           w_h2=None, out2=None, out2_coff=0, res1_up=False, in_up2=False, nxt=None, nxt_out=None, nxt_out_coff=0):
     require_cuda(x, w)
     assert w.is_contiguous() and x.dim() == 4 and w.dim() == 4
     N, H, W, Cs = x.shape
@@ -252,6 +253,19 @@
         if autodiff.TAPE is not None:
             raise _lib.TTError("conv2d: in_up2 is an inference-path fusion (the tape records bilinear_up2 and the convolution apart)")
         d.in_up2 = 1
+    nout, dn = None, None
+    if nxt is not None:
+        if autodiff.TAPE is not None:
+            raise _lib.TTError("conv2d: a joined stage is an inference-path fusion (the tape records the two convolutions apart)")
+        nw, nw_x3, nscale, nshift, nact = nxt
+        assert w_x3 is not None and nw_x3 is not None and x.dtype == torch.float32 and out.dtype == torch.float32 and splitk_ws is None
+        assert nw.is_contiguous() and nw_x3.is_contiguous() and tuple(nw.shape[1:]) == (1, 1, Cout) and nw_x3.shape == nw.shape
+        nout = nxt_out if nxt_out is not None else torch.empty(N, OH, OW, nw.shape[0], dtype=torch.float32, device=x.device)
+        assert nout.dtype == torch.float32 and nout.is_contiguous() and tuple(nout.shape[:3]) == (N, OH, OW)
+        dn = _ConvNext()
+        dn.next_weight = nw.data_ptr(); dn.next_weight_x3 = nw_x3.data_ptr(); dn.next_cout = nw.shape[0]
+        dn.next_scale = ptr(nscale); dn.next_shift = ptr(nshift); dn.next_act = nact
+        dn.next_out = nout.data_ptr(); dn.next_out_cstride = nout.shape[-1]; dn.next_out_coff = nxt_out_coff; dn.next_out_pair = 1
     if w_x3 is not None and Cout < 64 and (autodiff.TAPE is not None or _no_tape):
         w_x3 = None
     if w_x3 is not None:
@@ -271,11 +285,16 @@
     if CONV_PROFILE is not None:
         e0, e1 = torch.cuda.Event(enable_timing=True), torch.cuda.Event(enable_timing=True)
         e0.record()
-    rc = lib().tt_conv2d_fwd(ctypes.byref(d), cur_stream(x.device))
+    if dn is not None:
+        rc = lib().tt_conv2d_fwd_next(ctypes.byref(d), ctypes.byref(dn), cur_stream(x.device))
+    else:
+        rc = lib().tt_conv2d_fwd(ctypes.byref(d), cur_stream(x.device))
     check(rc, "tt_conv2d_fwd")
     if CONV_PROFILE is not None:
         e1.record()
-        CONV_PROFILE.append((2.0 * N * OH * OW * Cout * KH * KW * Cin, e0, e1,
+        n2 = 0 if nout is None else nxt[0].shape[0]
+        CONV_PROFILE.append((2.0 * N * OH * OW * Cout * (KH * KW * Cin + n2), e0, e1,
+                             f"M={N * OH * OW} N={Cout}->{n2} K={Cin} join k1x1s1" if n2 else
                              f"M={N * OH * OW} N={Cout} K={KH * KW * Cin} k{KH}x{KW}s{stride}"))
         if CONV_KERNELS is not None:
             CONV_KERNELS.append(_last_conv_kernel())
@@ -286,13 +305,14 @@
             wsz = w.numel() * w.element_size() * (2 if w_h2 is not None else 1)
             CONV_BYTES.append(in_px * (in_cstride or Cin) * esz + m_out * Cout * osz + wsz +
                               m_out * Cout * esz * ((res1 is not None) + (res2 is not None)) +
-                              (m_out * Cout * 4 if out2 is not None else 0))
+                              (m_out * Cout * 4 if out2 is not None else 0) +
+                              (m_out * n2 * 4 + nxt[0].numel() * 4 if n2 else 0))
     if not _no_tape:
         from . import autodiff
         if autodiff.TAPE is not None:
             autodiff.TAPE.conv(x, w, out, stride, pad, dil, scale, shift, act, in_coff, cin, out_coff, res1, res1_coff,
                                res2, res2_coff, pixel_shuffle2, in_cstride, shift_n, shift_n_mod, stop_grad, bn_raw)
-    return out
+    return out if nout is None else (out, nout)
 
 
 SEG_CHAIN = os.environ.get("TT_SEG_CHAIN", "1") != "0"
@@ -498,6 +518,16 @@
     from . import autodiff
     return (PAIR and autodiff.TAPE is None and rows > 4096 and cin % 32 == 0 and taps * cin >= 64 and
             (8 <= cout <= 32 or cout >= 64))
+
+
+BNECK_JOIN = os.environ.get("TT_BNECK_JOIN", "1") != "0"
+JOIN_MIN_ROWS = 32768
+JOIN_ROUTED = ((64, 256, 64), (64, 256, 128), (128, 512, 128))
+
+
+def join_ok(rows, k1, cout, next_cout):
+    from . import autodiff
+    return BNECK_JOIN and autodiff.TAPE is None and rows >= JOIN_MIN_ROWS and (k1, cout, next_cout) in JOIN_ROUTED
 
 
 SEG_UP2 = os.environ.get("TT_SEG_UP2", "1") != "0"
```
